# OFA-Sys/ONE-PEACE

Hardware: AMD Instinct MI355X
Metric: pretrain samples/s (tri-modal global batch) ONE-PEACE-4B (higher is better)
Workload: dtype bf16

## Files before the change

one-peace_amd/csrc/attention.hip:

```cpp
#include <type_traits>

#include "common.h"

namespace {

constexpr int HD = 64;
constexpr int BQ = 128;
constexpr int BKV = 64;
constexpr int VSTRIDE = 160;

struct AttnArgs {
  const bf16_t* q; const bf16_t* k; const bf16_t* v; int64_t ld;
  const bf16_t* bias;
  int64_t bias_bs;
  const uint8_t* key_pad;
  bf16_t* out; int64_t ldo;
  float* lse;
  int64_t lse_ld;
  int B, S, Spad, heads;
  float scale;
};

__device__ __forceinline__ bf16x8 pack8(const float* a, const float* b) {
  bf16x8 r;
#pragma unroll
  for (int i = 0; i < 4; ++i) { r[i] = (bf16_t)a[i]; r[4 + i] = (bf16_t)b[i]; }
  return r;
}

__device__ __forceinline__ s16x4 tr_read(const char* p) {
  return __builtin_amdgcn_ds_read_tr16_b64_v4i16((__attribute__((address_space(3))) s16x4*)(p));
}

__device__ __forceinline__ bf16x8 join_tr(s16x4 a, s16x4 b) {
  typedef __attribute__((ext_vector_type(8))) short s16x8;
  s16x8 r = {a[0], a[1], a[2], a[3], b[0], b[1], b[2], b[3]};
  return __builtin_bit_cast(bf16x8, r);
}

__device__ __forceinline__ int tr_off_swz(int rowblk, int db, int g, int t) {
  const int row = rowblk * 16 + g * 4 + (t >> 2);
  const int c = db * 2 + ((t >> 1) & 1);
  return row * 128 + ((c ^ (row & 7)) << 4) + (t & 1) * 8;
}

__device__ __forceinline__ void xcd_work_item(int& bx, int& by, int& bz) {
  const int nx = gridDim.x, ny = gridDim.y;
  const int total = nx * ny * (int)gridDim.z;
  int lin = blockIdx.x + nx * (blockIdx.y + ny * blockIdx.z);
  if ((total & 7) == 0) lin = (lin & 7) * (total >> 3) + (lin >> 3);
  bx = lin % nx;
  by = (lin / nx) % ny;
  bz = lin / (nx * ny);
}

template <bool HAS_BIAS, bool HAS_PAD>
__global__ __launch_bounds__(256, 2) void attn_fwd_kernel(AttnArgs p) {
  __shared__ __attribute__((aligned(16))) char smem[BKV * 128 + BKV * VSTRIDE];
  char* ldsK = smem;
  char* ldsV = smem + BKV * 128;
  const int tid = threadIdx.x, lane = tid & 63, wid = tid >> 6;
  const int g = lane >> 4, t = lane & 15;
  int bx, h, b;
  xcd_work_item(bx, h, b);
  const int q0 = bx * BQ + wid * 32;
  const bool wave_active = q0 < p.S;
  const int64_t row_base = (int64_t)b * p.S;

  bf16x8 qf[2][2];
#pragma unroll
  for (int qb = 0; qb < 2; ++qb) {
    const int qi = min(q0 + qb * 16 + t, p.S - 1);
    const bf16_t* qp = p.q + (row_base + qi) * p.ld + h * HD;
#pragma unroll
    for (int kk = 0; kk < 2; ++kk) qf[qb][kk] = *reinterpret_cast<const bf16x8*>(qp + kk * 32 + g * 8);
  }

  f32x4 ot[2][4];
  float m_run[2], l_run[2];
#pragma unroll
  for (int qb = 0; qb < 2; ++qb) {
    m_run[qb] = -INFINITY;
    l_run[qb] = 0.f;
#pragma unroll
    for (int db = 0; db < 4; ++db) ot[qb][db] = (f32x4){0.f, 0.f, 0.f, 0.f};
  }

  u32x4 rk[2], rv[2];
  int st_row[2], st_c[2];
#pragma unroll
  for (int i = 0; i < 2; ++i) {
    const int c2 = tid + 256 * i;
    st_row[i] = c2 >> 3;
    st_c[i] = c2 & 7;
  }
  auto load_tile = [&](int k0) {
#pragma unroll
    for (int i = 0; i < 2; ++i) {
      const int kr = min(k0 + st_row[i], p.S - 1);
      const int64_t off = (row_base + kr) * p.ld + h * HD + st_c[i] * 8;
      rk[i] = *reinterpret_cast<const u32x4*>(p.k + off);
      rv[i] = *reinterpret_cast<const u32x4*>(p.v + off);
    }
  };
  auto write_tile = [&]() {
#pragma unroll
    for (int i = 0; i < 2; ++i) {
      *reinterpret_cast<u32x4*>(ldsK + st_row[i] * 128 + ((st_c[i] ^ (st_row[i] & 7)) << 4)) = rk[i];
      *reinterpret_cast<u32x4*>(ldsV + st_row[i] * VSTRIDE + st_c[i] * 16) = rv[i];
    }
  };

  const bf16_t* brow[2] = {nullptr, nullptr};
  if constexpr (HAS_BIAS) {
#pragma unroll
    for (int qb = 0; qb < 2; ++qb) {
      const int qi = min(q0 + qb * 16 + t, p.S - 1);
      brow[qb] = p.bias + (int64_t)b * p.bias_bs + ((int64_t)h * p.S + qi) * p.Spad + g * 4;
    }
  }
  const uint8_t* padrow = HAS_PAD ? p.key_pad + (int64_t)b * p.Spad + g * 4 : nullptr;

  auto tile = [&](const int k0, auto full_c) {
    constexpr bool FULL = decltype(full_c)::value;
    const int nkb = FULL ? 4 : ((p.S - k0 + 15) >> 4);
    bf16x4 bv[2][4];
    unsigned padw[4] = {0u, 0u, 0u, 0u};
    if constexpr (HAS_BIAS) {
#pragma unroll
      for (int qb = 0; qb < 2; ++qb)
#pragma unroll
        for (int kb = 0; kb < 4; ++kb) bv[qb][kb] = *reinterpret_cast<const bf16x4*>(brow[qb] + k0 + kb * 16);
    }
    if constexpr (HAS_PAD) {
#pragma unroll
      for (int kb = 0; kb < 4; ++kb) padw[kb] = *reinterpret_cast<const unsigned*>(padrow + k0 + kb * 16);
    }

    f32x4 st[2][4];
#pragma unroll
    for (int qb = 0; qb < 2; ++qb)
#pragma unroll
      for (int kb = 0; kb < 4; ++kb) st[qb][kb] = (f32x4){0.f, 0.f, 0.f, 0.f};
#pragma unroll
    for (int kb = 0; kb < 4; ++kb) {
      if (!FULL && kb >= nkb) break;
#pragma unroll
      for (int kk = 0; kk < 2; ++kk) {
        const bf16x8 kf = *reinterpret_cast<const bf16x8*>(ldsK + (kb * 16 + t) * 128 + (((kk * 4 + g) ^ (t & 7)) << 4));
#pragma unroll
        for (int qb = 0; qb < 2; ++qb)
          st[qb][kb] = __builtin_amdgcn_mfma_f32_16x16x32_bf16(kf, qf[qb][kk], st[qb][kb], 0, 0, 0);
      }
    }

    bf16x8 pf[2][2];
#pragma unroll
    for (int qb = 0; qb < 2; ++qb) {
      float mx = -INFINITY;
#pragma unroll
      for (int kb = 0; kb < 4; ++kb) {
        const int key = k0 + kb * 16 + g * 4;
#pragma unroll
        for (int r = 0; r < 4; ++r) {
          float s = st[qb][kb][r] * p.scale;
          if constexpr (HAS_BIAS) s += (float)bv[qb][kb][r];
          if constexpr (!FULL || HAS_PAD) {
            bool masked = false;
            if constexpr (!FULL) masked = key + r >= p.S;
            if constexpr (HAS_PAD) masked = masked || ((padw[kb] >> (8 * r)) & 0xffu);
            s = masked ? -INFINITY : s;
          }
          st[qb][kb][r] = s;
          mx = fmaxf(mx, s);
        }
      }
      mx = fmaxf(mx, __shfl_xor(mx, 16));
      mx = fmaxf(mx, __shfl_xor(mx, 32));
      const float m_new = fmaxf(m_run[qb], mx);
      const float m_use = (m_new == -INFINITY) ? 0.f : m_new;
      const float alpha = __expf(m_run[qb] - m_use);
      m_run[qb] = m_new;
      float psum = 0.f;
      float pv[4][4];
#pragma unroll
      for (int kb = 0; kb < 4; ++kb)
#pragma unroll
        for (int r = 0; r < 4; ++r) {
          const float e = __expf(st[qb][kb][r] - m_use);
          pv[kb][r] = e;
          psum += e;
        }
      l_run[qb] = l_run[qb] * alpha + psum;
#pragma unroll
      for (int db = 0; db < 4; ++db)
#pragma unroll
        for (int r = 0; r < 4; ++r) ot[qb][db][r] *= alpha;
      pf[qb][0] = pack8(pv[0], pv[1]);
      pf[qb][1] = pack8(pv[2], pv[3]);
    }

#pragma unroll
    for (int m = 0; m < 2; ++m) {
      if (!FULL && 2 * m >= nkb) break;
#pragma unroll
      for (int db = 0; db < 4; ++db) {
        const char* base = ldsV + (t >> 2) * VSTRIDE + (db * 16 + (t & 3) * 4) * 2;
        const s16x4 v0 = tr_read(base + ((2 * m) * 16 + g * 4) * VSTRIDE);
        const s16x4 v1 = tr_read(base + ((2 * m + 1) * 16 + g * 4) * VSTRIDE);
        const bf16x8 vf = join_tr(v0, v1);
#pragma unroll
        for (int qb = 0; qb < 2; ++qb)
          ot[qb][db] = __builtin_amdgcn_mfma_f32_16x16x32_bf16(vf, pf[qb][m], ot[qb][db], 0, 0, 0);
      }
    }
  };

  const int ntiles = (p.S + BKV - 1) / BKV;
  load_tile(0);
  for (int kt = 0; kt < ntiles; ++kt) {
    const int k0 = kt * BKV;
    __syncthreads();
    write_tile();
    __syncthreads();
    if (kt + 1 < ntiles) load_tile(k0 + BKV);
    if (!wave_active) continue;
    if (k0 + BKV <= p.S) tile(k0, std::true_type{});
    else tile(k0, std::false_type{});
  }

  if (!wave_active) return;
#pragma unroll
  for (int qb = 0; qb < 2; ++qb) {
    float l = l_run[qb];
    l += __shfl_xor(l, 16);
    l += __shfl_xor(l, 32);
    const int qi = q0 + qb * 16 + t;
    if (qi >= p.S) continue;
    const float inv = 1.f / l;
    bf16_t* op = p.out + (row_base + qi) * p.ldo + h * HD;
#pragma unroll
    for (int db = 0; db < 4; ++db) {
      bf16x4 o;
#pragma unroll
      for (int r = 0; r < 4; ++r) o[r] = (bf16_t)(ot[qb][db][r] * inv);
      *reinterpret_cast<bf16x4*>(op + db * 16 + g * 4) = o;
    }
    if (g == 0 && p.lse) p.lse[((int64_t)b * p.heads + h) * p.lse_ld + qi] = m_run[qb] + logf(l);
  }
}


constexpr int RES_MAX_S = 320;
constexpr int RES_MAX_NW = 10;
constexpr float LOG2E = 1.4426950408889634f;

constexpr int FRAG_BLOCK = 512;

template <bool HAS_BIAS, bool HAS_PAD>
__global__ __launch_bounds__(RES_MAX_NW * 64, 5) void attn_fwd_res_kernel(AttnArgs p, const bf16_t* __restrict__ bias_frag,
                                                                            int rows_pad, int qb_per_wg, int abl) {
  extern __shared__ __attribute__((aligned(16))) char smem[];
  char* ldsK = smem;
  char* ldsV = smem + rows_pad * 128;
  const int tid = threadIdx.x, lane = tid & 63;
  const int wid = __builtin_amdgcn_readfirstlane(tid >> 6);
  const int nw = blockDim.x >> 6;
  const int g = lane >> 4, t = lane & 15;
  int bx, h, b;
  xcd_work_item(bx, h, b);
  const int64_t row_base = (int64_t)b * p.S;

  if (!(abl & 1)) {
    const int ngrp = rows_pad >> 3;
    const int r_in = lane >> 3, slot = lane & 7;
    for (int grp = wid; grp < 2 * ngrp; grp += nw) {
      const bool isv = grp >= ngrp;
      const int gi = isv ? grp - ngrp : grp;
      const int r = gi * 8 + r_in;
      const int kr = min(r, p.S - 1);
      const bf16_t* src = (isv ? p.v : p.k) + (row_base + kr) * p.ld + h * HD + ((slot ^ (r & 7)) << 3);
      char* dst = (isv ? ldsV : ldsK) + gi * 1024;
      __builtin_amdgcn_global_load_lds((const __attribute__((address_space(1))) void*)src,
                                       (__attribute__((address_space(3))) void*)dst, 16, 0, 0);
    }
  }

  const int nqb = (p.S + 15) >> 4, nkp = (p.S + 31) >> 5;
  for (int lblk = wid, trip = 0; trip == 0 || lblk < qb_per_wg; lblk += nw, ++trip) {
  const int qblk = bx * qb_per_wg + lblk;
  const bool active = lblk < qb_per_wg && qblk < nqb;
  const int q0 = min(qblk, nqb - 1) * 16;
  const int qi = min(q0 + t, p.S - 1);

  bf16x8 qf[2];
  {
    const bf16_t* qp = p.q + (row_base + qi) * p.ld + h * HD;
#pragma unroll
    for (int kk = 0; kk < 2; ++kk) qf[kk] = *reinterpret_cast<const bf16x8*>(qp + kk * 32 + g * 8);
  }
  const bf16_t* fbase = nullptr;
  if constexpr (HAS_BIAS) {
    const int64_t per_head = (int64_t)nqb * nkp * FRAG_BLOCK;
    fbase = bias_frag + ((p.bias_bs != 0 ? (int64_t)b * p.heads : 0) + h) * per_head + (int64_t)(q0 >> 4) * nkp * FRAG_BLOCK + lane * 8;
  }
  const uint8_t* padrow = HAS_PAD ? p.key_pad + (int64_t)b * p.Spad + g * 4 : nullptr;
  bf16x8 sel_lo, sel_hi;
  {
    const bf16_t inv = (bf16_t)(1.0f / p.scale), zero = (bf16_t)0.f;
#pragma unroll
    for (int i = 0; i < 8; ++i) {
      sel_lo[i] = (g * 8 + i == t) ? inv : zero;
      sel_hi[i] = (g * 8 + i == 16 + t) ? inv : zero;
    }
  }

  if (trip == 0) {
    asm volatile("s_waitcnt vmcnt(0)" ::: "memory");
    __syncthreads();
  }
  if (!active || (abl & 2)) continue;

  f32x4 ot[4];
  float m2_run = -INFINITY, l_run = 0.f;
#pragma unroll
  for (int db = 0; db < 4; ++db) ot[db] = (f32x4){0.f, 0.f, 0.f, 0.f};
  int trsw[4];
#pragma unroll
  for (int db = 0; db < 4; ++db) trsw[db] = tr_off_swz(0, db, g, t);
  const int kswz[2] = {((0 * 4 + g) ^ (t & 7)) << 4, ((1 * 4 + g) ^ (t & 7)) << 4};
  const float c1 = p.scale * LOG2E;

  auto tile = [&](const int k0, auto full_c) {
    constexpr bool FULL = decltype(full_c)::value;
    const int nkb = FULL ? 4 : ((p.S - k0 + 15) >> 4);
    bf16x8 bf[2];
    unsigned padw[4] = {0u, 0u, 0u, 0u};
    if constexpr (HAS_BIAS) {
#pragma unroll
      for (int m = 0; m < 2; ++m)
        if (FULL || 2 * m < nkb) bf[m] = *reinterpret_cast<const bf16x8*>(fbase + ((k0 >> 5) + m) * FRAG_BLOCK);
    }
    if constexpr (HAS_PAD) {
#pragma unroll
      for (int kb = 0; kb < 4; ++kb) padw[kb] = *reinterpret_cast<const unsigned*>(padrow + k0 + kb * 16);
    }
    const char* kt = ldsK + k0 * 128;
    const char* vt = ldsV + k0 * 128;

    f32x4 st[4];
#pragma unroll
    for (int kb = 0; kb < 4; ++kb) st[kb] = (f32x4){0.f, 0.f, 0.f, 0.f};
#pragma unroll
    for (int kb = 0; kb < 4; ++kb) {
      if (!FULL && kb >= nkb) break;
#pragma unroll
      for (int kk = 0; kk < 2; ++kk) {
        const bf16x8 kf = *reinterpret_cast<const bf16x8*>(kt + (kb * 16 + t) * 128 + kswz[kk]);
        st[kb] = __builtin_amdgcn_mfma_f32_16x16x32_bf16(kf, qf[kk], st[kb], 0, 0, 0);
      }
      if constexpr (HAS_BIAS)
        st[kb] = __builtin_amdgcn_mfma_f32_16x16x32_bf16(bf[kb >> 1], (kb & 1) ? sel_hi : sel_lo, st[kb], 0, 0, 0);
    }

    float mx = -INFINITY;
#pragma unroll
    for (int kb = 0; kb < 4; ++kb) {
      if (!FULL && kb >= nkb) break;
      const int key = k0 + kb * 16 + g * 4;
#pragma unroll
      for (int r = 0; r < 4; ++r) {
        if constexpr (!FULL || HAS_PAD) {
          bool masked = false;
          if constexpr (!FULL) masked = key + r >= p.S;
          if constexpr (HAS_PAD) masked = masked || ((padw[kb] >> (8 * r)) & 0xffu);
          st[kb][r] = masked ? -INFINITY : st[kb][r];
        }
        mx = fmaxf(mx, st[kb][r]);
      }
    }
    mx = fmaxf(mx, __shfl_xor(mx, 16));
    mx = fmaxf(mx, __shfl_xor(mx, 32));
    const float m2_new = fmaxf(m2_run, mx * c1);
    const float m2_use = (m2_new == -INFINITY) ? 0.f : m2_new;
    const float alpha = __builtin_amdgcn_exp2f(m2_run - m2_use);
    m2_run = m2_new;
    float psum = 0.f;
    float pv[4][4];
#pragma unroll
    for (int kb = 0; kb < 4; ++kb) {
      if (FULL || kb < nkb) {
#pragma unroll
        for (int r = 0; r < 4; ++r) {
          const float e = __builtin_amdgcn_exp2f(__builtin_fmaf(st[kb][r], c1, -m2_use));
          pv[kb][r] = e;
          psum += e;
        }
      } else {
#pragma unroll
        for (int r = 0; r < 4; ++r) pv[kb][r] = 0.f;
      }
    }
    l_run = l_run * alpha + psum;
#pragma unroll
    for (int db = 0; db < 4; ++db)
#pragma unroll
      for (int r = 0; r < 4; ++r) ot[db][r] *= alpha;
    bf16x8 pf[2];
    pf[0] = pack8(pv[0], pv[1]);
    pf[1] = pack8(pv[2], pv[3]);

#pragma unroll
    for (int m = 0; m < 2; ++m) {
      if (!FULL && 2 * m >= nkb) break;
#pragma unroll
      for (int db = 0; db < 4; ++db) {
        const bf16x8 vf = join_tr(tr_read(vt + trsw[db] + (2 * m) * 2048), tr_read(vt + trsw[db] + (2 * m + 1) * 2048));
        ot[db] = __builtin_amdgcn_mfma_f32_16x16x32_bf16(vf, pf[m], ot[db], 0, 0, 0);
      }
    }
  };

  const int ntiles = (p.S + BKV - 1) / BKV;
  for (int kt = 0; kt < ntiles; ++kt) {
    const int k0 = kt * BKV;
    if (k0 + BKV <= p.S) tile(k0, std::true_type{});
    else tile(k0, std::false_type{});
  }

  float l = l_run;
  l += __shfl_xor(l, 16);
  l += __shfl_xor(l, 32);
  if (q0 + t >= p.S) continue;
  const float inv = 1.f / l;
  bf16_t* op = p.out + (row_base + q0 + t) * p.ldo + h * HD;
#pragma unroll
  for (int db = 0; db < 4; ++db) {
    bf16x4 o;
#pragma unroll
    for (int r = 0; r < 4; ++r) o[r] = (bf16_t)(ot[db][r] * inv);
    *reinterpret_cast<bf16x4*>(op + db * 16 + g * 4) = o;
  }
  if (g == 0 && p.lse) p.lse[((int64_t)b * p.heads + h) * p.lse_ld + q0 + t] = m2_run * (1.0f / LOG2E) + logf(l);
  }
}

constexpr int PERS_NW = 8;
constexpr int PERS_MAX_ROWS = 288;
constexpr int PERS_SCR = 68;
constexpr int PERS_PPT = 2;

__device__ __forceinline__ s16x4 tr_read_a(const char* p) {
  s16x4 r;
  asm volatile("ds_read_b64_tr_b16 %0, %1" : "=v"(r) : "v"((unsigned)(uintptr_t)((__attribute__((address_space(3))) const char*)p)));
  return r;
}
#define ATTN_WAIT_LGKM0()                         \
  do {                                            \
    __builtin_amdgcn_s_waitcnt(0xC07F);           \
    __builtin_amdgcn_sched_barrier(0);            \
  } while (0)

__device__ __forceinline__ void gload16_asm(bf16x8& d, const void* p) { asm volatile("global_load_dwordx4 %0, %1, off" : "=v"(d) : "v"(p)); }
__device__ __forceinline__ void gload4_asm(unsigned& d, const void* p) { asm volatile("global_load_dword %0, %1, off" : "=v"(d) : "v"(p)); }
template <int OFF>
__device__ __forceinline__ void gload16_s(bf16x8& d, const void* sbase, unsigned voff) {
  asm volatile("s_nop 4\n\tglobal_load_dwordx4 %0, %1, %2 offset:%3" : "=v"(d) : "v"(voff), "s"(sbase), "n"(OFF));
}
template <int OFF>
__device__ __forceinline__ void gload4_s(unsigned& d, const void* sbase, unsigned voff) {
  asm volatile("s_nop 4\n\tglobal_load_dword %0, %1, %2 offset:%3" : "=v"(d) : "v"(voff), "s"(sbase), "n"(OFF));
}

template <bool HAS_BIAS, bool HAS_PAD>
__global__ __launch_bounds__(PERS_NW * 64, 2) void attn_fwd_pers_kernel(AttnArgs p, const bf16_t* __restrict__ bias_frag, int rows_pad,
                                                                         int nitems) {
  extern __shared__ __attribute__((aligned(16))) char smem[];
  const int tid = threadIdx.x, lane = tid & 63;
  const int wid = __builtin_amdgcn_readfirstlane(tid >> 6);
  const int g = lane >> 4, t = lane & 15;
  const int KVB = 2 * rows_pad * 128;
  float* scratch = reinterpret_cast<float*>(smem + 2 * KVB);
  const int nqb = (p.S + 15) >> 4, nkp = (p.S + 31) >> 5;
  const bool has_left = nqb > 2 * PERS_NW;
  const int q0 = wid * 32;
  const int nact = min(2, max(0, nqb - 2 * wid));
  const int64_t per_head = (int64_t)nqb * nkp * FRAG_BLOCK;
  const int ntiles = (p.S + BKV - 1) / BKV;
  const float c1 = p.scale * LOG2E;

  bf16x8 sel_lo, sel_hi;
  {
    const bf16_t inv = (bf16_t)(1.0f / p.scale), zero = (bf16_t)0.f;
#pragma unroll
    for (int i = 0; i < 8; ++i) {
      sel_lo[i] = (g * 8 + i == t) ? inv : zero;
      sel_hi[i] = (g * 8 + i == 16 + t) ? inv : zero;
    }
  }
  int trsw[4];
#pragma unroll
  for (int db = 0; db < 4; ++db) trsw[db] = tr_off_swz(0, db, g, t);
  const int kswz[2] = {((0 * 4 + g) ^ (t & 7)) << 4, ((1 * 4 + g) ^ (t & 7)) << 4};

  const int ngrp = rows_pad >> 3;
  const int r_in = lane >> 3, slot = lane & 7;
  const int npiece = (2 * ngrp - wid + PERS_NW - 1) / PERS_NW;
  auto piece = [&](int it, int buf, int j) {
    const int b = it / p.heads, h = it - b * p.heads;
    const int grp = wid + j * PERS_NW;
    const bool isv = grp >= ngrp;
    const int gi = isv ? grp - ngrp : grp;
    const int r = gi * 8 + r_in;
    const int kr = min(r, p.S - 1);
    const bf16_t* src = (isv ? p.v : p.k) + ((int64_t)b * p.S + kr) * p.ld + h * HD + ((slot ^ (r & 7)) << 3);
    char* dst = smem + buf * KVB + (isv ? rows_pad * 128 : 0) + gi * 1024;
    __builtin_amdgcn_global_load_lds((const __attribute__((address_space(1))) void*)src,
                                     (__attribute__((address_space(3))) void*)dst, 16, 0, 0);
  };
  auto load_q = [&](int it, int qrow, bf16x8 (&q)[2]) {
    const int b = it / p.heads, h = it - b * p.heads;
    const bf16_t* qp = p.q + ((int64_t)b * p.S + qrow) * p.ld + h * HD;
#pragma unroll
    for (int kk = 0; kk < 2; ++kk) q[kk] = *reinterpret_cast<const bf16x8*>(qp + kk * 32 + g * 8);
  };
  const int qi_main[2] = {min(q0 + t, p.S - 1), min(q0 + 16 + t, p.S - 1)};

  bf16x8 bn[2][2];
  unsigned padn[4] = {0u, 0u, 0u, 0u};
  auto small_loads = [&](int it, int kt) {
    const int b = it / p.heads, h = it - b * p.heads;
    if constexpr (HAS_BIAS) {
      const bf16_t* fhead = bias_frag + ((p.bias_bs != 0 ? (int64_t)b * p.heads : 0) + h) * per_head + lane * 8;
#pragma unroll
      for (int qb = 0; qb < 2; ++qb) {
        const bf16_t* fb = fhead + (int64_t)min(2 * wid + qb, nqb - 1) * nkp * FRAG_BLOCK;
#pragma unroll
        for (int m = 0; m < 2; ++m) gload16_asm(bn[qb][m], fb + min(2 * kt + m, nkp - 1) * FRAG_BLOCK);
      }
    }
    if constexpr (HAS_PAD) {
      const uint8_t* pr = p.key_pad + (int64_t)b * p.Spad + g * 4 + kt * BKV;
#pragma unroll
      for (int kb = 0; kb < 4; ++kb) gload4_asm(padn[kb], pr + kb * 16);
    }
  };

  constexpr int NSMALL = (HAS_BIAS ? 4 : 0) + (HAS_PAD ? 4 : 0);
  bf16x8 qn[2][2], ql[2], bfl[2];
  unsigned padl[2][2] = {{0u, 0u}, {0u, 0u}};
  auto late_loads = [&](int it_next, int it) {
    {
      const int b = it_next / p.heads, h = it_next - b * p.heads;
#pragma unroll
      for (int qb = 0; qb < 2; ++qb) {
        const bf16_t* qp = p.q + ((int64_t)b * p.S + qi_main[qb]) * p.ld + h * HD;
#pragma unroll
        for (int kk = 0; kk < 2; ++kk) gload16_asm(qn[qb][kk], qp + kk * 32 + g * 8);
      }
    }
    if (has_left) {
      const int b = it / p.heads, h = it - b * p.heads;
      const bf16_t* qp = p.q + ((int64_t)b * p.S + p.S - 1) * p.ld + h * HD;
#pragma unroll
      for (int kk = 0; kk < 2; ++kk) gload16_asm(ql[kk], qp + kk * 32 + g * 8);
      if constexpr (HAS_BIAS) {
        const bf16_t* fleft = bias_frag + ((p.bias_bs != 0 ? (int64_t)b * p.heads : 0) + h) * per_head + lane * 8 + (int64_t)(nqb - 1) * nkp * FRAG_BLOCK;
        gload16_asm(bfl[0], fleft + wid * FRAG_BLOCK);
        gload16_asm(bfl[1], fleft + min(PERS_NW, nkp - 1) * FRAG_BLOCK);
      }
      if constexpr (HAS_PAD) {
        const uint8_t* pr = p.key_pad + (int64_t)b * p.Spad + g * 4;
#pragma unroll
        for (int j = 0; j < 2; ++j) {
          gload4_asm(padl[0][j], pr + (2 * wid + j) * 16);
          gload4_asm(padl[1][j], pr + min((2 * PERS_NW + j) * 16, p.Spad - 16));
        }
      }
    }
  };

  int item = blockIdx.x;
  const int step = gridDim.x;
  if (item < nitems) {
    for (int j = 0; j < npiece; ++j) piece(item, 0, j);
    load_q(item, qi_main[0], qn[0]);
    load_q(item, qi_main[1], qn[1]);
    small_loads(item, 0);
  }
  int buf = 0, prev_item = -1;
  auto wait_all = [&]() {
    asm volatile("s_waitcnt vmcnt(0)" : "+v"(qn[0][0]), "+v"(qn[0][1]), "+v"(qn[1][0]), "+v"(qn[1][1]), "+v"(bn[0][0]), "+v"(bn[0][1]), "+v"(bn[1][0]), "+v"(bn[1][1]),
                 "+v"(padn[0]), "+v"(padn[1]), "+v"(padn[2]), "+v"(padn[3]) : : "memory");
  };
  wait_all();

  auto merge_left = [&](int it, int sb) {
    const float* sc = scratch + sb * (PERS_NW * PERS_SCR);
    float M = -INFINITY;
#pragma unroll
    for (int w = 0; w < PERS_NW; ++w) M = fmaxf(M, sc[w * PERS_SCR + 64]);
    float L = 0.f, o = 0.f;
#pragma unroll
    for (int w = 0; w < PERS_NW; ++w) {
      const float f = __builtin_amdgcn_exp2f(sc[w * PERS_SCR + 64] - M);
      L = __builtin_fmaf(sc[w * PERS_SCR + 65], f, L);
      o = __builtin_fmaf(sc[w * PERS_SCR + lane], f, o);
    }
    const int b = it / p.heads, h = it - b * p.heads;
    const int qrow = p.S - 1;
    p.out[((int64_t)b * p.S + qrow) * p.ldo + h * HD + lane] = (bf16_t)(o / L);
    if (lane == 0 && p.lse) p.lse[((int64_t)b * p.heads + h) * p.lse_ld + qrow] = M * (1.0f / LOG2E) + logf(L);
  };

  for (; item < nitems; item += step, buf ^= 1) {
    const int b = item / p.heads, h = item - b * p.heads;
    const int64_t row_base = (int64_t)b * p.S;
    __syncthreads();
    bf16x8 qf[2][2] = {{qn[0][0], qn[0][1]}, {qn[1][0], qn[1][1]}};
    const bool more = item + step < nitems;
    const int nxt = more ? item + step : item;
    if (has_left && prev_item >= 0 && wid == ((prev_item / step) & (PERS_NW - 1))) merge_left(prev_item, buf ^ 1);
    prev_item = item;

    const char* ldsK = smem + buf * KVB;
    const char* ldsV = ldsK + rows_pad * 128;

    f32x4 ot[2][4];
    float m2_run[2] = {-INFINITY, -INFINITY}, l_run[2] = {0.f, 0.f};
#pragma unroll
    for (int qb = 0; qb < 2; ++qb)
#pragma unroll
      for (int db = 0; db < 4; ++db) ot[qb][db] = (f32x4){0.f, 0.f, 0.f, 0.f};

    auto tile = [&](const int kt, auto full_c) {
      constexpr bool FULL = decltype(full_c)::value;
      const int k0 = kt * BKV;
      const int nkb = FULL ? 4 : ((p.S - k0 + 15) >> 4);
      bf16x8 bf[2][2];
      unsigned padw[4] = {0u, 0u, 0u, 0u};
      if constexpr (HAS_BIAS) {
#pragma unroll
        for (int qb = 0; qb < 2; ++qb)
#pragma unroll
          for (int m = 0; m < 2; ++m) bf[qb][m] = bn[qb][m];
      }
      if constexpr (HAS_PAD) {
#pragma unroll
        for (int kb = 0; kb < 4; ++kb) padw[kb] = padn[kb];
      }
      __builtin_amdgcn_sched_barrier(0);
      if constexpr (FULL) {
        small_loads(item, kt + 1);
      } else {
        late_loads(nxt, item);
        small_loads(nxt, 0);
      }
      __builtin_amdgcn_sched_barrier(0);
#pragma unroll
      for (int jj = 0; jj < PERS_PPT; ++jj) piece(nxt, buf ^ 1, min(kt * PERS_PPT + jj, npiece - 1));
      __builtin_amdgcn_sched_barrier(0);
      if (nact == 0) return;

      const char* kt_ = ldsK + k0 * 128;
      const char* vt = ldsV + k0 * 128;
      f32x4 st[2][4];
#pragma unroll
      for (int qb = 0; qb < 2; ++qb)
#pragma unroll
        for (int kb = 0; kb < 4; ++kb) st[qb][kb] = (f32x4){0.f, 0.f, 0.f, 0.f};
#pragma unroll
      for (int kb = 0; kb < 4; ++kb) {
        if (!FULL && kb >= nkb) break;
#pragma unroll
        for (int kk = 0; kk < 2; ++kk) {
          const bf16x8 kf = *reinterpret_cast<const bf16x8*>(kt_ + (kb * 16 + t) * 128 + kswz[kk]);
#pragma unroll
          for (int qb = 0; qb < 2; ++qb) st[qb][kb] = __builtin_amdgcn_mfma_f32_16x16x32_bf16(kf, qf[qb][kk], st[qb][kb], 0, 0, 0);
        }
        if constexpr (HAS_BIAS) {
#pragma unroll
          for (int qb = 0; qb < 2; ++qb)
            st[qb][kb] = __builtin_amdgcn_mfma_f32_16x16x32_bf16(bf[qb][kb >> 1], (kb & 1) ? sel_hi : sel_lo, st[qb][kb], 0, 0, 0);
        }
      }
      s16x4 va0[4], va1[4];
#pragma unroll
      for (int db = 0; db < 4; ++db) {
        va0[db] = tr_read_a(vt + trsw[db]);
        va1[db] = tr_read_a(vt + trsw[db] + 2048);
      }
      bf16x8 pf[2][2];
#pragma unroll
      for (int qb = 0; qb < 2; ++qb) {
        float mx = -INFINITY;
#pragma unroll
        for (int kb = 0; kb < 4; ++kb) {
          if (!FULL && kb >= nkb) break;
          const int key = k0 + kb * 16 + g * 4;
#pragma unroll
          for (int r = 0; r < 4; ++r) {
            if constexpr (!FULL || HAS_PAD) {
              bool masked = false;
              if constexpr (!FULL) masked = key + r >= p.S;
              if constexpr (HAS_PAD) masked = masked || ((padw[kb] >> (8 * r)) & 0xffu);
              st[qb][kb][r] = masked ? -INFINITY : st[qb][kb][r];
            }
            mx = fmaxf(mx, st[qb][kb][r]);
          }
        }
        mx = fmaxf(mx, __shfl_xor(mx, 16));
        mx = fmaxf(mx, __shfl_xor(mx, 32));
        const float m2_new = fmaxf(m2_run[qb], mx * c1);
        const float m2_use = (m2_new == -INFINITY) ? 0.f : m2_new;
        const float alpha = __builtin_amdgcn_exp2f(m2_run[qb] - m2_use);
        m2_run[qb] = m2_new;
        float psum = 0.f;
        float pv[4][4];
#pragma unroll
        for (int kb = 0; kb < 4; ++kb) {
          if (FULL || kb < nkb) {
#pragma unroll
            for (int r = 0; r < 4; ++r) {
              const float e = __builtin_amdgcn_exp2f(__builtin_fmaf(st[qb][kb][r], c1, -m2_use));
              pv[kb][r] = e;
              psum += e;
            }
          } else {
#pragma unroll
            for (int r = 0; r < 4; ++r) pv[kb][r] = 0.f;
          }
        }
        l_run[qb] = l_run[qb] * alpha + psum;
#pragma unroll
        for (int db = 0; db < 4; ++db)
#pragma unroll
          for (int r = 0; r < 4; ++r) ot[qb][db][r] *= alpha;
        pf[qb][0] = pack8(pv[0], pv[1]);
        pf[qb][1] = pack8(pv[2], pv[3]);
      }
      const bool second = FULL || nkb > 2;
      ATTN_WAIT_LGKM0();
      s16x4 vb0[4], vb1[4];
      if (second) {
#pragma unroll
        for (int db = 0; db < 4; ++db) {
          vb0[db] = tr_read_a(vt + trsw[db] + 2 * 2048);
          vb1[db] = tr_read_a(vt + trsw[db] + 3 * 2048);
        }
      }
#pragma unroll
      for (int db = 0; db < 4; ++db) {
        const bf16x8 vf = join_tr(va0[db], va1[db]);
#pragma unroll
        for (int qb = 0; qb < 2; ++qb) ot[qb][db] = __builtin_amdgcn_mfma_f32_16x16x32_bf16(vf, pf[qb][0], ot[qb][db], 0, 0, 0);
      }
      if (second) {
        ATTN_WAIT_LGKM0();
#pragma unroll
        for (int db = 0; db < 4; ++db) {
          const bf16x8 vf = join_tr(vb0[db], vb1[db]);
#pragma unroll
          for (int qb = 0; qb < 2; ++qb) ot[qb][db] = __builtin_amdgcn_mfma_f32_16x16x32_bf16(vf, pf[qb][1], ot[qb][db], 0, 0, 0);
        }
      }
    };
    auto wait_small = [&]() {
      if constexpr (HAS_BIAS && HAS_PAD)
        asm volatile("s_waitcnt vmcnt(%8)" : "+v"(bn[0][0]), "+v"(bn[0][1]), "+v"(bn[1][0]), "+v"(bn[1][1]), "+v"(padn[0]), "+v"(padn[1]), "+v"(padn[2]), "+v"(padn[3]) : "n"(PERS_PPT));
      else if constexpr (HAS_BIAS)
        asm volatile("s_waitcnt vmcnt(%4)" : "+v"(bn[0][0]), "+v"(bn[0][1]), "+v"(bn[1][0]), "+v"(bn[1][1]) : "n"(PERS_PPT));
      else if constexpr (HAS_PAD)
        asm volatile("s_waitcnt vmcnt(%4)" : "+v"(padn[0]), "+v"(padn[1]), "+v"(padn[2]), "+v"(padn[3]) : "n"(PERS_PPT));
    };
#pragma unroll 1
    for (int kt = 0; kt < ntiles - 1; ++kt) {
      tile(kt, std::true_type{});
      wait_small();
    }
    tile(ntiles - 1, std::false_type{});
    if (has_left) {
      f32x4 ol[4];
      float m2 = -INFINITY, lsum = 0.f;
#pragma unroll
      for (int db = 0; db < 4; ++db) ol[db] = (f32x4){0.f, 0.f, 0.f, 0.f};
      asm volatile("s_waitcnt vmcnt(%8)" : "+v"(ql[0]), "+v"(ql[1]), "+v"(bfl[0]), "+v"(bfl[1]), "+v"(padl[0][0]), "+v"(padl[0][1]), "+v"(padl[1][0]), "+v"(padl[1][1]) : "n"(NSMALL + PERS_PPT));
      const int npc = wid == 0 ? 2 : 1;
      for (int pc = 0; pc < npc; ++pc) {
        const int kp = pc == 0 ? wid : PERS_NW;
        f32x4 s4[2];
        const unsigned padw[2] = {padl[pc][0], padl[pc][1]};
#pragma unroll
        for (int j = 0; j < 2; ++j) {
          s4[j] = (f32x4){0.f, 0.f, 0.f, 0.f};
#pragma unroll
          for (int kk = 0; kk < 2; ++kk) {
            const bf16x8 kf = *reinterpret_cast<const bf16x8*>(ldsK + ((2 * kp + j) * 16 + t) * 128 + kswz[kk]);
            s4[j] = __builtin_amdgcn_mfma_f32_16x16x32_bf16(kf, ql[kk], s4[j], 0, 0, 0);
          }
          if constexpr (HAS_BIAS) s4[j] = __builtin_amdgcn_mfma_f32_16x16x32_bf16(bfl[pc], j ? sel_hi : sel_lo, s4[j], 0, 0, 0);
        }
        float mx = -INFINITY;
#pragma unroll
        for (int j = 0; j < 2; ++j)
#pragma unroll
          for (int r = 0; r < 4; ++r) {
            bool masked = (2 * kp + j) * 16 + g * 4 + r >= p.S;
            if constexpr (HAS_PAD) masked = masked || ((padw[j] >> (8 * r)) & 0xffu);
            s4[j][r] = masked ? -INFINITY : s4[j][r];
            mx = fmaxf(mx, s4[j][r]);
          }
        mx = fmaxf(mx, __shfl_xor(mx, 16));
        mx = fmaxf(mx, __shfl_xor(mx, 32));
        const float m2_new = fmaxf(m2, mx * c1);
        const float m2_use = (m2_new == -INFINITY) ? 0.f : m2_new;
        const float alpha = __builtin_amdgcn_exp2f(m2 - m2_use);
        m2 = m2_new;
        float pv[2][4];
        float psum = 0.f;
#pragma unroll
        for (int j = 0; j < 2; ++j)
#pragma unroll
          for (int r = 0; r < 4; ++r) {
            pv[j][r] = __builtin_amdgcn_exp2f(__builtin_fmaf(s4[j][r], c1, -m2_use));
            psum += pv[j][r];
          }
        lsum = lsum * alpha + psum;
        const bf16x8 pf = pack8(pv[0], pv[1]);
        s16x4 v0[4], v1[4];
#pragma unroll
        for (int db = 0; db < 4; ++db) {
          v0[db] = tr_read_a(ldsV + trsw[db] + (2 * kp) * 2048);
          v1[db] = tr_read_a(ldsV + trsw[db] + (2 * kp + 1) * 2048);
        }
        ATTN_WAIT_LGKM0();
#pragma unroll
        for (int db = 0; db < 4; ++db) {
#pragma unroll
          for (int r = 0; r < 4; ++r) ol[db][r] *= alpha;
          ol[db] = __builtin_amdgcn_mfma_f32_16x16x32_bf16(join_tr(v0[db], v1[db]), pf, ol[db], 0, 0, 0);
        }
      }
      lsum += __shfl_xor(lsum, 16);
      lsum += __shfl_xor(lsum, 32);
      float* sc = scratch + (buf * PERS_NW + wid) * PERS_SCR;
      if (t == 0) {
#pragma unroll
        for (int db = 0; db < 4; ++db) *reinterpret_cast<f32x4*>(sc + db * 16 + g * 4) = ol[db];
        if (g == 0) { sc[64] = m2; sc[65] = lsum; }
      }
    }
#pragma unroll
    for (int qb = 0; qb < 2; ++qb) {
      float l = l_run[qb];
      l += __shfl_xor(l, 16);
      l += __shfl_xor(l, 32);
      const int qrow = q0 + qb * 16 + t;
      if (qb < nact && qrow < p.S) {
        const float inv = 1.f / l;
        bf16_t* op = p.out + (row_base + qrow) * p.ldo + h * HD;
#pragma unroll
        for (int db = 0; db < 4; ++db) {
          bf16x4 o;
#pragma unroll
          for (int r = 0; r < 4; ++r) o[r] = (bf16_t)(ot[qb][db][r] * inv);
          *reinterpret_cast<bf16x4*>(op + db * 16 + g * 4) = o;
        }
        if (g == 0 && p.lse) p.lse[((int64_t)b * p.heads + h) * p.lse_ld + qrow] = m2_run[qb] * (1.0f / LOG2E) + logf(l);
      }
    }
    wait_all();
  }
  if (has_left && prev_item >= 0) {
    __syncthreads();
    if (wid == 0) merge_left(prev_item, buf ^ 1);
  }
}

__global__ __launch_bounds__(256) void bias_pack_kernel(const bf16_t* __restrict__ src, bf16_t* __restrict__ dst, int S, int Spad,
                                                        int nqb, int nkp, int64_t total) {
  const int64_t idx = (int64_t)blockIdx.x * 256 + threadIdx.x;
  if (idx >= total) return;
  const int lane = (int)(idx & 63);
  int64_t blk = idx >> 6;
  const int kp = (int)(blk % nkp);
  blk /= nkp;
  const int qb = (int)(blk % nqb);
  const int64_t img = blk / nqb;
  const int g = lane >> 4, t = lane & 15;
  const int key = kp * 32 + (g >> 1) * 16 + t;
  const int qbase = qb * 16 + (g & 1) * 8;
  bf16x8 v;
#pragma unroll
  for (int i = 0; i < 8; ++i) {
    const int q = qbase + i;
    v[i] = (q < S && key < S) ? src[(img * S + q) * Spad + key] : (bf16_t)0.f;
  }
  *reinterpret_cast<bf16x8*>(dst + idx * 8) = v;
}

struct AttnBwdArgs {
  const bf16_t* q; const bf16_t* k; const bf16_t* v; int64_t ld;
  const bf16_t* dout; int64_t ldo;
  const bf16_t* bias;
  const bf16_t* biasT;
  const bf16_t* bias_frag;
  int64_t bias_bs;
  const uint8_t* key_pad;
  const float* lse;
  const float* delta;
  const bf16_t* out;
  float* delta_w;
  bf16_t* dq; bf16_t* dk; bf16_t* dv; int64_t ldg;
  float* dbias;
  int B, S, Spad, heads, bchunk;
  float scale;
  int lone_keys;
};

__global__ __launch_bounds__(256) void attn_delta_kernel(const bf16_t* __restrict__ dout, const bf16_t* __restrict__ out,
                                                         int64_t ldo, float* __restrict__ delta, int B, int S, int Spad,
                                                         int heads) {
  const int64_t gid = (int64_t)blockIdx.x * 256 + threadIdx.x;
  const int per_row = heads * 8;
  const int64_t row = gid / per_row;
  const int rem = (int)(gid - row * per_row);
  float s = 0.f;
  if (row < (int64_t)B * S) {
    float a[8], b[8];
    Vec8<bf16_t>::load(dout + row * ldo + rem * 8, a);
    Vec8<bf16_t>::load(out + row * ldo + rem * 8, b);
#pragma unroll
    for (int j = 0; j < 8; ++j) s += a[j] * b[j];
  }
  s += __shfl_xor(s, 1);
  s += __shfl_xor(s, 2);
  s += __shfl_xor(s, 4);
  if (row < (int64_t)B * S && (rem & 7) == 0) {
    const int h = rem >> 3;
    const int64_t bb = row / S;
    const int qi = (int)(row - bb * S);
    delta[(bb * heads + h) * Spad + qi] = s;
  }
}

__device__ __forceinline__ float delta_from_frags(const bf16x8 (&dO)[2], const bf16x8 (&O)[2]) {
  float s = 0.f;
#pragma unroll
  for (int kk = 0; kk < 2; ++kk)
#pragma unroll
    for (int i = 0; i < 8; ++i) s = __builtin_fmaf((float)dO[kk][i], (float)O[kk][i], s);
  s += __shfl_xor(s, 16);
  s += __shfl_xor(s, 32);
  return s;
}

template <bool HAS_BIAS, int KBW, bool LONE>
__device__ __forceinline__ void attn_bwd_dkdv_body(const AttnBwdArgs& p, char* smem, int bx, int h, int b) {
  constexpr int KB = LONE ? 1 : KBW;
  char* ldsQ = smem;
  char* ldsO = smem + 64 * 128;
  const int tid = threadIdx.x, lane = tid & 63, wid = tid >> 6;
  const int g = lane >> 4, t = lane & 15;
  const int kbase = LONE ? bx * (64 * KBW) : bx * (64 * KBW) + wid * (16 * KBW);
  const bool wave_active = LONE || kbase < p.S;
  const int my_m = wid >> 1, my_j = wid & 1;
  const int64_t row_base = (int64_t)b * p.S;

  bf16x8 kf[KB][2], vf[KB][2];
  bool kdead[KB];
#pragma unroll
  for (int kb = 0; kb < KB; ++kb) {
    const int key = kbase + kb * 16 + t;
    const int kc = min(key, p.S - 1);
    const int64_t off = (row_base + kc) * p.ld + h * HD;
#pragma unroll
    for (int kk = 0; kk < 2; ++kk) {
      kf[kb][kk] = *reinterpret_cast<const bf16x8*>(p.k + off + kk * 32 + g * 8);
      vf[kb][kk] = *reinterpret_cast<const bf16x8*>(p.v + off + kk * 32 + g * 8);
    }
    kdead[kb] = p.key_pad && key < p.S && p.key_pad[(int64_t)b * p.Spad + key];
  }
  f32x4 dvT[KB][4], dkT[KB][4];
#pragma unroll
  for (int kb = 0; kb < KB; ++kb)
#pragma unroll
    for (int db = 0; db < 4; ++db) { dvT[kb][db] = (f32x4){0.f, 0.f, 0.f, 0.f}; dkT[kb][db] = (f32x4){0.f, 0.f, 0.f, 0.f}; }

  u32x4 rq[2], ro[2];
  int st_row[2], st_c[2];
#pragma unroll
  for (int i = 0; i < 2; ++i) { const int c2 = tid + 256 * i; st_row[i] = c2 >> 3; st_c[i] = c2 & 7; }
  auto load_tile = [&](int q0) {
#pragma unroll
    for (int i = 0; i < 2; ++i) {
      const int qr = min(q0 + st_row[i], p.S - 1);
      rq[i] = *reinterpret_cast<const u32x4*>(p.q + (row_base + qr) * p.ld + h * HD + st_c[i] * 8);
      ro[i] = *reinterpret_cast<const u32x4*>(p.dout + (row_base + qr) * p.ldo + h * HD + st_c[i] * 8);
    }
  };
  auto write_tile = [&]() {
#pragma unroll
    for (int i = 0; i < 2; ++i) {
      const int off = st_row[i] * 128 + ((st_c[i] ^ (st_row[i] & 7)) << 4);
      *reinterpret_cast<u32x4*>(ldsQ + off) = rq[i];
      *reinterpret_cast<u32x4*>(ldsO + off) = ro[i];
    }
  };
  int trsw[4];
#pragma unroll
  for (int db = 0; db < 4; ++db) trsw[db] = tr_off_swz(0, db, g, t);

  const int ntiles = (p.S + 63) / 64;
  const float* lse_b = p.lse + ((int64_t)b * p.heads + h) * p.Spad;
  const float* del_b = p.delta + ((int64_t)b * p.heads + h) * p.Spad;
  const bf16_t* brow[KB] = {};
  bf16x8 sel_lo, sel_hi;
  if constexpr (HAS_BIAS) {
#pragma unroll
    for (int kb = 0; kb < KB; ++kb) {
      const int key = min(kbase + kb * 16 + t, p.S - 1);
      brow[kb] = p.biasT + (int64_t)b * p.bias_bs + ((int64_t)h * p.S + key) * p.Spad + g * 8;
    }
    const bf16_t inv = (bf16_t)(1.0f / p.scale), zero = (bf16_t)0.f;
#pragma unroll
    for (int i = 0; i < 8; ++i) {
      sel_lo[i] = (g * 8 + i == t) ? inv : zero;
      sel_hi[i] = (g * 8 + i == 16 + t) ? inv : zero;
    }
  }
  const float c1 = p.scale * LOG2E;
  load_tile(0);
  for (int qt = 0; qt < ntiles; ++qt) {
    const int q0 = qt * 64;
    __syncthreads();
    write_tile();
    __syncthreads();
    if (!wave_active) {
      load_tile(q0 + 64);
      continue;
    }
    f32x4 l4[2][2], d4[2][2];
    bf16x8 bfr[2][KB];
#pragma unroll
    for (int m = 0; m < 2; ++m) {
#pragma unroll
      for (int j = 0; j < 2; ++j) {
        const int qrow = q0 + (2 * m + j) * 16 + g * 4;
        l4[m][j] = *reinterpret_cast<const f32x4*>(lse_b + qrow);
        d4[m][j] = *reinterpret_cast<const f32x4*>(del_b + qrow);
      }
      if constexpr (HAS_BIAS) {
#pragma unroll
        for (int kb = 0; kb < KB; ++kb) bfr[m][kb] = *reinterpret_cast<const bf16x8*>(brow[kb] + q0 + m * 32);
      }
    }
    __builtin_amdgcn_sched_barrier(0);
    load_tile(q0 + 64);
    __builtin_amdgcn_sched_barrier(0);

#pragma unroll
    for (int m = 0; m < 2; ++m) {
      if (q0 + m * 32 >= p.S) break;
      if (LONE && (m != my_m || q0 + (2 * m + my_j) * 16 >= p.S)) continue;
      f32x4 s[2][KB], dp[2][KB];
#pragma unroll
      for (int j = 0; j < 2; ++j)
#pragma unroll
        for (int kb = 0; kb < KB; ++kb) { s[j][kb] = (f32x4){0.f, 0.f, 0.f, 0.f}; dp[j][kb] = (f32x4){0.f, 0.f, 0.f, 0.f}; }
#pragma unroll
      for (int j = 0; j < 2; ++j) {
        if (LONE && j != my_j) continue;
        if (q0 + (2 * m + j) * 16 >= p.S) continue;
        const int qb = 2 * m + j;
#pragma unroll
        for (int kk = 0; kk < 2; ++kk) {
          const int off = (qb * 16 + t) * 128 + (((kk * 4 + g) ^ (t & 7)) << 4);
          const bf16x8 qfr = *reinterpret_cast<const bf16x8*>(ldsQ + off);
          const bf16x8 ofr = *reinterpret_cast<const bf16x8*>(ldsO + off);
#pragma unroll
          for (int kb = 0; kb < KB; ++kb) {
            s[j][kb] = __builtin_amdgcn_mfma_f32_16x16x32_bf16(qfr, kf[kb][kk], s[j][kb], 0, 0, 0);
            dp[j][kb] = __builtin_amdgcn_mfma_f32_16x16x32_bf16(ofr, vf[kb][kk], dp[j][kb], 0, 0, 0);
          }
        }
        if constexpr (HAS_BIAS) {
#pragma unroll
          for (int kb = 0; kb < KB; ++kb)
            s[j][kb] = __builtin_amdgcn_mfma_f32_16x16x32_bf16(j ? sel_hi : sel_lo, bfr[m][kb], s[j][kb], 0, 0, 0);
        }
      }
#pragma unroll
      for (int j = 0; j < 2; ++j) {
        if ((LONE && j != my_j) || q0 + (2 * m + j) * 16 >= p.S) continue;
        const int qrow = q0 + (2 * m + j) * 16 + g * 4;
        float l2[4], dl[4];
#pragma unroll
        for (int r = 0; r < 4; ++r) {
          const bool live = qrow + r < p.S;
          l2[r] = live ? l4[m][j][r] * LOG2E : INFINITY;
          dl[r] = live ? d4[m][j][r] : 0.f;
        }
#pragma unroll
        for (int kb = 0; kb < KB; ++kb) {
#pragma unroll
          for (int r = 0; r < 4; ++r) {
            const float pr = __builtin_amdgcn_exp2f(__builtin_fmaf(s[j][kb][r], c1, -l2[r]));
            s[j][kb][r] = pr;
            dp[j][kb][r] = pr * (dp[j][kb][r] - dl[r]);
          }
        }
      }
      bf16x8 pfr[KB], dsf[KB];
#pragma unroll
      for (int kb = 0; kb < KB; ++kb) {
        float a0[4], a1[4], b0[4], b1[4];
#pragma unroll
        for (int r = 0; r < 4; ++r) {
          a0[r] = s[0][kb][r]; a1[r] = s[1][kb][r];
          b0[r] = dp[0][kb][r]; b1[r] = dp[1][kb][r];
        }
        pfr[kb] = pack8(a0, a1);
        dsf[kb] = pack8(b0, b1);
      }
#pragma unroll
      for (int db = 0; db < 4; ++db) {
        const bf16x8 oT = join_tr(tr_read(ldsO + trsw[db] + (2 * m) * 2048), tr_read(ldsO + trsw[db] + (2 * m + 1) * 2048));
        const bf16x8 qT = join_tr(tr_read(ldsQ + trsw[db] + (2 * m) * 2048), tr_read(ldsQ + trsw[db] + (2 * m + 1) * 2048));
#pragma unroll
        for (int kb = 0; kb < KB; ++kb) {
          dvT[kb][db] = __builtin_amdgcn_mfma_f32_16x16x32_bf16(oT, pfr[kb], dvT[kb][db], 0, 0, 0);
          dkT[kb][db] = __builtin_amdgcn_mfma_f32_16x16x32_bf16(qT, dsf[kb], dkT[kb][db], 0, 0, 0);
        }
      }
    }
  }
  if (!wave_active) return;
  if constexpr (LONE) {
    f32x4* red = reinterpret_cast<f32x4*>(smem);
#pragma unroll
    for (int which = 0; which < 2; ++which) {
      __syncthreads();
      if (wid > 0) {
#pragma unroll
        for (int db = 0; db < 4; ++db) red[((wid - 1) * 4 + db) * 64 + lane] = which ? dkT[0][db] : dvT[0][db];
      }
      __syncthreads();
      if (wid == 0) {
#pragma unroll
        for (int w = 0; w < 3; ++w)
#pragma unroll
          for (int db = 0; db < 4; ++db) {
            if (which) dkT[0][db] += red[(w * 4 + db) * 64 + lane];
            else dvT[0][db] += red[(w * 4 + db) * 64 + lane];
          }
      }
    }
    if (wid > 0) return;
  }
#pragma unroll
  for (int kb = 0; kb < KB; ++kb) {
    const int key = kbase + kb * 16 + t;
    if (key >= p.S) continue;
    bf16_t* kp = p.dk + (row_base + key) * p.ldg + h * HD;
    bf16_t* vp = p.dv + (row_base + key) * p.ldg + h * HD;
#pragma unroll
    for (int db = 0; db < 4; ++db) {
      bf16x4 a, c;
#pragma unroll
      for (int r = 0; r < 4; ++r) {
        a[r] = kdead[kb] ? (bf16_t)0.f : (bf16_t)(dkT[kb][db][r] * p.scale);
        c[r] = kdead[kb] ? (bf16_t)0.f : (bf16_t)dvT[kb][db][r];
      }
      *reinterpret_cast<bf16x4*>(kp + db * 16 + g * 4) = a;
      *reinterpret_cast<bf16x4*>(vp + db * 16 + g * 4) = c;
    }
  }
}

template <bool HAS_BIAS, int KB>
__global__ __launch_bounds__(256, KB == 1 ? 3 : 2) void attn_bwd_dkdv_kernel(AttnBwdArgs p) {
  __shared__ __attribute__((aligned(16))) char smem[2 * 64 * 128];
  int bx, h, b;
  xcd_work_item(bx, h, b);
  if (KB == 2 && bx > 0 && p.S - bx * 128 <= 16 && p.lone_keys) attn_bwd_dkdv_body<HAS_BIAS, KB, true>(p, smem, bx, h, b);
  else attn_bwd_dkdv_body<HAS_BIAS, KB, false>(p, smem, bx, h, b);
}

template <int QB, bool HAS_BIAS, bool HOIST, typename KF, typename VF, typename BF, typename PF>
__device__ __forceinline__ void ds_tile(const AttnBwdArgs& p, int b, int h, int k0, int q0w, int g, int t,
                                        const bf16x8 (&qf)[QB][2], const bf16x8 (&of)[QB][2], const float (&lse)[QB],
                                        const float (&del)[QB], KF kfrag, VF vfrag, BF biasfrag, PF prefetch,
                                        f32x4 (&ds)[QB][4]) {
  unsigned padw[4] = {0u, 0u, 0u, 0u};
  auto load_pad = [&]() {
    if (p.key_pad) {
#pragma unroll
      for (int kb = 0; kb < 4; ++kb)
        padw[kb] = *reinterpret_cast<const unsigned*>(p.key_pad + (int64_t)b * p.Spad + k0 + kb * 16 + g * 4);
    }
  };
  if constexpr (HOIST) load_pad();
  bf16x4 bv[QB][4];
  if constexpr (HAS_BIAS && HOIST) {
#pragma unroll
    for (int qb = 0; qb < QB; ++qb) {
      const int qi = min(q0w + qb * 16 + t, p.S - 1);
#pragma unroll
      for (int kb = 0; kb < 4; ++kb) bv[qb][kb] = biasfrag(qb, kb, qi, k0 + kb * 16 + g * 4);
    }
  }
  if constexpr (HOIST) __builtin_amdgcn_sched_barrier(0);
  prefetch();
  if constexpr (HOIST) __builtin_amdgcn_sched_barrier(0);
  f32x4 st[QB][4];
#pragma unroll
  for (int qb = 0; qb < QB; ++qb)
#pragma unroll
    for (int kb = 0; kb < 4; ++kb) { st[qb][kb] = (f32x4){0.f, 0.f, 0.f, 0.f}; ds[qb][kb] = (f32x4){0.f, 0.f, 0.f, 0.f}; }
#pragma unroll
  for (int kb = 0; kb < 4; ++kb) {
    if (k0 + kb * 16 >= p.S) break;
#pragma unroll
    for (int kk = 0; kk < 2; ++kk) {
      const bf16x8 kfr = kfrag(kb, kk);
      const bf16x8 vfr = vfrag(kb, kk);
#pragma unroll
      for (int qb = 0; qb < QB; ++qb) {
        st[qb][kb] = __builtin_amdgcn_mfma_f32_16x16x32_bf16(kfr, qf[qb][kk], st[qb][kb], 0, 0, 0);
        ds[qb][kb] = __builtin_amdgcn_mfma_f32_16x16x32_bf16(vfr, of[qb][kk], ds[qb][kb], 0, 0, 0);
      }
    }
  }
  if constexpr (!HOIST) load_pad();
#pragma unroll
  for (int qb = 0; qb < QB; ++qb) {
    const int qraw = q0w + qb * 16 + t;
    const int qi = min(qraw, p.S - 1);
#pragma unroll
    for (int kb = 0; kb < 4; ++kb) {
      const int key = k0 + kb * 16 + g * 4;
      if constexpr (HAS_BIAS && !HOIST) bv[qb][kb] = biasfrag(qb, kb, qi, key);
#pragma unroll
      for (int r = 0; r < 4; ++r) {
        const bool dead = (key + r >= p.S) || ((padw[kb] >> (8 * r)) & 0xffu) || (qraw >= p.S);
        float x = st[qb][kb][r] * p.scale;
        if constexpr (HAS_BIAS) x += (float)bv[qb][kb][r];
        x -= lse[qb];
        float pr;
        if constexpr (HOIST) pr = __expf(dead ? -INFINITY : x);
        else pr = dead ? 0.f : __expf(x);
        const float dsv = pr * (ds[qb][kb][r] - del[qb]);
        ds[qb][kb][r] = dead ? 0.f : dsv;
      }
    }
  }
}

template <bool HAS_BIAS>
__global__ __launch_bounds__(256, 2) void attn_bwd_dq_kernel(AttnBwdArgs p) {
  __shared__ __attribute__((aligned(16))) char smem[2 * 64 * 128];
  char* ldsK = smem;
  char* ldsV = smem + 64 * 128;
  const int tid = threadIdx.x, lane = tid & 63, wid = tid >> 6;
  const int g = lane >> 4, t = lane & 15;
  int bx, h, b;
  xcd_work_item(bx, h, b);
  const int q0w = bx * BQ + wid * 32;
  const bool wave_active = q0w < p.S;
  const int64_t row_base = (int64_t)b * p.S;

  bf16x8 qf[2][2], of[2][2];
  float lse[2], del[2];
#pragma unroll
  for (int qb = 0; qb < 2; ++qb) {
    const int qi = min(q0w + qb * 16 + t, p.S - 1);
#pragma unroll
    for (int kk = 0; kk < 2; ++kk) {
      qf[qb][kk] = *reinterpret_cast<const bf16x8*>(p.q + (row_base + qi) * p.ld + h * HD + kk * 32 + g * 8);
      of[qb][kk] = *reinterpret_cast<const bf16x8*>(p.dout + (row_base + qi) * p.ldo + h * HD + kk * 32 + g * 8);
    }
    lse[qb] = p.lse[((int64_t)b * p.heads + h) * p.Spad + qi];
    if (p.out) {
      bf16x8 oo[2];
#pragma unroll
      for (int kk = 0; kk < 2; ++kk) oo[kk] = *reinterpret_cast<const bf16x8*>(p.out + (row_base + qi) * p.ldo + h * HD + kk * 32 + g * 8);
      del[qb] = delta_from_frags(of[qb], oo);
      if (g == 0 && q0w + qb * 16 + t < p.S) p.delta_w[((int64_t)b * p.heads + h) * p.Spad + qi] = del[qb];
    } else {
      del[qb] = p.delta[((int64_t)b * p.heads + h) * p.Spad + qi];
    }
  }
  f32x4 dqT[2][4];
#pragma unroll
  for (int qb = 0; qb < 2; ++qb)
#pragma unroll
    for (int db = 0; db < 4; ++db) dqT[qb][db] = (f32x4){0.f, 0.f, 0.f, 0.f};

  u32x4 rk[2], rv[2];
  int st_row[2], st_c[2];
#pragma unroll
  for (int i = 0; i < 2; ++i) { const int c2 = tid + 256 * i; st_row[i] = c2 >> 3; st_c[i] = c2 & 7; }
  auto load_tile = [&](int k0) {
#pragma unroll
    for (int i = 0; i < 2; ++i) {
      const int kr = min(k0 + st_row[i], p.S - 1);
      const int64_t off = (row_base + kr) * p.ld + h * HD + st_c[i] * 8;
      rk[i] = *reinterpret_cast<const u32x4*>(p.k + off);
      rv[i] = *reinterpret_cast<const u32x4*>(p.v + off);
    }
  };
  auto write_tile = [&]() {
#pragma unroll
    for (int i = 0; i < 2; ++i) {
      const int off = st_row[i] * 128 + ((st_c[i] ^ (st_row[i] & 7)) << 4);
      *reinterpret_cast<u32x4*>(ldsK + off) = rk[i];
      *reinterpret_cast<u32x4*>(ldsV + off) = rv[i];
    }
  };
  int trsw[4];
#pragma unroll
  for (int db = 0; db < 4; ++db) trsw[db] = tr_off_swz(0, db, g, t);

  const int ntiles = (p.S + BKV - 1) / BKV;
  load_tile(0);
  for (int kt = 0; kt < ntiles; ++kt) {
    const int k0 = kt * BKV;
    __syncthreads();
    write_tile();
    __syncthreads();
    if (!wave_active) {
      load_tile(k0 + BKV);
      continue;
    }
    auto prefetch = [&]() { load_tile(k0 + BKV); };
    f32x4 ds[2][4];
    auto kfrag = [&](int kb, int kk) {
      return *reinterpret_cast<const bf16x8*>(ldsK + (kb * 16 + t) * 128 + (((kk * 4 + g) ^ (t & 7)) << 4));
    };
    auto vfrag = [&](int kb, int kk) {
      return *reinterpret_cast<const bf16x8*>(ldsV + (kb * 16 + t) * 128 + (((kk * 4 + g) ^ (t & 7)) << 4));
    };
    auto biasfrag = [&](int, int, int qi, int key) {
      return *reinterpret_cast<const bf16x4*>(p.bias + (int64_t)b * p.bias_bs + ((int64_t)h * p.S + qi) * p.Spad + key);
    };
    ds_tile<2, HAS_BIAS, true>(p, b, h, k0, q0w, g, t, qf, of, lse, del, kfrag, vfrag, biasfrag, prefetch, ds);
#pragma unroll
    for (int m = 0; m < 2; ++m) {
      if (k0 + m * 32 >= p.S) break;
      bf16x8 dsf[2];
#pragma unroll
      for (int qb = 0; qb < 2; ++qb) {
        float a0[4], a1[4];
#pragma unroll
        for (int r = 0; r < 4; ++r) { a0[r] = ds[qb][2 * m][r]; a1[r] = ds[qb][2 * m + 1][r]; }
        dsf[qb] = pack8(a0, a1);
      }
#pragma unroll
      for (int db = 0; db < 4; ++db) {
        const bf16x8 kT = join_tr(tr_read(ldsK + trsw[db] + (2 * m) * 2048), tr_read(ldsK + trsw[db] + (2 * m + 1) * 2048));
#pragma unroll
        for (int qb = 0; qb < 2; ++qb)
          dqT[qb][db] = __builtin_amdgcn_mfma_f32_16x16x32_bf16(kT, dsf[qb], dqT[qb][db], 0, 0, 0);
      }
    }
  }
  if (!wave_active) return;
#pragma unroll
  for (int qb = 0; qb < 2; ++qb) {
    const int qi = q0w + qb * 16 + t;
    if (qi >= p.S) continue;
    bf16_t* qp = p.dq + (row_base + qi) * p.ldg + h * HD;
#pragma unroll
    for (int db = 0; db < 4; ++db) {
      bf16x4 a;
#pragma unroll
      for (int r = 0; r < 4; ++r) a[r] = (bf16_t)(dqT[qb][db][r] * p.scale);
      *reinterpret_cast<bf16x4*>(qp + db * 16 + g * 4) = a;
    }
  }
}

template <int NT, bool FRAG, int LASTB>
__global__ __launch_bounds__(256, 2) void attn_bwd_dq_dbias_kernel(AttnBwdArgs p) {
  __shared__ __attribute__((aligned(16))) char smem[2 * 64 * 128];
  char* ldsK = smem;
  char* ldsV = smem + 64 * 128;
  const int tid = threadIdx.x, lane = tid & 63, wid = tid >> 6;
  const int g = lane >> 4, t = lane & 15;
  int bx, h, chunk;
  xcd_work_item(bx, h, chunk);
  const int q0w = bx * 64 + wid * 16;
  const bool wave_active = q0w < p.S;
  const int qi = min(q0w + t, p.S - 1);

  f32x4 acc[NT][4];
#pragma unroll
  for (int kt = 0; kt < NT; ++kt)
#pragma unroll
    for (int kb = 0; kb < 4; ++kb) acc[kt][kb] = (f32x4){0.f, 0.f, 0.f, 0.f};

  u32x4 rk[2], rv[2];
  int st_row[2], st_c[2];
#pragma unroll
  for (int i = 0; i < 2; ++i) { const int c2 = tid + 256 * i; st_row[i] = c2 >> 3; st_c[i] = c2 & 7; }
  auto load_tile = [&](int b, int k0) {
#pragma unroll
    for (int i = 0; i < 2; ++i) {
      const int kr = min(k0 + st_row[i], p.S - 1);
      const int64_t off = ((int64_t)b * p.S + kr) * p.ld + h * HD + st_c[i] * 8;
      rk[i] = *reinterpret_cast<const u32x4*>(p.k + off);
      rv[i] = *reinterpret_cast<const u32x4*>(p.v + off);
    }
  };
  auto write_tile = [&]() {
#pragma unroll
    for (int i = 0; i < 2; ++i) {
      const int off = st_row[i] * 128 + ((st_c[i] ^ (st_row[i] & 7)) << 4);
      *reinterpret_cast<u32x4*>(ldsK + off) = rk[i];
      *reinterpret_cast<u32x4*>(ldsV + off) = rv[i];
    }
  };
  bf16x8 qn[1][2], on[1][2], oon[2];
  float lsen[1], deln[1];
  const bool own_delta = p.out != nullptr;
  auto load_q = [&](int b) {
    const int64_t row = (int64_t)b * p.S + qi;
#pragma unroll
    for (int kk = 0; kk < 2; ++kk) {
      qn[0][kk] = *reinterpret_cast<const bf16x8*>(p.q + row * p.ld + h * HD + kk * 32 + g * 8);
      on[0][kk] = *reinterpret_cast<const bf16x8*>(p.dout + row * p.ldo + h * HD + kk * 32 + g * 8);
      if (own_delta) oon[kk] = *reinterpret_cast<const bf16x8*>(p.out + row * p.ldo + h * HD + kk * 32 + g * 8);
    }
    lsen[0] = p.lse[((int64_t)b * p.heads + h) * p.Spad + qi];
    if (!own_delta) deln[0] = p.delta[((int64_t)b * p.heads + h) * p.Spad + qi];
  };
  int trsw[4];
#pragma unroll
  for (int db = 0; db < 4; ++db) trsw[db] = tr_off_swz(0, db, g, t);

  const int nqb = (p.S + 15) >> 4, nkp = (p.S + 31) >> 5;
  const int64_t per_head = (int64_t)nqb * nkp * FRAG_BLOCK;
  const bf16_t* fbase = nullptr;
  bf16x8 sel_lo, sel_hi;
  const float c1 = p.scale * LOG2E;
  if constexpr (FRAG) {
    fbase = p.bias_frag + (int64_t)h * per_head + (int64_t)(min(q0w, p.S - 1) >> 4) * nkp * FRAG_BLOCK + lane * 8;
    const bf16_t inv = (bf16_t)(1.0f / p.scale), zero = (bf16_t)0.f;
#pragma unroll
    for (int i = 0; i < 8; ++i) {
      sel_lo[i] = (g * 8 + i == t) ? inv : zero;
      sel_hi[i] = (g * 8 + i == 16 + t) ? inv : zero;
    }
  }
  const int b_begin = chunk * p.bchunk, b_end = min(p.B, (chunk + 1) * p.bchunk);
  if (b_begin >= b_end) return;
  load_tile(b_begin, 0);
  load_q(b_begin);
  for (int b = b_begin; b < b_end; ++b) {
    bf16x8 qf[1][2], of[1][2];
    float lse[1], del[1];
#pragma unroll
    for (int kk = 0; kk < 2; ++kk) { qf[0][kk] = qn[0][kk]; of[0][kk] = on[0][kk]; }
    lse[0] = lsen[0];
    if (own_delta) {
      del[0] = delta_from_frags(of[0], oon);
      if (g == 0 && q0w + t < p.S) p.delta_w[((int64_t)b * p.heads + h) * p.Spad + qi] = del[0];
    } else {
      del[0] = deln[0];
    }
    if (b + 1 < b_end) load_q(b + 1);
    int bias_resample = 0;
    asm volatile("" : "+s"(bias_resample));
    f32x4 dqT[4];
#pragma unroll
    for (int db = 0; db < 4; ++db) dqT[db] = (f32x4){0.f, 0.f, 0.f, 0.f};
#pragma unroll 1
    for (int kt = 0; kt < NT; ++kt) {
      const int k0 = kt * BKV;
      __syncthreads();
      write_tile();
      __syncthreads();
      const bool last_kt = kt + 1 >= NT;
      const int nb = last_kt ? min(b + 1, b_end - 1) : b, nk0 = last_kt ? 0 : k0 + BKV;
      auto prefetch = [&]() { load_tile(nb, nk0); };
      if (!wave_active) {
        prefetch();
        continue;
      }
      f32x4 ds[1][4];
      auto kfrag = [&](int kb, int kk) {
        return *reinterpret_cast<const bf16x8*>(ldsK + (kb * 16 + t) * 128 + (((kk * 4 + g) ^ (t & 7)) << 4));
      };
      auto vfrag = [&](int kb, int kk) {
        return *reinterpret_cast<const bf16x8*>(ldsV + (kb * 16 + t) * 128 + (((kk * 4 + g) ^ (t & 7)) << 4));
      };
      auto biasfrag = [&](int, int, int qrow, int key) {
        return *reinterpret_cast<const bf16x4*>(p.bias + bias_resample + (int64_t)b * p.bias_bs + ((int64_t)h * p.S + qrow) * p.Spad + key);
      };
      if constexpr (FRAG) {
        bf16x8 bfr[2];
        unsigned padw[4] = {0u, 0u, 0u, 0u};
        const bf16_t* fb = fbase + (p.bias_bs != 0 ? (int64_t)b * p.heads * per_head : 0) + bias_resample;
#pragma unroll
        for (int m = 0; m < 2; ++m) bfr[m] = *reinterpret_cast<const bf16x8*>(fb + (int64_t)min((k0 >> 5) + m, nkp - 1) * FRAG_BLOCK);
        if (p.key_pad) {
#pragma unroll
          for (int kb = 0; kb < 4; ++kb)
            padw[kb] = *reinterpret_cast<const unsigned*>(p.key_pad + (int64_t)b * p.Spad + k0 + kb * 16 + g * 4);
        }
        __builtin_amdgcn_sched_barrier(0);
        prefetch();
        __builtin_amdgcn_sched_barrier(0);
        f32x4 st[4];
#pragma unroll
        for (int kb = 0; kb < 4; ++kb) { st[kb] = (f32x4){0.f, 0.f, 0.f, 0.f}; ds[0][kb] = (f32x4){0.f, 0.f, 0.f, 0.f}; }
#pragma unroll
        for (int kb = 0; kb < 4; ++kb) {
          if (k0 + kb * 16 >= p.S) break;
#pragma unroll
          for (int kk = 0; kk < 2; ++kk) {
            st[kb] = __builtin_amdgcn_mfma_f32_16x16x32_bf16(kfrag(kb, kk), qf[0][kk], st[kb], 0, 0, 0);
            ds[0][kb] = __builtin_amdgcn_mfma_f32_16x16x32_bf16(vfrag(kb, kk), of[0][kk], ds[0][kb], 0, 0, 0);
          }
          st[kb] = __builtin_amdgcn_mfma_f32_16x16x32_bf16(bfr[kb >> 1], (kb & 1) ? sel_hi : sel_lo, st[kb], 0, 0, 0);
        }
        const float nl2 = -lse[0] * LOG2E, dl = del[0];
        const bool may_mask = (k0 + BKV > p.S) || (p.key_pad != nullptr);
        if (may_mask) {
#pragma unroll
          for (int kb = 0; kb < 4; ++kb) {
            const int key = k0 + kb * 16 + g * 4;
#pragma unroll
            for (int r = 0; r < 4; ++r) {
              const bool dead = (key + r >= p.S) || ((padw[kb] >> (8 * r)) & 0xffu);
              const float pr = __builtin_amdgcn_exp2f(dead ? -INFINITY : __builtin_fmaf(st[kb][r], c1, nl2));
              ds[0][kb][r] = pr * (ds[0][kb][r] - dl);
            }
          }
        } else {
#pragma unroll
          for (int kb = 0; kb < 4; ++kb)
#pragma unroll
            for (int r = 0; r < 4; ++r)
              ds[0][kb][r] = __builtin_amdgcn_exp2f(__builtin_fmaf(st[kb][r], c1, nl2)) * (ds[0][kb][r] - dl);
        }
      } else {
        ds_tile<1, true, (NT < 6)>(p, b, h, k0, q0w, g, t, qf, of, lse, del, kfrag, vfrag, biasfrag, prefetch, ds);
      }
#pragma unroll
      for (int c = 0; c < NT; ++c) {
        if (kt == c) {
#pragma unroll
          for (int kb = 0; kb < 4; ++kb)
            if (c < NT - 1 || kb < LASTB) acc[c][kb] += ds[0][kb];
        }
      }
#pragma unroll
      for (int m = 0; m < 2; ++m) {
        if (k0 + m * 32 >= p.S) break;
        float a0[4], a1[4];
#pragma unroll
        for (int r = 0; r < 4; ++r) { a0[r] = ds[0][2 * m][r]; a1[r] = ds[0][2 * m + 1][r]; }
        const bf16x8 dsf = pack8(a0, a1);
#pragma unroll
        for (int db = 0; db < 4; ++db) {
          const bf16x8 kT = join_tr(tr_read(ldsK + trsw[db] + (2 * m) * 2048), tr_read(ldsK + trsw[db] + (2 * m + 1) * 2048));
          dqT[db] = __builtin_amdgcn_mfma_f32_16x16x32_bf16(kT, dsf, dqT[db], 0, 0, 0);
        }
      }
    }
    if (wave_active && q0w + t < p.S) {
      bf16_t* qp = p.dq + ((int64_t)b * p.S + q0w + t) * p.ldg + h * HD;
#pragma unroll
      for (int db = 0; db < 4; ++db) {
        bf16x4 a;
#pragma unroll
        for (int r = 0; r < 4; ++r) a[r] = (bf16_t)(dqT[db][r] * p.scale);
        *reinterpret_cast<bf16x4*>(qp + db * 16 + g * 4) = a;
      }
    }
  }
  if (!wave_active || q0w + t >= p.S) return;
  float* drow = p.dbias + (((int64_t)chunk * p.heads + h) * p.S + q0w + t) * p.Spad + g * 4;
#pragma unroll
  for (int kt = 0; kt < NT; ++kt) {
    f32x4 cur[4];
#pragma unroll
    for (int kb = 0; kb < 4; ++kb)
      if ((kt < NT - 1 || kb < LASTB) && kt * BKV + kb * 16 < p.Spad) cur[kb] = *reinterpret_cast<const f32x4*>(drow + kt * BKV + kb * 16);
#pragma unroll
    for (int kb = 0; kb < 4; ++kb)
      if ((kt < NT - 1 || kb < LASTB) && kt * BKV + kb * 16 < p.Spad)
        *reinterpret_cast<f32x4*>(drow + kt * BKV + kb * 16) = cur[kb] + acc[kt][kb];
  }
}

template <bool HAS_BIAS, bool HAS_PAD, int NT, int LASTB, bool LEFT>
__device__ __forceinline__ void attn_bwd_dq_pers_body(const AttnBwdArgs& p, char* smem, int rows_pad, int nqh, int qhalf0) {
  const int tid = threadIdx.x, lane = tid & 63;
  const int wid = __builtin_amdgcn_readfirstlane(tid >> 6);
  const int g = lane >> 4, t = lane & 15;
  const int KVB = 2 * rows_pad * 128;
  float* scratch = reinterpret_cast<float*>(smem + 2 * KVB);
  const int nqb = (p.S + 15) >> 4, nkp = (p.S + 31) >> 5;
  const int qhalf = qhalf0, h = (blockIdx.x / nqh) % p.heads, chunk = blockIdx.x / (nqh * p.heads);
  const int b_begin = chunk * p.bchunk, b_end = min(p.B, b_begin + p.bchunk);
  if (b_begin >= b_end) return;
  const int qblk = qhalf * PERS_NW + wid;
  const bool active = qblk < min(nqb, 2 * PERS_NW);
  constexpr bool has_left = LEFT;
  const int q0w = min(qblk, nqb - 1) * 16;
  const int qi = min(q0w + t, p.S - 1);
  const float c1 = p.scale * LOG2E;
  const int64_t per_head = (int64_t)nqb * nkp * FRAG_BLOCK;

  bf16x8 sel_lo, sel_hi;
  {
    const bf16_t inv = (bf16_t)(1.0f / p.scale), zero = (bf16_t)0.f;
#pragma unroll
    for (int i = 0; i < 8; ++i) {
      sel_lo[i] = (g * 8 + i == t) ? inv : zero;
      sel_hi[i] = (g * 8 + i == 16 + t) ? inv : zero;
    }
  }
  int trsw[4];
#pragma unroll
  for (int db = 0; db < 4; ++db) trsw[db] = tr_off_swz(0, db, g, t);
  const int kswz[2] = {((0 * 4 + g) ^ (t & 7)) << 4, ((1 * 4 + g) ^ (t & 7)) << 4};

  const int ngrp = rows_pad >> 3;
  const int r_in = lane >> 3, slot = lane & 7;
  const int npiece = (2 * ngrp - wid + PERS_NW - 1) / PERS_NW;
  auto piece = [&](int b, int buf, int j) {
    const int grp = wid + j * PERS_NW;
    const bool isv = grp >= ngrp;
    const int gi = isv ? grp - ngrp : grp;
    int rl = r_in;
    asm volatile("" : "+v"(rl));
    const int r = gi * 8 + rl;
    const int kr = min(r, p.S - 1);
    const unsigned voff = (unsigned)((kr * (int)p.ld + ((slot ^ (r & 7)) << 3)) * 2);
    const char* sbase = (const char*)((isv ? p.v : p.k) + (int64_t)b * p.S * p.ld + h * HD);
    char* dst = smem + buf * KVB + (isv ? rows_pad * 128 : 0) + gi * 1024;
    __builtin_amdgcn_global_load_lds((const __attribute__((address_space(1))) void*)(sbase + voff),
                                     (__attribute__((address_space(3))) void*)dst, 16, 0, 0);
  };

  constexpr int NSMALL = (HAS_BIAS ? 2 : 0) + (HAS_PAD ? 4 : 0);
  constexpr int BPPT = 3;
  auto ppt_of = [](int kt) { return kt < 3 ? BPPT : 0; };
  const bf16_t* fwave = HAS_BIAS ? p.bias_frag + (int64_t)h * per_head + (int64_t)(q0w >> 4) * nkp * FRAG_BLOCK : nullptr;
  const bf16_t* fleft = HAS_BIAS ? p.bias_frag + (int64_t)h * per_head + (int64_t)(nqb - 1) * nkp * FRAG_BLOCK : nullptr;
  const unsigned vo_frag = lane * 16, vo_pad = g * 4;
  const unsigned vo_q = (unsigned)(((int64_t)qi * p.ld + h * HD + g * 8) * 2), vo_o = (unsigned)(((int64_t)qi * p.ldo + h * HD + g * 8) * 2);
  const unsigned vo_ql = (unsigned)(((int64_t)(p.S - 1) * p.ld + h * HD + g * 8) * 2), vo_ol = (unsigned)(((int64_t)(p.S - 1) * p.ldo + h * HD + g * 8) * 2);
  const unsigned vo_lse = qi * 4, vo_lsel = (p.S - 1) * 4;
  bf16x8 bn[2];
  unsigned padn[4] = {0u, 0u, 0u, 0u};
  auto small_loads = [&](int b, int kt) {
    if constexpr (HAS_BIAS) {
      gload16_s<0>(bn[0], fwave + min(2 * kt, nkp - 1) * FRAG_BLOCK, vo_frag);
      gload16_s<0>(bn[1], fwave + min(2 * kt + 1, nkp - 1) * FRAG_BLOCK, vo_frag);
    }
    if constexpr (HAS_PAD) {
      const uint8_t* pr = p.key_pad + (int64_t)b * p.Spad + kt * BKV;
      gload4_s<0>(padn[0], pr, vo_pad);
      gload4_s<16>(padn[1], pr, vo_pad);
      gload4_s<32>(padn[2], pr, vo_pad);
      gload4_s<48>(padn[3], pr, vo_pad);
    }
  };
  bf16x8 qn[2], don[2], oon[2], ql[2], dol[2], ool[2], bfl[2];
  float lsen, lsel;
  unsigned padl[2][2] = {{0u, 0u}, {0u, 0u}};
  auto query_loads = [&](int b, unsigned voq, unsigned voo, unsigned vol, bf16x8 (&q)[2], bf16x8 (&d)[2], bf16x8 (&o)[2], float& l) {
    const bf16_t* sq = p.q + (int64_t)b * p.S * p.ld;
    const bf16_t* sd = p.dout + (int64_t)b * p.S * p.ldo;
    const bf16_t* so = p.out + (int64_t)b * p.S * p.ldo;
    gload16_s<0>(q[0], sq, voq);
    gload16_s<64>(q[1], sq, voq);
    gload16_s<0>(d[0], sd, voo);
    gload16_s<64>(d[1], sd, voo);
    gload16_s<0>(o[0], so, voo);
    gload16_s<64>(o[1], so, voo);
    unsigned lw;
    gload4_s<0>(lw, p.lse + ((int64_t)b * p.heads + h) * p.Spad, vol);
    l = __builtin_bit_cast(float, lw);
  };
  auto late_loads = [&](int b_next, int b) {
    (void)b_next;
    if (has_left) {
      query_loads(b, vo_ql, vo_ol, vo_lsel, ql, dol, ool, lsel);
      if constexpr (HAS_BIAS) {
        gload16_s<0>(bfl[0], fleft + wid * FRAG_BLOCK, vo_frag);
        gload16_s<0>(bfl[1], fleft + min(PERS_NW, nkp - 1) * FRAG_BLOCK, vo_frag);
      }
      if constexpr (HAS_PAD) {
        const uint8_t* pr = p.key_pad + (int64_t)b * p.Spad;
        gload4_s<0>(padl[0][0], pr + 2 * wid * 16, vo_pad);
        gload4_s<16>(padl[0][1], pr + 2 * wid * 16, vo_pad);
        gload4_s<0>(padl[1][0], pr + min(2 * PERS_NW * 16, p.Spad - 32), vo_pad);
        gload4_s<16>(padl[1][1], pr + min(2 * PERS_NW * 16, p.Spad - 32), vo_pad);
      }
    }
  };

  f32x4 acc[NT][4], accl[2][2];
#pragma unroll
  for (int kt = 0; kt < NT; ++kt)
#pragma unroll
    for (int kb = 0; kb < 4; ++kb) acc[kt][kb] = (f32x4){0.f, 0.f, 0.f, 0.f};
#pragma unroll
  for (int i = 0; i < 2; ++i)
#pragma unroll
    for (int j = 0; j < 2; ++j) accl[i][j] = (f32x4){0.f, 0.f, 0.f, 0.f};

  for (int j = 0; j < npiece; ++j) piece(b_begin, 0, j);
  query_loads(b_begin, vo_q, vo_o, vo_lse, qn, don, oon, lsen);
  small_loads(b_begin, 0);
  int buf = 0, prev_b = -1;
  auto merge_left = [&](int b, int sb) {
    const float* sc = scratch + sb * (PERS_NW * 64);
    float o = 0.f;
#pragma unroll
    for (int w = 0; w < PERS_NW; ++w) o += sc[w * 64 + lane];
    p.dq[((int64_t)b * p.S + p.S - 1) * p.ldg + h * HD + lane] = (bf16_t)(o * p.scale);
  };

  auto wait_all = [&]() {
    asm volatile("s_waitcnt vmcnt(0)" : "+v"(qn[0]), "+v"(qn[1]), "+v"(don[0]), "+v"(don[1]), "+v"(oon[0]), "+v"(oon[1]), "+v"(lsen), "+v"(bn[0]), "+v"(bn[1]),
                 "+v"(padn[0]), "+v"(padn[1]), "+v"(padn[2]), "+v"(padn[3]) : : "memory");
  };
  wait_all();
  for (int b = b_begin; b < b_end; ++b, buf ^= 1) {
    __syncthreads();
    const bf16x8 qf[2] = {qn[0], qn[1]}, dof[2] = {don[0], don[1]};
    const float dl = delta_from_frags(dof, oon);
    const float nl2 = -lsen * LOG2E;
    if (active && g == 0 && q0w + t < p.S) p.delta_w[((int64_t)b * p.heads + h) * p.Spad + q0w + t] = dl;
    const int nxt = b + 1 < b_end ? b + 1 : b;
    if (has_left && prev_b >= 0 && wid == (prev_b & (PERS_NW - 1))) merge_left(prev_b, buf ^ 1);
    prev_b = b;
    const char* ldsK = smem + buf * KVB;
    const char* ldsV = ldsK + rows_pad * 128;
    f32x4 dqT[4];
#pragma unroll
    for (int db = 0; db < 4; ++db) dqT[db] = (f32x4){0.f, 0.f, 0.f, 0.f};

    auto tile = [&](const int kt, auto last_c) {
      constexpr bool LAST = decltype(last_c)::value;
      const int k0 = kt * BKV;
      if (kt > 0) {
        if (ppt_of(kt - 1) > 0) {
          if constexpr (HAS_BIAS && HAS_PAD)
            asm volatile("s_waitcnt vmcnt(%6)" : "+v"(bn[0]), "+v"(bn[1]), "+v"(padn[0]), "+v"(padn[1]), "+v"(padn[2]), "+v"(padn[3]) : "n"(BPPT));
          else if constexpr (HAS_BIAS)
            asm volatile("s_waitcnt vmcnt(%2)" : "+v"(bn[0]), "+v"(bn[1]) : "n"(BPPT));
          else if constexpr (HAS_PAD)
            asm volatile("s_waitcnt vmcnt(%4)" : "+v"(padn[0]), "+v"(padn[1]), "+v"(padn[2]), "+v"(padn[3]) : "n"(BPPT));
        } else {
          if constexpr (HAS_BIAS && HAS_PAD)
            asm volatile("s_waitcnt vmcnt(0)" : "+v"(bn[0]), "+v"(bn[1]), "+v"(padn[0]), "+v"(padn[1]), "+v"(padn[2]), "+v"(padn[3]));
          else if constexpr (HAS_BIAS)
            asm volatile("s_waitcnt vmcnt(0)" : "+v"(bn[0]), "+v"(bn[1]));
          else if constexpr (HAS_PAD)
            asm volatile("s_waitcnt vmcnt(0)" : "+v"(padn[0]), "+v"(padn[1]), "+v"(padn[2]), "+v"(padn[3]));
        }
      }
      bf16x8 bf[2];
      unsigned padw[4] = {0u, 0u, 0u, 0u};
      if constexpr (HAS_BIAS) { bf[0] = bn[0]; bf[1] = bn[1]; }
      if constexpr (HAS_PAD) {
#pragma unroll
        for (int kb = 0; kb < 4; ++kb) padw[kb] = padn[kb];
      }
      __builtin_amdgcn_sched_barrier(0);
      if constexpr (!LAST) {
        if constexpr (!LEFT) {
          if (kt == NT - 2) query_loads(nxt, vo_q, vo_o, vo_lse, qn, don, oon, lsen);
        }
        small_loads(b, kt + 1);
      } else {
        late_loads(nxt, b);
        small_loads(nxt, 0);
      }
      __builtin_amdgcn_sched_barrier(0);
#pragma unroll
      for (int jj = 0; jj < BPPT; ++jj)
        if (ppt_of(kt) > 0) piece(nxt, buf ^ 1, min(kt * BPPT + jj, npiece - 1));
      __builtin_amdgcn_sched_barrier(0);
      const char* kt_ = ldsK + k0 * 128;
      const char* vt = ldsV + k0 * 128;
      constexpr int NKB = LAST ? LASTB : 4;
      constexpr int NM = (NKB + 1) / 2;
      if (!active) return;
#pragma unroll
      for (int m = 0; m < NM; ++m) {
        f32x4 st[2], ds[2];
#pragma unroll
        for (int j = 0; j < 2; ++j) {
          const int kb = 2 * m + j;
          st[j] = (f32x4){0.f, 0.f, 0.f, 0.f};
          ds[j] = (f32x4){0.f, 0.f, 0.f, 0.f};
          if (kb >= NKB) continue;
#pragma unroll
          for (int kk = 0; kk < 2; ++kk) {
            const bf16x8 kf = *reinterpret_cast<const bf16x8*>(kt_ + (kb * 16 + t) * 128 + kswz[kk]);
            const bf16x8 vf = *reinterpret_cast<const bf16x8*>(vt + (kb * 16 + t) * 128 + kswz[kk]);
            st[j] = __builtin_amdgcn_mfma_f32_16x16x32_bf16(kf, qf[kk], st[j], 0, 0, 0);
            ds[j] = __builtin_amdgcn_mfma_f32_16x16x32_bf16(vf, dof[kk], ds[j], 0, 0, 0);
          }
          if constexpr (HAS_BIAS) st[j] = __builtin_amdgcn_mfma_f32_16x16x32_bf16(bf[m], j ? sel_hi : sel_lo, st[j], 0, 0, 0);
        }
#pragma unroll
        for (int j = 0; j < 2; ++j) {
          const int kb = 2 * m + j;
          if (kb >= NKB) continue;
          const int key = k0 + kb * 16 + g * 4;
#pragma unroll
          for (int r = 0; r < 4; ++r) {
            float x = __builtin_fmaf(st[j][r], c1, nl2);
            if constexpr (LAST || HAS_PAD) {
              bool dead = false;
              if constexpr (LAST) dead = key + r >= p.S;
              if constexpr (HAS_PAD) dead = dead || ((padw[kb] >> (8 * r)) & 0xffu);
              x = dead ? -INFINITY : x;
            }
            ds[j][r] = __builtin_amdgcn_exp2f(x) * (ds[j][r] - dl);
          }
        }
        if constexpr (HAS_BIAS) {
#pragma unroll
          for (int j = 0; j < 2; ++j)
            if (2 * m + j < NKB) acc[kt][2 * m + j] += ds[j];
        }
        float a0[4], a1[4];
#pragma unroll
        for (int r = 0; r < 4; ++r) { a0[r] = ds[0][r]; a1[r] = ds[1][r]; }
        const bf16x8 dsf = pack8(a0, a1);
        s16x4 k0r[4], k1r[4];
#pragma unroll
        for (int db = 0; db < 4; ++db) {
          k0r[db] = tr_read_a(kt_ + trsw[db] + (2 * m) * 2048);
          k1r[db] = tr_read_a(kt_ + trsw[db] + (2 * m + 1) * 2048);
        }
        ATTN_WAIT_LGKM0();
#pragma unroll
        for (int db = 0; db < 4; ++db) dqT[db] = __builtin_amdgcn_mfma_f32_16x16x32_bf16(join_tr(k0r[db], k1r[db]), dsf, dqT[db], 0, 0, 0);
      }
    };
#pragma unroll
    for (int kt = 0; kt < NT - 1; ++kt) tile(kt, std::false_type{});
    tile(NT - 1, std::true_type{});

    if (active && q0w + t < p.S) {
      bf16_t* qp = p.dq + ((int64_t)b * p.S + q0w + t) * p.ldg + h * HD;
#pragma unroll
      for (int db = 0; db < 4; ++db) {
        bf16x4 a;
#pragma unroll
        for (int r = 0; r < 4; ++r) a[r] = (bf16_t)(dqT[db][r] * p.scale);
        *reinterpret_cast<bf16x4*>(qp + db * 16 + g * 4) = a;
      }
    }
    if (has_left) {
      query_loads(nxt, vo_q, vo_o, vo_lse, qn, don, oon, lsen);
      asm volatile("s_waitcnt vmcnt(%0)" :: "n"(NSMALL + 7) : "memory");
      asm volatile("" : "+v"(ql[0]), "+v"(ql[1]), "+v"(dol[0]), "+v"(dol[1]), "+v"(ool[0]), "+v"(ool[1]), "+v"(bfl[0]), "+v"(bfl[1]), "+v"(lsel),
                   "+v"(padl[0][0]), "+v"(padl[0][1]), "+v"(padl[1][0]), "+v"(padl[1][1]));
      const float dll = delta_from_frags(dol, ool);
      const float nl2l = -lsel * LOG2E;
      if (wid == 0 && lane == 0) p.delta_w[((int64_t)b * p.heads + h) * p.Spad + p.S - 1] = dll;
      f32x4 dql[4];
#pragma unroll
      for (int db = 0; db < 4; ++db) dql[db] = (f32x4){0.f, 0.f, 0.f, 0.f};
#pragma unroll
      for (int pc = 0; pc < 2; ++pc) {
        if (pc == 1 && wid != 0) break;
        const int kp = pc == 0 ? wid : PERS_NW;
        f32x4 s4[2], d4[2];
#pragma unroll
        for (int j = 0; j < 2; ++j) {
          s4[j] = (f32x4){0.f, 0.f, 0.f, 0.f};
          d4[j] = (f32x4){0.f, 0.f, 0.f, 0.f};
#pragma unroll
          for (int kk = 0; kk < 2; ++kk) {
            const bf16x8 kf = *reinterpret_cast<const bf16x8*>(ldsK + ((2 * kp + j) * 16 + t) * 128 + kswz[kk]);
            const bf16x8 vf = *reinterpret_cast<const bf16x8*>(ldsV + ((2 * kp + j) * 16 + t) * 128 + kswz[kk]);
            s4[j] = __builtin_amdgcn_mfma_f32_16x16x32_bf16(kf, ql[kk], s4[j], 0, 0, 0);
            d4[j] = __builtin_amdgcn_mfma_f32_16x16x32_bf16(vf, dol[kk], d4[j], 0, 0, 0);
          }
          if constexpr (HAS_BIAS) s4[j] = __builtin_amdgcn_mfma_f32_16x16x32_bf16(bfl[pc], j ? sel_hi : sel_lo, s4[j], 0, 0, 0);
        }
        float a0[4], a1[4];
#pragma unroll
        for (int j = 0; j < 2; ++j)
#pragma unroll
          for (int r = 0; r < 4; ++r) {
            bool dead = (2 * kp + j) * 16 + g * 4 + r >= p.S;
            if constexpr (HAS_PAD) dead = dead || ((padl[pc][j] >> (8 * r)) & 0xffu);
            const float x = dead ? -INFINITY : __builtin_fmaf(s4[j][r], c1, nl2l);
            const float v = __builtin_amdgcn_exp2f(x) * (d4[j][r] - dll);
            d4[j][r] = v;
            (j ? a1 : a0)[r] = v;
          }
        if constexpr (HAS_BIAS) { accl[pc][0] += d4[0]; accl[pc][1] += d4[1]; }
        const bf16x8 dsf = pack8(a0, a1);
        s16x4 k0r[4], k1r[4];
#pragma unroll
        for (int db = 0; db < 4; ++db) {
          k0r[db] = tr_read_a(ldsK + trsw[db] + (2 * kp) * 2048);
          k1r[db] = tr_read_a(ldsK + trsw[db] + (2 * kp + 1) * 2048);
        }
        ATTN_WAIT_LGKM0();
#pragma unroll
        for (int db = 0; db < 4; ++db) dql[db] = __builtin_amdgcn_mfma_f32_16x16x32_bf16(join_tr(k0r[db], k1r[db]), dsf, dql[db], 0, 0, 0);
      }
      float* sc = scratch + (buf * PERS_NW + wid) * 64;
      if (t == 0) {
#pragma unroll
        for (int db = 0; db < 4; ++db) *reinterpret_cast<f32x4*>(sc + db * 16 + g * 4) = dql[db];
      }
    }

    wait_all();
  }
  if (has_left && prev_b >= 0) {
    __syncthreads();
    if (wid == 0) merge_left(prev_b, buf ^ 1);
  }
  if constexpr (HAS_BIAS) {
    if (p.dbias == nullptr) return;
    if (active && q0w + t < p.S) {
      float* drow = p.dbias + (((int64_t)chunk * p.heads + h) * p.S + q0w + t) * p.Spad + g * 4;
#pragma unroll
      for (int kt = 0; kt < NT; ++kt) {
        f32x4 cur[4];
#pragma unroll
        for (int kb = 0; kb < 4; ++kb)
          if ((kt < NT - 1 || kb < LASTB) && kt * BKV + kb * 16 < p.Spad) cur[kb] = *reinterpret_cast<const f32x4*>(drow + kt * BKV + kb * 16);
#pragma unroll
        for (int kb = 0; kb < 4; ++kb)
          if ((kt < NT - 1 || kb < LASTB) && kt * BKV + kb * 16 < p.Spad)
            *reinterpret_cast<f32x4*>(drow + kt * BKV + kb * 16) = cur[kb] + acc[kt][kb];
      }
    }
    if (has_left && t == 0) {
      float* drow = p.dbias + (((int64_t)chunk * p.heads + h) * p.S + p.S - 1) * p.Spad + g * 4;
#pragma unroll
      for (int pc = 0; pc < 2; ++pc) {
        if (pc == 1 && wid != 0) break;
        const int kp = pc == 0 ? wid : PERS_NW;
#pragma unroll
        for (int j = 0; j < 2; ++j) {
          const int key0 = (2 * kp + j) * 16;
          if (key0 < p.Spad) {
            float* d = drow + key0;
            *reinterpret_cast<f32x4*>(d) = *reinterpret_cast<const f32x4*>(d) + accl[pc][j];
          }
        }
      }
    }
  }
}

template <bool HAS_BIAS, bool HAS_PAD, int NT, int LASTB>
__global__ __launch_bounds__(PERS_NW * 64, 2) void attn_bwd_dq_pers_kernel(AttnBwdArgs p, int rows_pad, int nqh) {
  extern __shared__ __attribute__((aligned(16))) char smem[];
  const int qhalf = blockIdx.x % nqh;
  const bool lone = ((p.S + 15) >> 4) > 2 * PERS_NW && qhalf == nqh - 1;
  if constexpr (NT == 5) {
    if (lone) {
      attn_bwd_dq_pers_body<HAS_BIAS, HAS_PAD, NT, LASTB, true>(p, smem, rows_pad, nqh, qhalf);
      return;
    }
  }
  attn_bwd_dq_pers_body<HAS_BIAS, HAS_PAD, NT, LASTB, false>(p, smem, rows_pad, nqh, qhalf);
}

constexpr int PERS_SCRL = 136;

template <int OFF>
__device__ __forceinline__ void gload1_s(unsigned& d, const void* sbase, unsigned voff) {
  asm volatile("s_nop 4\n\tglobal_load_ubyte %0, %1, %2 offset:%3" : "=v"(d) : "v"(voff), "s"(sbase), "n"(OFF));
}

__device__ __forceinline__ u32x4 attn_raw_rsrc(const void* base, int nbytes) {
  const uint64_t a = (uint64_t)base;
  return (u32x4){(unsigned)__builtin_amdgcn_readfirstlane((int)(unsigned)a), (unsigned)__builtin_amdgcn_readfirstlane((int)(unsigned)(a >> 32)) & 0xffffu,
                 (unsigned)__builtin_amdgcn_readfirstlane(nbytes), 0x00020000u};
}
__device__ __forceinline__ void bstore8(const bf16x4& data, const u32x4& rsrc, unsigned voff) {
  asm volatile("s_nop 4\n\tbuffer_store_dwordx2 %0, %1, %2, 0 offen\n\ts_nop 1" ::"v"(data), "v"(voff), "s"(rsrc) : "memory");
}

template <bool HAS_BIAS, bool HAS_PAD, int NT, bool LONE>
__global__ __launch_bounds__(PERS_NW * 64, 2) void attn_bwd_dkdv_pers_kernel(AttnBwdArgs p, int rows_pad, int nitems) {
  extern __shared__ __attribute__((aligned(16))) char smem[];
  const int tid = threadIdx.x, lane = tid & 63;
  const int wid = __builtin_amdgcn_readfirstlane(tid >> 6);
  const int g = lane >> 4, t = lane & 15;
  const int QBY = rows_pad * 128;
  const int BUFB = 2 * QBY + 6144;
  float* scratch = reinterpret_cast<float*>(smem + 2 * BUFB);
  const int kbase = wid * 32;
  const bool wave_active = kbase < min(p.S, 256);
  const float c1 = p.scale * LOG2E;

  bf16x8 sel_lo, sel_hi;
  {
    const bf16_t inv = (bf16_t)(1.0f / p.scale), zero = (bf16_t)0.f;
#pragma unroll
    for (int i = 0; i < 8; ++i) {
      sel_lo[i] = (g * 8 + i == t) ? inv : zero;
      sel_hi[i] = (g * 8 + i == 16 + t) ? inv : zero;
    }
  }
  int trsw[4];
#pragma unroll
  for (int db = 0; db < 4; ++db) trsw[db] = tr_off_swz(0, db, g, t);
  const int kswz[2] = {((0 * 4 + g) ^ (t & 7)) << 4, ((1 * 4 + g) ^ (t & 7)) << 4};

  const int ngrp = rows_pad >> 3;
  const int NG = 2 * ngrp + (LONE ? 6 : 4);
  const int r_in = lane >> 3, slot = lane & 7;
  const int npiece = (NG - wid + PERS_NW - 1) / PERS_NW;
  auto piece = [&](int it, int buf, int j) {
    const int b = it / p.heads, h = it - b * p.heads;
    const int grp = wid + j * PERS_NW;
    int rl = r_in;
    asm volatile("" : "+v"(rl));
    const char* sbase;
    unsigned voff;
    int dst_off;
    if (grp < 2 * ngrp) {
      const bool isd = grp >= ngrp;
      const int gi = isd ? grp - ngrp : grp;
      const int r = gi * 8 + rl;
      const int qr = min(r, p.S - 1);
      const int ldx = isd ? (int)p.ldo : (int)p.ld;
      voff = (unsigned)((qr * ldx + ((slot ^ (r & 7)) << 3)) * 2);
      sbase = isd ? (const char*)(p.dout + (int64_t)b * p.S * p.ldo + h * HD) : (const char*)(p.q + (int64_t)b * p.S * p.ld + h * HD);
      dst_off = (isd ? QBY : 0) + gi * 1024;
    } else {
      const int e = grp - 2 * ngrp;
      if (e < 4) {
        voff = (unsigned)min((e & 1) * 1024 + (rl * 8 + slot) * 16, p.Spad * 4 - 16);
        sbase = (const char*)((e < 2 ? p.lse : p.delta) + ((int64_t)b * p.heads + h) * p.Spad);
      } else {
        voff = (unsigned)(((p.S - 1) * (int)p.ld + slot * 8) * 2);
        sbase = (const char*)((e == 4 ? p.k : p.v) + (int64_t)b * p.S * p.ld + h * HD);
      }
      dst_off = 2 * QBY + e * 1024;
    }
    __builtin_amdgcn_global_load_lds((const __attribute__((address_space(1))) void*)(sbase + voff),
                                     (__attribute__((address_space(3))) void*)(smem + buf * BUFB + dst_off), 16, 0, 0);
  };

  const int key_kb[2] = {min(kbase + t, p.S - 1), min(kbase + 16 + t, p.S - 1)};
  const unsigned vo_k[2] = {(unsigned)((key_kb[0] * (int)p.ld + g * 8) * 2), (unsigned)((key_kb[1] * (int)p.ld + g * 8) * 2)};
  bf16x8 kf[2][2], vf[2][2], kn[LONE ? 1 : 2][2], vn[LONE ? 1 : 2][2];
  unsigned kdn[2] = {0u, 0u}, kdl = 0u;
  auto kv_loads = [&](int it, bf16x8 (&kd)[2][2], bf16x8 (&vd)[2][2]) {
    const int b = it / p.heads, h = it - b * p.heads;
    const bf16_t* sk = p.k + (int64_t)b * p.S * p.ld + h * HD;
    const bf16_t* sv = p.v + (int64_t)b * p.S * p.ld + h * HD;
#pragma unroll
    for (int kb = 0; kb < 2; ++kb) {
      gload16_s<0>(kd[kb][0], sk, vo_k[kb]);
      gload16_s<64>(kd[kb][1], sk, vo_k[kb]);
      gload16_s<0>(vd[kb][0], sv, vo_k[kb]);
      gload16_s<64>(vd[kb][1], sv, vo_k[kb]);
    }
    if constexpr (HAS_PAD) {
      const uint8_t* pr = p.key_pad + (int64_t)b * p.Spad;
      gload1_s<0>(kdn[0], pr, (unsigned)key_kb[0]);
      gload1_s<0>(kdn[1], pr, (unsigned)key_kb[1]);
      if constexpr (LONE) gload1_s<0>(kdl, pr, (unsigned)(p.S - 1));
    }
  };
  constexpr int NKV = 8 + (HAS_PAD ? (LONE ? 3 : 2) : 0);
  const unsigned vo_b[2] = {(unsigned)((key_kb[0] * p.Spad + g * 8) * 2), (unsigned)((key_kb[1] * p.Spad + g * 8) * 2)};
  const unsigned vo_bl = (unsigned)(((p.S - 1) * p.Spad + g * 8) * 2);
  bf16x8 bn[2][2], bfl[2];
  auto bias_loads = [&](int it, auto qt_c, auto m_c) {
    constexpr int QT = decltype(qt_c)::value, M = decltype(m_c)::value;
    if constexpr (HAS_BIAS) {
      const int h = it % p.heads;
      const bf16_t* sb = p.biasT + (int64_t)h * p.S * p.Spad;
      gload16_s<(QT * 64 + M * 32) * 2>(bn[M][0], sb, vo_b[0]);
      gload16_s<(QT * 64 + M * 32) * 2>(bn[M][1], sb, vo_b[1]);
    }
  };
  constexpr int NBH = HAS_BIAS ? 2 : 0;
  auto lone_bias_loads = [&](int it) {
    if constexpr (HAS_BIAS && LONE) {
      const int h = it % p.heads;
      const bf16_t* sb = p.biasT + (int64_t)h * p.S * p.Spad;
      gload16_s<0>(bfl[0], sb + wid * 32, vo_bl);
      gload16_s<512>(bfl[1], sb, vo_bl);
    }
  };
  constexpr int NLB = (HAS_BIAS && LONE) ? 2 : 0;
  constexpr int BPPT = NT == 5 ? 3 : 4;

  int item = blockIdx.x;
  const int step = gridDim.x;
  using I0 = std::integral_constant<int, 0>;
  using I1 = std::integral_constant<int, 1>;
  if (item < nitems) {
    for (int j = 0; j < npiece; ++j) piece(item, 0, j);
    if constexpr (LONE) kv_loads(item, kf, vf);
    else kv_loads(item, kn, vn);
    bias_loads(item, I0{}, I0{});
    bias_loads(item, I0{}, I1{});
  }
#define DKDV_WAIT_LOADS(NST)                                                                                                                  \
  do {                                                                                                                                     \
    if constexpr (LONE)                                                                                                                    \
      asm volatile("s_waitcnt vmcnt(%15)" : "+v"(kf[0][0]), "+v"(kf[0][1]), "+v"(kf[1][0]), "+v"(kf[1][1]), "+v"(vf[0][0]), "+v"(vf[0][1]),   \
                   "+v"(vf[1][0]), "+v"(vf[1][1]), "+v"(bn[0][0]), "+v"(bn[0][1]), "+v"(bn[1][0]), "+v"(bn[1][1]), "+v"(kdn[0]), "+v"(kdn[1]), \
                   "+v"(kdl) : "n"(NST) : "memory");                                                                                      \
    else                                                                                                                                   \
      asm volatile("s_waitcnt vmcnt(%15)" : "+v"(kn[0][0]), "+v"(kn[0][1]), "+v"(kn[1][0]), "+v"(kn[1][1]), "+v"(vn[0][0]), "+v"(vn[0][1]),   \
                   "+v"(vn[1][0]), "+v"(vn[1][1]), "+v"(bn[0][0]), "+v"(bn[0][1]), "+v"(bn[1][0]), "+v"(bn[1][1]), "+v"(kdn[0]), "+v"(kdn[1]), \
                   "+v"(kdl) : "n"(NST) : "memory");                                                                                      \
  } while (0)
  DKDV_WAIT_LOADS(0);
  int buf = 0, prev_item = -1;
  auto merge_lone = [&](int it, int sb) {
    const float* sc = scratch + sb * (PERS_NW * PERS_SCRL);
    float dv = 0.f, dk = 0.f;
#pragma unroll
    for (int w = 0; w < PERS_NW; ++w) { dv += sc[w * PERS_SCRL + lane]; dk += sc[w * PERS_SCRL + 64 + lane]; }
    const bool dead = sc[128] != 0.f;
    const int b = it / p.heads, h = it - b * p.heads;
    const int64_t row = ((int64_t)b * p.S + p.S - 1) * p.ldg + h * HD + lane;
    p.dv[row] = dead ? (bf16_t)0.f : (bf16_t)dv;
    p.dk[row] = dead ? (bf16_t)0.f : (bf16_t)(dk * p.scale);
  };

  for (; item < nitems; item += step, buf ^= 1) {
    const int b = item / p.heads, h = item - b * p.heads;
    asm volatile("s_waitcnt lgkmcnt(0)" ::: "memory");
    __builtin_amdgcn_s_barrier();
    asm volatile("" ::: "memory");
    if constexpr (!LONE) {
#pragma unroll
      for (int kb = 0; kb < 2; ++kb)
#pragma unroll
        for (int kk = 0; kk < 2; ++kk) { kf[kb][kk] = kn[kb][kk]; vf[kb][kk] = vn[kb][kk]; }
    }
    const bool kdead[2] = {HAS_PAD && kdn[0] != 0u, HAS_PAD && kdn[1] != 0u};
    const bool ldead = HAS_PAD && LONE && kdl != 0u;
    const int nxt = item + step < nitems ? item + step : item;
    if (LONE && prev_item >= 0 && wid == ((prev_item / step) & (PERS_NW - 1))) merge_lone(prev_item, buf ^ 1);
    prev_item = item;
    const char* ldsQ = smem + buf * BUFB;
    const char* ldsO = ldsQ + QBY;
    const float* ldsL = reinterpret_cast<const float*>(ldsQ + 2 * QBY);
    const float* ldsD = ldsL + 512;

    f32x4 dvT[2][4], dkT[2][4];
#pragma unroll
    for (int kb = 0; kb < 2; ++kb)
#pragma unroll
      for (int db = 0; db < 4; ++db) { dvT[kb][db] = (f32x4){0.f, 0.f, 0.f, 0.f}; dkT[kb][db] = (f32x4){0.f, 0.f, 0.f, 0.f}; }

    auto half = [&](const int q0h, auto nkb_c, const bf16x8 (&kx)[2][2], const bf16x8 (&vx)[2][2], const bf16x8 (&bx)[2],
                    f32x4 (&dvx)[2][4], f32x4 (&dkx)[2][4]) {
      constexpr int NKB = decltype(nkb_c)::value;
      f32x4 s[2][NKB], dp[2][NKB];
#pragma unroll
      for (int j = 0; j < 2; ++j)
#pragma unroll
        for (int kb = 0; kb < NKB; ++kb) { s[j][kb] = (f32x4){0.f, 0.f, 0.f, 0.f}; dp[j][kb] = (f32x4){0.f, 0.f, 0.f, 0.f}; }
      const bool second = q0h + 16 < p.S;
#pragma unroll
      for (int j = 0; j < 2; ++j) {
        if (j == 1 && !second) continue;
#pragma unroll
        for (int kk = 0; kk < 2; ++kk) {
          const int off = (q0h + j * 16 + t) * 128 + kswz[kk];
          const bf16x8 qfr = *reinterpret_cast<const bf16x8*>(ldsQ + off);
          const bf16x8 ofr = *reinterpret_cast<const bf16x8*>(ldsO + off);
#pragma unroll
          for (int kb = 0; kb < NKB; ++kb) {
            s[j][kb] = __builtin_amdgcn_mfma_f32_16x16x32_bf16(qfr, kx[kb][kk], s[j][kb], 0, 0, 0);
            dp[j][kb] = __builtin_amdgcn_mfma_f32_16x16x32_bf16(ofr, vx[kb][kk], dp[j][kb], 0, 0, 0);
          }
        }
        if constexpr (HAS_BIAS) {
#pragma unroll
          for (int kb = 0; kb < NKB; ++kb) s[j][kb] = __builtin_amdgcn_mfma_f32_16x16x32_bf16(j ? sel_hi : sel_lo, bx[kb], s[j][kb], 0, 0, 0);
        }
      }
      const s16x4 zero4 = {0, 0, 0, 0};
      s16x4 o0[2], o1[2], q0r[2], q1r[2];
      auto tr_request = [&](int dh) {
#pragma unroll
        for (int i = 0; i < 2; ++i) {
          const int db = 2 * dh + i;
          o0[i] = tr_read_a(ldsO + q0h * 128 + trsw[db]);
          q0r[i] = tr_read_a(ldsQ + q0h * 128 + trsw[db]);
          o1[i] = zero4;
          q1r[i] = zero4;
          if (second) {
            o1[i] = tr_read_a(ldsO + q0h * 128 + trsw[db] + 2048);
            q1r[i] = tr_read_a(ldsQ + q0h * 128 + trsw[db] + 2048);
          }
        }
      };
      float l2[2][4], dl[2][4];
#pragma unroll
      for (int j = 0; j < 2; ++j) {
        if (j == 1 && !second) continue;
        const int qrow = q0h + j * 16 + g * 4;
        const f32x4 l4 = *reinterpret_cast<const f32x4*>(ldsL + qrow);
        const f32x4 d4 = *reinterpret_cast<const f32x4*>(ldsD + qrow);
#pragma unroll
        for (int r = 0; r < 4; ++r) {
          const bool live = qrow + r < p.S;
          l2[j][r] = live ? l4[r] * LOG2E : INFINITY;
          dl[j][r] = live ? d4[r] : 0.f;
        }
      }
      __builtin_amdgcn_sched_barrier(0);
      tr_request(0);
      __builtin_amdgcn_sched_barrier(0);
#pragma unroll
      for (int j = 0; j < 2; ++j) {
        if (j == 1 && !second) continue;
#pragma unroll
        for (int kb = 0; kb < NKB; ++kb) {
#pragma unroll
          for (int r = 0; r < 4; ++r) {
            const float pr = __builtin_amdgcn_exp2f(__builtin_fmaf(s[j][kb][r], c1, -l2[j][r]));
            s[j][kb][r] = pr;
            dp[j][kb][r] = pr * (dp[j][kb][r] - dl[j][r]);
          }
        }
      }
      bf16x8 pfr[NKB], dsf[NKB];
#pragma unroll
      for (int kb = 0; kb < NKB; ++kb) {
        float a0[4], a1[4], b0[4], b1[4];
#pragma unroll
        for (int r = 0; r < 4; ++r) {
          a0[r] = s[0][kb][r]; a1[r] = s[1][kb][r];
          b0[r] = dp[0][kb][r]; b1[r] = dp[1][kb][r];
        }
        pfr[kb] = pack8(a0, a1);
        dsf[kb] = pack8(b0, b1);
      }
#pragma unroll
      for (int dh = 0; dh < 2; ++dh) {
        if (dh == 1) tr_request(1);
        ATTN_WAIT_LGKM0();
#pragma unroll
        for (int i = 0; i < 2; ++i) {
          const int db = 2 * dh + i;
          const bf16x8 oT = join_tr(o0[i], o1[i]), qT = join_tr(q0r[i], q1r[i]);
#pragma unroll
          for (int kb = 0; kb < NKB; ++kb) {
            dvx[kb][db] = __builtin_amdgcn_mfma_f32_16x16x32_bf16(oT, pfr[kb], dvx[kb][db], 0, 0, 0);
            dkx[kb][db] = __builtin_amdgcn_mfma_f32_16x16x32_bf16(qT, dsf[kb], dkx[kb][db], 0, 0, 0);
          }
        }
      }
    };

    auto tile = [&](auto qt_c) {
      constexpr int QT = decltype(qt_c)::value;
      constexpr bool LAST = QT == NT - 1;
      using QN = std::integral_constant<int, LAST ? 0 : QT + 1>;
      if constexpr (!LAST) {
#pragma unroll
        for (int jj = 0; jj < BPPT; ++jj) piece(nxt, buf ^ 1, min(QT * BPPT + jj, npiece - 1));
      }
      __builtin_amdgcn_sched_barrier(0);
      if (wave_active) half(QT * 64, std::integral_constant<int, 2>{}, kf, vf, bn[0], dvT, dkT);
      __builtin_amdgcn_sched_barrier(0);
      if constexpr (!LAST) bias_loads(item, QN{}, I0{});
      if constexpr (HAS_BIAS && QT > 0) {
        if constexpr (!LAST) asm volatile("s_waitcnt vmcnt(%2)" : "+v"(bn[1][0]), "+v"(bn[1][1]) : "n"(BPPT + NBH));
        else asm volatile("s_waitcnt vmcnt(0)" : "+v"(bn[1][0]), "+v"(bn[1][1]));
      }
      __builtin_amdgcn_sched_barrier(0);
      if (wave_active && QT * 64 + 32 < p.S) half(QT * 64 + 32, std::integral_constant<int, 2>{}, kf, vf, bn[1], dvT, dkT);
      __builtin_amdgcn_sched_barrier(0);
      if constexpr (!LAST) {
        bias_loads(item, QN{}, I1{});
        if constexpr (HAS_BIAS) asm volatile("s_waitcnt vmcnt(%2)" : "+v"(bn[0][0]), "+v"(bn[0][1]) : "n"(NBH));
      } else {
        lone_bias_loads(item);
        bias_loads(nxt, I0{}, I0{});
        bias_loads(nxt, I0{}, I1{});
        if constexpr (!LONE) kv_loads(nxt, kn, vn);
      }
    };
    tile(std::integral_constant<int, 0>{});
    tile(std::integral_constant<int, 1>{});
    tile(std::integral_constant<int, 2>{});
    tile(std::integral_constant<int, 3>{});
    if constexpr (NT == 5) tile(std::integral_constant<int, 4>{});

    if constexpr (LONE) {
      kv_loads(nxt, kf, vf);
      if constexpr (NLB > 0) asm volatile("s_waitcnt vmcnt(%2)" : "+v"(bfl[0]), "+v"(bfl[1]) : "n"(NKV + 2 * NBH));
      const char* ldsLK = ldsQ + 2 * QBY + 4096;
      bf16x8 kl[2][2], vl[2][2];
#pragma unroll
      for (int kk = 0; kk < 2; ++kk) {
        kl[0][kk] = *reinterpret_cast<const bf16x8*>(ldsLK + (kk * 4 + g) * 16);
        vl[0][kk] = *reinterpret_cast<const bf16x8*>(ldsLK + 1024 + (kk * 4 + g) * 16);
        kl[1][kk] = kl[0][kk];
        vl[1][kk] = vl[0][kk];
      }
      f32x4 dvl[2][4], dkl[2][4];
#pragma unroll
      for (int db = 0; db < 4; ++db) { dvl[0][db] = (f32x4){0.f, 0.f, 0.f, 0.f}; dkl[0][db] = (f32x4){0.f, 0.f, 0.f, 0.f}; }
      const bf16x8 bl0[2] = {bfl[0], bfl[0]}, bl1[2] = {bfl[1], bfl[1]};
      half(wid * 32, std::integral_constant<int, 1>{}, kl, vl, bl0, dvl, dkl);
      if (wid == 0) half(256, std::integral_constant<int, 1>{}, kl, vl, bl1, dvl, dkl);
      float* sc = scratch + (buf * PERS_NW + wid) * PERS_SCRL;
      if (t == 0) {
#pragma unroll
        for (int db = 0; db < 4; ++db) {
          *reinterpret_cast<f32x4*>(sc + db * 16 + g * 4) = dvl[0][db];
          *reinterpret_cast<f32x4*>(sc + 64 + db * 16 + g * 4) = dkl[0][db];
        }
      }
      if (wid == 0 && lane == 0) sc[128] = ldead ? 1.f : 0.f;
    }

    {
      const int nrec = ((min(p.S, 256) - 1) * (int)p.ldg + HD) * 2;
      const u32x4 rk = attn_raw_rsrc(p.dk + (int64_t)b * p.S * p.ldg + h * HD, nrec);
      const u32x4 rv = attn_raw_rsrc(p.dv + (int64_t)b * p.S * p.ldg + h * HD, nrec);
#pragma unroll
      for (int kb = 0; kb < 2; ++kb) {
        const unsigned voff = (unsigned)(((kbase + kb * 16 + t) * (int)p.ldg + g * 4) * 2);
#pragma unroll
        for (int db = 0; db < 4; ++db) {
          bf16x4 a, c;
#pragma unroll
          for (int r = 0; r < 4; ++r) {
            a[r] = kdead[kb] ? (bf16_t)0.f : (bf16_t)(dkT[kb][db][r] * p.scale);
            c[r] = kdead[kb] ? (bf16_t)0.f : (bf16_t)dvT[kb][db][r];
          }
          bstore8(a, rk, voff + db * 32);
          bstore8(c, rv, voff + db * 32);
        }
      }
      DKDV_WAIT_LOADS(16);
    }
  }
  if (LONE && prev_item >= 0) {
    __syncthreads();
    if (wid == 0) merge_lone(prev_item, buf ^ 1);
  }
}

#undef DKDV_WAIT_LOADS

__global__ __launch_bounds__(256, 2) void attn_bwd_dbias_kernel(AttnBwdArgs p) {
  __shared__ __attribute__((aligned(16))) char smem[2 * 64 * 128];
  char* ldsK = smem;
  char* ldsV = smem + 64 * 128;
  const int tid = threadIdx.x, lane = tid & 63, wid = tid >> 6;
  const int g = lane >> 4, t = lane & 15;
  const int h = blockIdx.z % p.heads, chunk = blockIdx.z / p.heads;
  const int q0w = blockIdx.x * BQ + wid * 32;
  const int k0 = blockIdx.y * BKV;
  const bool wave_active = q0w < p.S;
  f32x4 acc[2][4];
  bf16x4 breg[2][4];
#pragma unroll
  for (int qb = 0; qb < 2; ++qb) {
    const int qi = min(q0w + qb * 16 + t, p.S - 1);
#pragma unroll
    for (int kb = 0; kb < 4; ++kb) {
      acc[qb][kb] = (f32x4){0.f, 0.f, 0.f, 0.f};
      if (p.bias)
        breg[qb][kb] = *reinterpret_cast<const bf16x4*>(p.bias + (int64_t)(chunk * p.bchunk) * p.bias_bs + ((int64_t)h * p.S + qi) * p.Spad +
                                                        k0 + kb * 16 + g * 4);
    }
  }
  u32x4 rk[2], rv[2];
  int st_row[2], st_c[2];
#pragma unroll
  for (int i = 0; i < 2; ++i) { const int c2 = tid + 256 * i; st_row[i] = c2 >> 3; st_c[i] = c2 & 7; }
  auto load_tile = [&](int b) {
#pragma unroll
    for (int i = 0; i < 2; ++i) {
      const int kr = min(k0 + st_row[i], p.S - 1);
      const int64_t off = ((int64_t)b * p.S + kr) * p.ld + h * HD + st_c[i] * 8;
      rk[i] = *reinterpret_cast<const u32x4*>(p.k + off);
      rv[i] = *reinterpret_cast<const u32x4*>(p.v + off);
    }
  };
  auto write_tile = [&]() {
#pragma unroll
    for (int i = 0; i < 2; ++i) {
      const int off = st_row[i] * 128 + ((st_c[i] ^ (st_row[i] & 7)) << 4);
      *reinterpret_cast<u32x4*>(ldsK + off) = rk[i];
      *reinterpret_cast<u32x4*>(ldsV + off) = rv[i];
    }
  };
  const int b_begin = chunk * p.bchunk, b_end = min(p.B, (chunk + 1) * p.bchunk);
  bf16x8 qn[2][2], on[2][2];
  float lsen[2], deln[2];
  auto load_q = [&](int b) {
    const int64_t row_base = (int64_t)b * p.S;
#pragma unroll
    for (int qb = 0; qb < 2; ++qb) {
      const int qi = min(q0w + qb * 16 + t, p.S - 1);
#pragma unroll
      for (int kk = 0; kk < 2; ++kk) {
        qn[qb][kk] = *reinterpret_cast<const bf16x8*>(p.q + (row_base + qi) * p.ld + h * HD + kk * 32 + g * 8);
        on[qb][kk] = *reinterpret_cast<const bf16x8*>(p.dout + (row_base + qi) * p.ldo + h * HD + kk * 32 + g * 8);
      }
      lsen[qb] = p.lse[((int64_t)b * p.heads + h) * p.Spad + qi];
      deln[qb] = p.delta[((int64_t)b * p.heads + h) * p.Spad + qi];
    }
  };
  if (b_begin < b_end) {
    load_tile(b_begin);
    if (wave_active) load_q(b_begin);
  }
  for (int b = b_begin; b < b_end; ++b) {
    __syncthreads();
    write_tile();
    __syncthreads();
    if (b + 1 < b_end) load_tile(b + 1);
    if (!wave_active) continue;
    bf16x8 qf[2][2], of[2][2];
    float lse[2], del[2];
#pragma unroll
    for (int qb = 0; qb < 2; ++qb) {
#pragma unroll
      for (int kk = 0; kk < 2; ++kk) { qf[qb][kk] = qn[qb][kk]; of[qb][kk] = on[qb][kk]; }
      lse[qb] = lsen[qb];
      del[qb] = deln[qb];
    }
    if (b + 1 < b_end) load_q(b + 1);
    auto kfrag = [&](int kb, int kk) {
      return *reinterpret_cast<const bf16x8*>(ldsK + (kb * 16 + t) * 128 + (((kk * 4 + g) ^ (t & 7)) << 4));
    };
    auto vfrag = [&](int kb, int kk) {
      return *reinterpret_cast<const bf16x8*>(ldsV + (kb * 16 + t) * 128 + (((kk * 4 + g) ^ (t & 7)) << 4));
    };
    auto biasfrag = [&](int qb, int kb, int, int) { return breg[qb][kb]; };
    f32x4 ds[2][4];
    ds_tile<2, true, false>(p, b, h, k0, q0w, g, t, qf, of, lse, del, kfrag, vfrag, biasfrag, [] {}, ds);
#pragma unroll
    for (int qb = 0; qb < 2; ++qb)
#pragma unroll
      for (int kb = 0; kb < 4; ++kb)
#pragma unroll
        for (int r = 0; r < 4; ++r) acc[qb][kb][r] += ds[qb][kb][r];
  }
  if (!wave_active) return;
#pragma unroll
  for (int qb = 0; qb < 2; ++qb) {
    const int qi = q0w + qb * 16 + t;
    if (qi >= p.S) continue;
#pragma unroll
    for (int kb = 0; kb < 4; ++kb) {
      float* dst = p.dbias + ((int64_t)chunk * p.heads + h) * ((int64_t)p.S * p.Spad) + (int64_t)qi * p.Spad + k0 + kb * 16 + g * 4;
      if (k0 + kb * 16 >= p.Spad) continue;
#pragma unroll
      for (int r = 0; r < 4; ++r) dst[r] += acc[qb][kb][r];
    }
  }
}


template <bool HAS_BIAS, bool HAS_PAD>
int launch_fwd_res(const AttnArgs& a, const bf16_t* frag, dim3 grid, int nw, size_t sh, int rows_pad, int qb_per_wg, int abl,
                   hipStream_t s) {
  OP_ENSURE_LDS((attn_fwd_res_kernel<HAS_BIAS, HAS_PAD>), 2 * RES_MAX_S * 128, "attn_fwd");
  hipLaunchKernelGGL((attn_fwd_res_kernel<HAS_BIAS, HAS_PAD>), grid, dim3(nw * 64), sh, s, a, frag, rows_pad, qb_per_wg, abl);
  return OP_OK;
}

template <bool HAS_BIAS, bool HAS_PAD>
int launch_fwd_pers(const AttnArgs& a, const bf16_t* frag, int nwg, size_t sh, int rows_pad, int nitems, hipStream_t s) {
  OP_ENSURE_LDS((attn_fwd_pers_kernel<HAS_BIAS, HAS_PAD>), 4 * PERS_MAX_ROWS * 128 + 2 * PERS_NW * PERS_SCR * 4, "attn_fwd");
  hipLaunchKernelGGL((attn_fwd_pers_kernel<HAS_BIAS, HAS_PAD>), dim3(nwg), dim3(PERS_NW * 64), sh, s, a, frag, rows_pad, nitems);
  return OP_OK;
}

inline int attn_num_cus() {
  static int cached[16] = {0};
  int dev = 0;
  if (hipGetDevice(&dev) != hipSuccess || dev < 0 || dev >= 16) dev = 0;
  if (cached[dev] == 0) {
    int n = 0;
    if (hipDeviceGetAttribute(&n, hipDeviceAttributeMultiprocessorCount, dev) != hipSuccess || n <= 0) n = 256;
    cached[dev] = n;
  }
  return cached[dev];
}

inline int dbias_chunks(int64_t B, int64_t S, int64_t heads, bool merge, bool round2_rule = false, int forced = 0) {
  if (!merge || ceil_div(S, BKV) > 6) return 1;
  if (forced > 0) return ceil_div(B, ceil_div(B, min((int64_t)forced, B)));
  if (round2_rule) {
    const int64_t base2 = (int64_t)ceil_div(S, 64) * heads;
    int chunks = (int)((768 + base2 - 1) / base2);
    if (chunks < 1) chunks = 1;
    if (chunks > B) chunks = (int)B;
    return ceil_div(B, ceil_div(B, chunks));
  }
  const int cus = attn_num_cus();
  const int64_t base = (int64_t)ceil_div(S, 64) * heads, slots = 2 * (int64_t)cus;
  int best = 1;
  double best_cost = 1e30;
  for (int c = 1; c <= 32 && c <= B; ++c) {
    const int bchunk = ceil_div(B, c), n = ceil_div(B, bchunk);
    if (n != c) continue;
    const double cost = (double)ceil_div(base * n, slots) * bchunk + 0.05 * n;
    if (cost < best_cost - 1e-9) { best_cost = cost; best = c; }
  }
  return best;
}

inline int sep_bchunk(int64_t B, int64_t S, int64_t heads) {
  const int64_t base = (int64_t)ceil_div(S, BQ) * ceil_div(S, BKV) * heads;
  int chunks = (int)((1024 + base - 1) / base);
  if (chunks < 1) chunks = 1;
  if (chunks > B) chunks = (int)B;
  return ceil_div(B, chunks);
}

inline int pers_bwd_chunks(int64_t B, int64_t S, int64_t heads) {
  const int nqh = ceil_div(min((int64_t)ceil_div(S, 16), (int64_t)2 * PERS_NW), PERS_NW);
  int c = (int)(attn_num_cus() / (heads * nqh));
  if (c < 1) c = 1;
  if (c > B) c = (int)B;
  return ceil_div(B, ceil_div(B, c));
}
inline bool pers_bwd_shape(int64_t S) { return S > 192 && S <= 257; }

template <bool HAS_BIAS, bool HAS_PAD>
int launch_bwd_dq_pers(const AttnBwdArgs& a, int nwg, size_t sh, int rows_pad, int nqh, hipStream_t s) {
  if (a.S > 256) {
    OP_ENSURE_LDS((attn_bwd_dq_pers_kernel<HAS_BIAS, HAS_PAD, 5, 1>), 4 * PERS_MAX_ROWS * 128 + 2 * PERS_NW * 64 * 4, "attn_bwd");
    hipLaunchKernelGGL((attn_bwd_dq_pers_kernel<HAS_BIAS, HAS_PAD, 5, 1>), dim3(nwg), dim3(PERS_NW * 64), sh, s, a, rows_pad, nqh);
  } else {
    OP_ENSURE_LDS((attn_bwd_dq_pers_kernel<HAS_BIAS, HAS_PAD, 4, 4>), 4 * PERS_MAX_ROWS * 128 + 2 * PERS_NW * 64 * 4, "attn_bwd");
    hipLaunchKernelGGL((attn_bwd_dq_pers_kernel<HAS_BIAS, HAS_PAD, 4, 4>), dim3(nwg), dim3(PERS_NW * 64), sh, s, a, rows_pad, nqh);
  }
  return OP_OK;
}

inline int dkdv_pers_rows(int64_t S) { return (int)((S + 15) / 16) * 16; }
inline size_t dkdv_pers_lds(int64_t S) { return (size_t)2 * (2 * dkdv_pers_rows(S) * 128 + 6144) + 2 * PERS_NW * PERS_SCRL * 4; }
template <bool HAS_BIAS, bool HAS_PAD>
int launch_bwd_dkdv_pers(const AttnBwdArgs& a, hipStream_t s) {
  const int rows_pad = dkdv_pers_rows(a.S);
  const size_t sh = dkdv_pers_lds(a.S);
  const int nitems = a.B * a.heads;
  const int nwg = min(nitems, attn_num_cus());
  if (a.S > 256) {
    OP_ENSURE_LDS((attn_bwd_dkdv_pers_kernel<HAS_BIAS, HAS_PAD, 5, true>), (int)dkdv_pers_lds(257), "attn_bwd");
    hipLaunchKernelGGL((attn_bwd_dkdv_pers_kernel<HAS_BIAS, HAS_PAD, 5, true>), dim3(nwg), dim3(PERS_NW * 64), sh, s, a, rows_pad, nitems);
  } else {
    OP_ENSURE_LDS((attn_bwd_dkdv_pers_kernel<HAS_BIAS, HAS_PAD, 4, false>), (int)dkdv_pers_lds(256), "attn_bwd");
    hipLaunchKernelGGL((attn_bwd_dkdv_pers_kernel<HAS_BIAS, HAS_PAD, 4, false>), dim3(nwg), dim3(PERS_NW * 64), sh, s, a, rows_pad, nitems);
  }
  return OP_OK;
}

}

extern "C" int op_prof_begin(int family, double work, void* stream);
extern "C" void op_prof_end(int slot, void* stream);

extern "C" {

int64_t op_attn_bwd_dbias_slabs(int64_t B, int64_t S, int64_t heads, int64_t tune) {
  if ((tune & 1) || ceil_div(S, BKV) > 6) return ceil_div(B, sep_bchunk(B, S, heads));
  const int64_t n = dbias_chunks(B, S, heads, !(tune & 1), (tune & 2) != 0, (int)((tune >> 4) & 63));
  if (!(tune & 1) && !(tune & 1024) && pers_bwd_shape(S)) return max(n, (int64_t)pers_bwd_chunks(B, S, heads));
  return n;
}

int op_attn_fwd(const void* q, const void* k, const void* v, int64_t ld, const void* bias, int64_t bias_batch_stride,
                const void* bias_frag, const void* key_pad, void* out, int64_t ldo, float* lse, int64_t lse_ld, int64_t B,
                int64_t S, int64_t Spad, int64_t heads, int64_t head_dim, float scale, int64_t tune, void* stream) {
  OP_CHECK_ARG(q && k && v && out, "attn_fwd: null pointer");
  OP_CHECK_ARG(head_dim == HD, "attn_fwd: head_dim %lld unsupported (only 64)", (long long)head_dim);
  OP_CHECK_ARG(B > 0 && S > 0 && heads > 0 && ld % 8 == 0 && ldo % 4 == 0, "attn_fwd: bad sizes");
  OP_CHECK_ARG((!bias && !key_pad) || (Spad >= ((S + 63) / 64) * 64 && Spad % 8 == 0),
               "attn_fwd: Spad must be >= S rounded up to 64");
  AttnArgs a;
  a.q = (const bf16_t*)q; a.k = (const bf16_t*)k; a.v = (const bf16_t*)v; a.ld = ld;
  a.bias = (const bf16_t*)bias; a.bias_bs = bias ? bias_batch_stride : 0; a.key_pad = (const uint8_t*)key_pad;
  a.out = (bf16_t*)out; a.ldo = ldo; a.lse = lse; a.lse_ld = lse_ld > 0 ? lse_ld : S;
  a.B = (int)B; a.S = (int)S; a.Spad = (int)Spad; a.heads = (int)heads; a.scale = scale;
  dim3 grid(ceil_div(S, BQ), (unsigned)heads, (unsigned)B);
  const int slot = op_prof_begin(1, 4.0 * (double)B * (double)heads * (double)S * (double)S * HD, stream);
  hipStream_t s = (hipStream_t)stream;
  const bool inv_exact = (float)(bf16_t)(1.0f / scale) * scale == 1.0f;
  if (!(tune & 1) && !(tune & 128) && S > 192 && S <= 257 && (!bias || (bias_frag && inv_exact))) {
    const int rows_pad = ceil_div(S, 32) * 32;
    const size_t sh = (size_t)4 * rows_pad * 128 + 2 * PERS_NW * PERS_SCR * 4;
    const int nitems = (int)(B * heads);
    const int nwg = min(nitems, attn_num_cus());
    const bf16_t* fr = (const bf16_t*)bias_frag;
    int rc;
    if (bias && key_pad) rc = launch_fwd_pers<true, true>(a, fr, nwg, sh, rows_pad, nitems, s);
    else if (bias) rc = launch_fwd_pers<true, false>(a, fr, nwg, sh, rows_pad, nitems, s);
    else if (key_pad) rc = launch_fwd_pers<false, true>(a, fr, nwg, sh, rows_pad, nitems, s);
    else rc = launch_fwd_pers<false, false>(a, fr, nwg, sh, rows_pad, nitems, s);
    op_prof_end(slot, stream);
    if (rc != OP_OK) return rc;
    OP_LAUNCH_CHECK();
    return OP_OK;
  }
  if (!(tune & 1) && S <= RES_MAX_S && (!bias || (bias_frag && inv_exact))) {
    const int nqb = ceil_div(S, 16);
    const int nwg = ceil_div(nqb, RES_MAX_NW);
    const int qb_per_wg = ceil_div(nqb, nwg);
    int nwaves = qb_per_wg;
    if ((tune >> 3) & 15) nwaves = min(qb_per_wg, (int)((tune >> 3) & 15));
    else if (qb_per_wg == 9) nwaves = 8;
    const int rows_pad = ceil_div(S, 32) * 32;
    const size_t sh = (size_t)2 * rows_pad * 128;
    const dim3 rgrid(nwg, (unsigned)heads, (unsigned)B);
    const int abl = (int)((tune >> 1) & 3);
    const bf16_t* fr = (const bf16_t*)bias_frag;
    int rc;
    if (bias && key_pad) rc = launch_fwd_res<true, true>(a, fr, rgrid, nwaves, sh, rows_pad, qb_per_wg, abl, s);
    else if (bias) rc = launch_fwd_res<true, false>(a, fr, rgrid, nwaves, sh, rows_pad, qb_per_wg, abl, s);
    else if (key_pad) rc = launch_fwd_res<false, true>(a, fr, rgrid, nwaves, sh, rows_pad, qb_per_wg, abl, s);
    else rc = launch_fwd_res<false, false>(a, fr, rgrid, nwaves, sh, rows_pad, qb_per_wg, abl, s);
    op_prof_end(slot, stream);
    if (rc != OP_OK) return rc;
    OP_LAUNCH_CHECK();
    return OP_OK;
  }
  if (bias && key_pad) hipLaunchKernelGGL((attn_fwd_kernel<true, true>), grid, dim3(256), 0, s, a);
  else if (bias) hipLaunchKernelGGL((attn_fwd_kernel<true, false>), grid, dim3(256), 0, s, a);
  else if (key_pad) hipLaunchKernelGGL((attn_fwd_kernel<false, true>), grid, dim3(256), 0, s, a);
  else hipLaunchKernelGGL((attn_fwd_kernel<false, false>), grid, dim3(256), 0, s, a);
  op_prof_end(slot, stream);
  OP_LAUNCH_CHECK();
  return OP_OK;
}


int64_t op_attn_bias_frag_elems(int64_t n_img, int64_t S) {
  return n_img * (int64_t)ceil_div(S, 16) * ceil_div(S, 32) * FRAG_BLOCK;
}

int op_attn_bias_pack(const void* src, void* dst, int64_t n_img, int64_t S, int64_t Spad, void* stream) {
  OP_CHECK_ARG(src && dst && n_img > 0 && S > 0 && Spad >= S, "attn_bias_pack: bad args");
  const int nqb = ceil_div(S, 16), nkp = ceil_div(S, 32);
  const int64_t total = n_img * nqb * nkp * 64;
  hipLaunchKernelGGL(bias_pack_kernel, dim3(ceil_div(total, 256)), dim3(256), 0, (hipStream_t)stream, (const bf16_t*)src,
                     (bf16_t*)dst, (int)S, (int)Spad, nqb, nkp, total);
  OP_LAUNCH_CHECK();
  return OP_OK;
}

int op_attn_bwd_delta(const void* dout, const void* out, int64_t ldo, float* delta, int64_t B, int64_t S, int64_t Spad,
                      int64_t heads, void* stream) {
  OP_CHECK_ARG(dout && out && delta && ldo % 8 == 0, "attn_bwd_delta: bad args");
  const int64_t threads = B * S * heads * 8;
  hipLaunchKernelGGL(attn_delta_kernel, dim3(ceil_div(threads, 256)), dim3(256), 0, (hipStream_t)stream, (const bf16_t*)dout,
                     (const bf16_t*)out, ldo, delta, (int)B, (int)S, (int)Spad, (int)heads);
  OP_LAUNCH_CHECK();
  return OP_OK;
}

int op_attn_bwd(const void* q, const void* k, const void* v, int64_t ld, const void* dout, const void* out, int64_t ldo, const void* bias,
                const void* biasT, const void* bias_frag, int64_t bias_batch_stride, const void* key_pad, const float* lse,
                float* delta, void* dq,
                void* dk, void* dv, int64_t ldg, float* dbias, int64_t B, int64_t S, int64_t Spad, int64_t heads,
                int64_t head_dim, float scale, int64_t tune, void* stream) {
  const bool merge_dbias = !(tune & 1);
  OP_CHECK_ARG(q && k && v && dout && lse && delta && dq && dk && dv, "attn_bwd: null pointer");
  OP_CHECK_ARG(head_dim == HD, "attn_bwd: head_dim %lld unsupported (only 64)", (long long)head_dim);
  OP_CHECK_ARG(Spad >= ((S + 127) / 128) * 128 && Spad % 8 == 0, "attn_bwd: Spad must be >= S rounded up to 128");
  OP_CHECK_ARG((bias == nullptr) == (biasT == nullptr), "attn_bwd: bias and biasT must be given together");
  OP_CHECK_ARG(!dbias || bias, "attn_bwd: dbias without a bias");
  OP_CHECK_ARG(ld % 8 == 0 && ldo % 8 == 0 && ldg % 4 == 0, "attn_bwd: bad leading dims");
  AttnBwdArgs a;
  a.q = (const bf16_t*)q; a.k = (const bf16_t*)k; a.v = (const bf16_t*)v; a.ld = ld;
  a.dout = (const bf16_t*)dout; a.ldo = ldo; a.bias = (const bf16_t*)bias; a.biasT = (const bf16_t*)biasT;
  a.bias_frag = bias ? (const bf16_t*)bias_frag : nullptr;
  a.bias_bs = bias ? bias_batch_stride : 0;
  a.key_pad = (const uint8_t*)key_pad; a.lse = lse; a.delta = delta; a.out = (const bf16_t*)out; a.delta_w = delta;
  a.dq = (bf16_t*)dq; a.dk = (bf16_t*)dk; a.dv = (bf16_t*)dv; a.ldg = ldg; a.dbias = dbias;
  a.B = (int)B; a.S = (int)S; a.Spad = (int)Spad; a.heads = (int)heads; a.scale = scale;
  a.lone_keys = !(tune & 2048);
  a.bchunk = sep_bchunk(B, S, heads);
  hipStream_t s = (hipStream_t)stream;
  const double fl = 4.0 * (double)B * (double)heads * (double)S * (double)S * HD;
  int slot;
  const int bchunk_dkdv = a.bchunk;
  auto launch_dkdv = [&]() {
    AttnBwdArgs d = a;
    d.bchunk = bchunk_dkdv;
    const int sl = op_prof_begin(2, 2.0 * fl, stream);
    const bool kb1 = ((tune >> 2) & 3) == 2;
    if (kb1) {
      if (bias) hipLaunchKernelGGL((attn_bwd_dkdv_kernel<true, 1>), dim3(ceil_div(S, 64), (unsigned)heads, (unsigned)B), dim3(256), 0, s, d);
      else hipLaunchKernelGGL((attn_bwd_dkdv_kernel<false, 1>), dim3(ceil_div(S, 64), (unsigned)heads, (unsigned)B), dim3(256), 0, s, d);
    } else {
      if (bias) hipLaunchKernelGGL((attn_bwd_dkdv_kernel<true, 2>), dim3(ceil_div(S, 128), (unsigned)heads, (unsigned)B), dim3(256), 0, s, d);
      else hipLaunchKernelGGL((attn_bwd_dkdv_kernel<false, 2>), dim3(ceil_div(S, 128), (unsigned)heads, (unsigned)B), dim3(256), 0, s, d);
    }
    op_prof_end(sl, stream);
  };
  if (!out) {
    launch_dkdv();
    OP_LAUNCH_CHECK();
  }
  const int nt = ceil_div(S, BKV);
  if (merge_dbias && !(tune & 1024) && out && pers_bwd_shape(S) && a.bias_bs == 0 &&
      (!bias || (a.bias_frag != nullptr && (float)(bf16_t)(1.0f / scale) * scale == 1.0f))) {
    const int nqb = ceil_div(S, 16);
    const int nqh = ceil_div(min(nqb, 2 * PERS_NW), PERS_NW);
    const int chunks = pers_bwd_chunks(B, S, heads);
    a.bchunk = ceil_div(B, chunks);
    const int rows_pad = S > 256 ? PERS_MAX_ROWS : 256;
    const size_t sh = (size_t)4 * rows_pad * 128 + 2 * PERS_NW * 64 * 4;
    const int nwg = chunks * (int)heads * nqh;
    AttnBwdArgs d = a;
    if (!bias) d.dbias = nullptr;
    slot = op_prof_begin(2, 1.5 * fl, stream);
    int rc;
    if (bias && key_pad) rc = launch_bwd_dq_pers<true, true>(d, nwg, sh, rows_pad, nqh, s);
    else if (bias) rc = launch_bwd_dq_pers<true, false>(d, nwg, sh, rows_pad, nqh, s);
    else if (key_pad) rc = launch_bwd_dq_pers<false, true>(d, nwg, sh, rows_pad, nqh, s);
    else rc = launch_bwd_dq_pers<false, false>(d, nwg, sh, rows_pad, nqh, s);
    op_prof_end(slot, stream);
    if (rc != OP_OK) return rc;
    OP_LAUNCH_CHECK();
    a.bchunk = bchunk_dkdv;
    if (!(tune & 4096) && (!bias || biasT) && (S != 256 || (tune & 8192))) {
      const int sl = op_prof_begin(2, 2.0 * fl, stream);
      if (bias && key_pad) rc = launch_bwd_dkdv_pers<true, true>(a, s);
      else if (bias) rc = launch_bwd_dkdv_pers<true, false>(a, s);
      else if (key_pad) rc = launch_bwd_dkdv_pers<false, true>(a, s);
      else rc = launch_bwd_dkdv_pers<false, false>(a, s);
      op_prof_end(sl, stream);
      if (rc != OP_OK) return rc;
    } else {
      launch_dkdv();
    }
    OP_LAUNCH_CHECK();
    return OP_OK;
  }
  if (dbias && nt <= 6 && merge_dbias) {
    const int chunks = a.bias_bs != 0 ? (int)B : dbias_chunks(B, S, heads, true, (tune & 2) != 0, (int)((tune >> 4) & 63));
    a.bchunk = ceil_div(B, chunks);
    const dim3 grid(ceil_div(S, 64), (unsigned)heads, (unsigned)chunks);
    const bool one_block = ceil_div(S - (nt - 1) * BKV, 16) == 1;
    const bool frag = a.bias_frag != nullptr && (float)(bf16_t)(1.0f / scale) * scale == 1.0f && (nt <= 4 || (nt == 5 && one_block));
#define DQDB(N)                                                                                                           \
  do {                                                                                                                    \
    if (frag && one_block) hipLaunchKernelGGL((attn_bwd_dq_dbias_kernel<N, true, 1>), grid, dim3(256), 0, s, a);           \
    else if (frag) hipLaunchKernelGGL((attn_bwd_dq_dbias_kernel<N, true, 4>), grid, dim3(256), 0, s, a);                   \
    else if (one_block) hipLaunchKernelGGL((attn_bwd_dq_dbias_kernel<N, false, 1>), grid, dim3(256), 0, s, a);             \
    else hipLaunchKernelGGL((attn_bwd_dq_dbias_kernel<N, false, 4>), grid, dim3(256), 0, s, a);                            \
  } while (0)
    slot = op_prof_begin(2, 1.5 * fl, stream);
    switch (nt) {
      case 1: DQDB(1); break;
      case 2: DQDB(2); break;
      case 3: DQDB(3); break;
      case 4: DQDB(4); break;
      case 5: DQDB(5); break;
      default: DQDB(6); break;
    }
#undef DQDB
    op_prof_end(slot, stream);
    OP_LAUNCH_CHECK();
    if (out) {
      launch_dkdv();
      OP_LAUNCH_CHECK();
    }
    return OP_OK;
  }
  slot = op_prof_begin(2, 1.5 * fl, stream);
  if (bias) hipLaunchKernelGGL(attn_bwd_dq_kernel<true>, dim3(ceil_div(S, BQ), (unsigned)heads, (unsigned)B), dim3(256), 0, s, a);
  else hipLaunchKernelGGL(attn_bwd_dq_kernel<false>, dim3(ceil_div(S, BQ), (unsigned)heads, (unsigned)B), dim3(256), 0, s, a);
  op_prof_end(slot, stream);
  OP_LAUNCH_CHECK();
  if (out) {
    launch_dkdv();
    OP_LAUNCH_CHECK();
  }
  if (dbias) {
    if (a.bias_bs != 0) a.bchunk = 1;
    const int chunks = ceil_div(B, a.bchunk);
    hipLaunchKernelGGL(attn_bwd_dbias_kernel, dim3(ceil_div(S, BQ), ceil_div(S, BKV), (unsigned)(heads * chunks)), dim3(256), 0,
                       s, a);
    OP_LAUNCH_CHECK();
  }
  return OP_OK;
}

}
```

Before: 187.7.

## Cut register pressure in persistent attention kernels via rematerialized kernargs and scalar offsets

New measurement: 188.5 (median of 6 runs). About the same (+0.5%).

```diff
diff --git a/one-peace_amd/csrc/attention.hip b/one-peace_amd/csrc/attention.hip
--- a/one-peace_amd/csrc/attention.hip
+++ b/one-peace_amd/csrc/attention.hip
@@ -472,6 +472,42 @@
   asm volatile("s_nop 4\n\tglobal_load_dword %0, %1, %2 offset:%3" : "=v"(d) : "v"(voff), "s"(sbase), "n"(OFF));
 }
 
+__device__ __forceinline__ int lane_fresh(int v) {
+  asm volatile("" : "+v"(v));
+  return v;
+}
+__device__ __forceinline__ int wave_fresh(int v) {
+  v = __builtin_amdgcn_readfirstlane(v);
+  asm volatile("" : "+s"(v));
+  return v;
+}
+template <typename A>
+__device__ __forceinline__ const A __attribute__((address_space(4)))* kernarg_fresh() {
+  auto* ka = __builtin_amdgcn_kernarg_segment_ptr();
+  asm volatile("" : "+s"(ka));
+  return (const A __attribute__((address_space(4)))*)ka;
+}
+template <int R>
+__device__ __forceinline__ void mask_pad2(f32x4& a, f32x4& b, unsigned w, float ninf) {
+  unsigned tmp;
+  float s0 = a[R], s1 = b[R];
+  asm("v_and_b32 %2, %4, %3\n\tv_cmp_ne_u32 vcc, 0, %2\n\tv_cndmask_b32 %0, %0, %5, vcc\n\tv_cndmask_b32 %1, %1, %5, vcc"
+      : "+v"(s0), "+v"(s1), "=&v"(tmp) : "v"(w), "n"(0xffu << (8 * R)), "v"(ninf) : "vcc");
+  a[R] = s0;
+  b[R] = s1;
+}
+static_assert(sizeof(AttnArgs) % 8 == 0, "the argument behind AttnArgs starts right behind it (kernarg_fresh)");
+__device__ __forceinline__ void gload16x2_s(bf16x8& d0, bf16x8& d1, const void* s0, const void* s1, unsigned voff) {
+  asm volatile("s_nop 4\n\tglobal_load_dwordx4 %0, %2, %3\n\tglobal_load_dwordx4 %1, %2, %4" : "=&v"(d0), "=&v"(d1) : "v"(voff), "s"(s0), "s"(s1));
+}
+__device__ __forceinline__ void gload16x2_i(bf16x8& d0, bf16x8& d1, const void* s0, unsigned voff) {
+  asm volatile("s_nop 4\n\tglobal_load_dwordx4 %0, %2, %3\n\tglobal_load_dwordx4 %1, %2, %3 offset:64" : "=&v"(d0), "=&v"(d1) : "v"(voff), "s"(s0));
+}
+__device__ __forceinline__ void gload4x4_s(unsigned (&d)[4], const void* s0, unsigned voff) {
+  asm volatile("s_nop 4\n\tglobal_load_dword %0, %4, %5\n\tglobal_load_dword %1, %4, %5 offset:16\n\tglobal_load_dword %2, %4, %5 offset:32\n\t"
+               "global_load_dword %3, %4, %5 offset:48" : "=&v"(d[0]), "=&v"(d[1]), "=&v"(d[2]), "=&v"(d[3]) : "v"(voff), "s"(s0));
+}
+
 template <bool HAS_BIAS, bool HAS_PAD>
 __global__ __launch_bounds__(PERS_NW * 64, 2) void attn_fwd_pers_kernel(AttnArgs p, const bf16_t* __restrict__ bias_frag, int rows_pad,
                                                                          int nitems) {
@@ -479,14 +515,16 @@
   const int tid = threadIdx.x, lane = tid & 63;
   const int wid = __builtin_amdgcn_readfirstlane(tid >> 6);
   const int g = lane >> 4, t = lane & 15;
+  const int S = p.S, heads = p.heads;
+  const unsigned ldb = (unsigned)p.ld * 2u;
   const int KVB = 2 * rows_pad * 128;
   float* scratch = reinterpret_cast<float*>(smem + 2 * KVB);
-  const int nqb = (p.S + 15) >> 4, nkp = (p.S + 31) >> 5;
-  const bool has_left = nqb > 2 * PERS_NW;
+  const int nqb = (S + 15) >> 4, nkp = (S + 31) >> 5;
+  const int has_left_ = wave_fresh(nqb > 2 * PERS_NW);
   const int q0 = wid * 32;
-  const int nact = min(2, max(0, nqb - 2 * wid));
-  const int64_t per_head = (int64_t)nqb * nkp * FRAG_BLOCK;
-  const int ntiles = (p.S + BKV - 1) / BKV;
+  const int nact_ = min(2, max(0, nqb - 2 * wid));
+  const unsigned qb_bytes = (unsigned)nkp * (FRAG_BLOCK * 2);
+  const int ntiles = (S + BKV - 1) / BKV;
   const float c1 = p.scale * LOG2E;
 
   bf16x8 sel_lo, sel_hi;
@@ -503,78 +541,62 @@
   for (int db = 0; db < 4; ++db) trsw[db] = tr_off_swz(0, db, g, t);
   const int kswz[2] = {((0 * 4 + g) ^ (t & 7)) << 4, ((1 * 4 + g) ^ (t & 7)) << 4};
 
+  auto qkv_off = [&](int b, int h) { return (int64_t)(b * S) * ldb + h * (HD * 2); };
+  auto bias_ptr = [&](const char* frag, bool per_sample, int b, int h) {
+    return frag + (int64_t)((per_sample ? b * heads : 0) + h) * ((int64_t)nqb * qb_bytes);
+  };
+  auto pad_ptr = [&](const uint8_t* key_pad, int Spad, int b) { return reinterpret_cast<const char*>(key_pad) + (int64_t)b * Spad; };
+  const unsigned g4 = g * 4, g16 = g * 16, l16 = lane * 16;
+  const unsigned qvoff[2] = {(unsigned)min(q0 + t, S - 1) * ldb + g16, (unsigned)min(q0 + 16 + t, S - 1) * ldb + g16};
+  const unsigned bvoff[2] = {(unsigned)min(2 * wid, nqb - 1) * qb_bytes + l16, (unsigned)min(2 * wid + 1, nqb - 1) * qb_bytes + l16};
+
   const int ngrp = rows_pad >> 3;
-  const int r_in = lane >> 3, slot = lane & 7;
+  const int r_in = lane >> 3;
+  const unsigned pswz = ((lane & 7) ^ r_in) << 4;
   const int npiece = (2 * ngrp - wid + PERS_NW - 1) / PERS_NW;
-  auto piece = [&](int it, int buf, int j) {
-    const int b = it / p.heads, h = it - b * p.heads;
+  auto piece = [&](const char* kb_, const char* vb_, int buf, int j) {
     const int grp = wid + j * PERS_NW;
     const bool isv = grp >= ngrp;
     const int gi = isv ? grp - ngrp : grp;
-    const int r = gi * 8 + r_in;
-    const int kr = min(r, p.S - 1);
-    const bf16_t* src = (isv ? p.v : p.k) + ((int64_t)b * p.S + kr) * p.ld + h * HD + ((slot ^ (r & 7)) << 3);
-    char* dst = smem + buf * KVB + (isv ? rows_pad * 128 : 0) + gi * 1024;
+    const unsigned voff = __umul24((unsigned)min(gi * 8 + r_in, S - 1), ldb) + pswz;
+    const char* src = (isv ? vb_ : kb_) + voff;
+    char* dst = smem + buf * KVB + grp * 1024;
     __builtin_amdgcn_global_load_lds((const __attribute__((address_space(1))) void*)src,
                                      (__attribute__((address_space(3))) void*)dst, 16, 0, 0);
   };
-  auto load_q = [&](int it, int qrow, bf16x8 (&q)[2]) {
-    const int b = it / p.heads, h = it - b * p.heads;
-    const bf16_t* qp = p.q + ((int64_t)b * p.S + qrow) * p.ld + h * HD;
-#pragma unroll
-    for (int kk = 0; kk < 2; ++kk) q[kk] = *reinterpret_cast<const bf16x8*>(qp + kk * 32 + g * 8);
-  };
-  const int qi_main[2] = {min(q0 + t, p.S - 1), min(q0 + 16 + t, p.S - 1)};
 
   bf16x8 bn[2][2];
   unsigned padn[4] = {0u, 0u, 0u, 0u};
-  auto small_loads = [&](int it, int kt) {
-    const int b = it / p.heads, h = it - b * p.heads;
+  auto small_loads = [&](const char* bias_it, const char* pad_it, int kt) {
     if constexpr (HAS_BIAS) {
-      const bf16_t* fhead = bias_frag + ((p.bias_bs != 0 ? (int64_t)b * p.heads : 0) + h) * per_head + lane * 8;
-#pragma unroll
-      for (int qb = 0; qb < 2; ++qb) {
-        const bf16_t* fb = fhead + (int64_t)min(2 * wid + qb, nqb - 1) * nkp * FRAG_BLOCK;
-#pragma unroll
-        for (int m = 0; m < 2; ++m) gload16_asm(bn[qb][m], fb + min(2 * kt + m, nkp - 1) * FRAG_BLOCK);
-      }
-    }
-    if constexpr (HAS_PAD) {
-      const uint8_t* pr = p.key_pad + (int64_t)b * p.Spad + g * 4 + kt * BKV;
-#pragma unroll
-      for (int kb = 0; kb < 4; ++kb) gload4_asm(padn[kb], pr + kb * 16);
-    }
+      const char* s0 = bias_it + kt * (2 * FRAG_BLOCK * 2);
+      const char* s1 = bias_it + min(2 * kt + 1, nkp - 1) * (FRAG_BLOCK * 2);
+#pragma unroll
+      for (int qb = 0; qb < 2; ++qb) gload16x2_s(bn[qb][0], bn[qb][1], s0, s1, bvoff[qb]);
+    }
+    if constexpr (HAS_PAD) gload4x4_s(padn, pad_it + kt * BKV, g4);
   };
 
   constexpr int NSMALL = (HAS_BIAS ? 4 : 0) + (HAS_PAD ? 4 : 0);
   bf16x8 qn[2][2], ql[2], bfl[2];
   unsigned padl[2][2] = {{0u, 0u}, {0u, 0u}};
-  auto late_loads = [&](int it_next, int it) {
-    {
-      const int b = it_next / p.heads, h = it_next - b * p.heads;
-#pragma unroll
-      for (int qb = 0; qb < 2; ++qb) {
-        const bf16_t* qp = p.q + ((int64_t)b * p.S + qi_main[qb]) * p.ld + h * HD;
-#pragma unroll
-        for (int kk = 0; kk < 2; ++kk) gload16_asm(qn[qb][kk], qp + kk * 32 + g * 8);
-      }
-    }
-    if (has_left) {
-      const int b = it / p.heads, h = it - b * p.heads;
-      const bf16_t* qp = p.q + ((int64_t)b * p.S + p.S - 1) * p.ld + h * HD;
-#pragma unroll
-      for (int kk = 0; kk < 2; ++kk) gload16_asm(ql[kk], qp + kk * 32 + g * 8);
+  auto load_q = [&](const char* q_it) {
+#pragma unroll
+    for (int qb = 0; qb < 2; ++qb) gload16x2_i(qn[qb][0], qn[qb][1], q_it, qvoff[qb]);
+  };
+  auto late_loads = [&](const char* q_next, int b, int h, const char* bias_it, const char* pad_it) {
+    load_q(q_next);
+    if (wave_fresh(has_left_)) {
+      gload16x2_i(ql[0], ql[1], reinterpret_cast<const char*>(kernarg_fresh<AttnArgs>()->q) + qkv_off(b, h) + (unsigned)(S - 1) * ldb, g16);
       if constexpr (HAS_BIAS) {
-        const bf16_t* fleft = bias_frag + ((p.bias_bs != 0 ? (int64_t)b * p.heads : 0) + h) * per_head + lane * 8 + (int64_t)(nqb - 1) * nkp * FRAG_BLOCK;
-        gload16_asm(bfl[0], fleft + wid * FRAG_BLOCK);
-        gload16_asm(bfl[1], fleft + min(PERS_NW, nkp - 1) * FRAG_BLOCK);
+        const char* fleft = bias_it + (unsigned)(nqb - 1) * qb_bytes;
+        gload16x2_s(bfl[0], bfl[1], fleft + wid * (FRAG_BLOCK * 2), fleft + min(PERS_NW, nkp - 1) * (FRAG_BLOCK * 2), l16);
       }
       if constexpr (HAS_PAD) {
-        const uint8_t* pr = p.key_pad + (int64_t)b * p.Spad + g * 4;
 #pragma unroll
         for (int j = 0; j < 2; ++j) {
-          gload4_asm(padl[0][j], pr + (2 * wid + j) * 16);
-          gload4_asm(padl[1][j], pr + min((2 * PERS_NW + j) * 16, p.Spad - 16));
+          gload4_s<0>(padl[0][j], pad_it + (2 * wid + j) * 16, g4);
+          gload4_s<0>(padl[1][j], pad_it + min((2 * PERS_NW + j) * 16, kernarg_fresh<AttnArgs>()->Spad - 16), g4);
         }
       }
     }
@@ -582,20 +604,21 @@
 
   int item = blockIdx.x;
   const int step = gridDim.x;
+  int b = item / heads, h = item - b * heads;
   if (item < nitems) {
-    for (int j = 0; j < npiece; ++j) piece(item, 0, j);
-    load_q(item, qi_main[0], qn[0]);
-    load_q(item, qi_main[1], qn[1]);
-    small_loads(item, 0);
-  }
-  int buf = 0, prev_item = -1;
+    const int64_t o = qkv_off(b, h);
+    for (int j = 0; j < npiece; ++j) piece(reinterpret_cast<const char*>(p.k) + o, reinterpret_cast<const char*>(p.v) + o, 0, j);
+    load_q(reinterpret_cast<const char*>(p.q) + o);
+    small_loads(bias_ptr(reinterpret_cast<const char*>(bias_frag), p.bias_bs != 0, b, h), pad_ptr(p.key_pad, p.Spad, b), 0);
+  }
+  int buf = 0, trip = 0, pb = 0, ph = 0;
   auto wait_all = [&]() {
     asm volatile("s_waitcnt vmcnt(0)" : "+v"(qn[0][0]), "+v"(qn[0][1]), "+v"(qn[1][0]), "+v"(qn[1][1]), "+v"(bn[0][0]), "+v"(bn[0][1]), "+v"(bn[1][0]), "+v"(bn[1][1]),
                  "+v"(padn[0]), "+v"(padn[1]), "+v"(padn[2]), "+v"(padn[3]) : : "memory");
   };
   wait_all();
 
-  auto merge_left = [&](int it, int sb) {
+  auto merge_left = [&](int b_, int h_, int sb) {
     const float* sc = scratch + sb * (PERS_NW * PERS_SCR);
     float M = -INFINITY;
 #pragma unroll
@@ -607,21 +630,34 @@
       L = __builtin_fmaf(sc[w * PERS_SCR + 65], f, L);
       o = __builtin_fmaf(sc[w * PERS_SCR + lane], f, o);
     }
-    const int b = it / p.heads, h = it - b * p.heads;
-    const int qrow = p.S - 1;
-    p.out[((int64_t)b * p.S + qrow) * p.ldo + h * HD + lane] = (bf16_t)(o / L);
-    if (lane == 0 && p.lse) p.lse[((int64_t)b * p.heads + h) * p.lse_ld + qrow] = M * (1.0f / LOG2E) + logf(L);
-  };
-
-  for (; item < nitems; item += step, buf ^= 1) {
-    const int b = item / p.heads, h = item - b * p.heads;
-    const int64_t row_base = (int64_t)b * p.S;
+    const int qrow = S - 1;
+    const auto* pa = kernarg_fresh<AttnArgs>();
+    float* const lse = pa->lse;
+    pa->out[((int64_t)b_ * S + qrow) * pa->ldo + h_ * HD + lane] = (bf16_t)(o / L);
+    if (lane_fresh(lane) == 0 && lse) lse[((int64_t)b_ * heads + h_) * pa->lse_ld + qrow] = M * (1.0f / LOG2E) + logf(L);
+  };
+
+  for (; item < nitems; item += step, buf ^= 1, ++trip) {
+    const bool has_left = wave_fresh(has_left_) != 0;
+    const int nact = wave_fresh(nact_);
     __syncthreads();
     bf16x8 qf[2][2] = {{qn[0][0], qn[0][1]}, {qn[1][0], qn[1][1]}};
     const bool more = item + step < nitems;
     const int nxt = more ? item + step : item;
-    if (has_left && prev_item >= 0 && wid == ((prev_item / step) & (PERS_NW - 1))) merge_left(prev_item, buf ^ 1);
-    prev_item = item;
+    if (has_left && trip > 0 && wid == ((trip - 1) & (PERS_NW - 1))) merge_left(pb, ph, buf ^ 1);
+    const int bn_ = nxt / heads, hn_ = nxt - bn_ * heads;
+    const auto* pi = kernarg_fresh<AttnArgs>();
+    const int64_t off_n = qkv_off(bn_, hn_);
+    const char* const k_nxt = reinterpret_cast<const char*>(pi->k) + off_n;
+    const char* const v_nxt = reinterpret_cast<const char*>(pi->v) + off_n;
+    const char* const q_nxt = reinterpret_cast<const char*>(pi->q) + off_n;
+    const char* const frag = *reinterpret_cast<const char* const __attribute__((address_space(4)))*>(
+        reinterpret_cast<const char __attribute__((address_space(4)))*>(pi) + sizeof(AttnArgs));
+    const bool per_sample = pi->bias_bs != 0;
+    const char* const bias_it = HAS_BIAS ? bias_ptr(frag, per_sample, b, h) : nullptr;
+    const char* const bias_nxt = HAS_BIAS ? bias_ptr(frag, per_sample, bn_, hn_) : nullptr;
+    const char* const pad_it = HAS_PAD ? pad_ptr(pi->key_pad, pi->Spad, b) : nullptr;
+    const char* const pad_nxt = HAS_PAD ? pad_ptr(pi->key_pad, pi->Spad, bn_) : nullptr;
 
     const char* ldsK = smem + buf * KVB;
     const char* ldsV = ldsK + rows_pad * 128;
@@ -636,7 +672,7 @@
     auto tile = [&](const int kt, auto full_c) {
       constexpr bool FULL = decltype(full_c)::value;
       const int k0 = kt * BKV;
-      const int nkb = FULL ? 4 : ((p.S - k0 + 15) >> 4);
+      const int nkb = FULL ? 4 : wave_fresh((S - k0 + 15) >> 4);
       bf16x8 bf[2][2];
       unsigned padw[4] = {0u, 0u, 0u, 0u};
       if constexpr (HAS_BIAS) {
@@ -651,14 +687,14 @@
       }
       __builtin_amdgcn_sched_barrier(0);
       if constexpr (FULL) {
-        small_loads(item, kt + 1);
+        small_loads(bias_it, pad_it, kt + 1);
       } else {
-        late_loads(nxt, item);
-        small_loads(nxt, 0);
+        late_loads(q_nxt, b, h, bias_it, pad_it);
+        small_loads(bias_nxt, pad_nxt, 0);
       }
       __builtin_amdgcn_sched_barrier(0);
 #pragma unroll
-      for (int jj = 0; jj < PERS_PPT; ++jj) piece(nxt, buf ^ 1, min(kt * PERS_PPT + jj, npiece - 1));
+      for (int jj = 0; jj < PERS_PPT; ++jj) piece(k_nxt, v_nxt, buf ^ 1, min(kt * PERS_PPT + jj, npiece - 1));
       __builtin_amdgcn_sched_barrier(0);
       if (nact == 0) return;
 
@@ -691,23 +727,40 @@
         va1[db] = tr_read_a(vt + trsw[db] + 2048);
       }
       bf16x8 pf[2][2];
+      if constexpr (!FULL || HAS_PAD) {
+        const int lim = FULL ? 0 : lane_fresh(S - k0 - (int)g4);
+        float ninf = -INFINITY;
+        if constexpr (HAS_PAD) {
+          asm volatile("s_nop 7\n\ts_nop 3" : "+v"(ninf), "+v"(st[0][0]), "+v"(st[0][1]), "+v"(st[0][2]), "+v"(st[0][3]), "+v"(st[1][0]), "+v"(st[1][1]),
+                       "+v"(st[1][2]), "+v"(st[1][3]));
+        }
+#pragma unroll
+        for (int kb = 0; kb < 4; ++kb) {
+          if (!FULL && kb >= nkb) break;
+          if constexpr (!FULL) {
+#pragma unroll
+            for (int r = 0; r < 4; ++r) {
+              const bool masked = kb * 16 + r >= lim;
+#pragma unroll
+              for (int qb = 0; qb < 2; ++qb) st[qb][kb][r] = masked ? -INFINITY : st[qb][kb][r];
+            }
+          }
+          if constexpr (HAS_PAD) {
+            mask_pad2<0>(st[0][kb], st[1][kb], padw[kb], ninf);
+            mask_pad2<1>(st[0][kb], st[1][kb], padw[kb], ninf);
+            mask_pad2<2>(st[0][kb], st[1][kb], padw[kb], ninf);
+            mask_pad2<3>(st[0][kb], st[1][kb], padw[kb], ninf);
+          }
+        }
+      }
 #pragma unroll
       for (int qb = 0; qb < 2; ++qb) {
         float mx = -INFINITY;
 #pragma unroll
         for (int kb = 0; kb < 4; ++kb) {
           if (!FULL && kb >= nkb) break;
-          const int key = k0 + kb * 16 + g * 4;
-#pragma unroll
-          for (int r = 0; r < 4; ++r) {
-            if constexpr (!FULL || HAS_PAD) {
-              bool masked = false;
-              if constexpr (!FULL) masked = key + r >= p.S;
-              if constexpr (HAS_PAD) masked = masked || ((padw[kb] >> (8 * r)) & 0xffu);
-              st[qb][kb][r] = masked ? -INFINITY : st[qb][kb][r];
-            }
-            mx = fmaxf(mx, st[qb][kb][r]);
-          }
+#pragma unroll
+          for (int r = 0; r < 4; ++r) mx = fmaxf(mx, st[qb][kb][r]);
         }
         mx = fmaxf(mx, __shfl_xor(mx, 16));
         mx = fmaxf(mx, __shfl_xor(mx, 32));
@@ -732,10 +785,12 @@
           }
         }
         l_run[qb] = l_run[qb] * alpha + psum;
-#pragma unroll
-        for (int db = 0; db < 4; ++db)
-#pragma unroll
-          for (int r = 0; r < 4; ++r) ot[qb][db][r] *= alpha;
+        if (__builtin_amdgcn_ballot_w64(alpha != 1.0f) != 0) {
+#pragma unroll
+          for (int db = 0; db < 4; ++db)
+#pragma unroll
+            for (int r = 0; r < 4; ++r) asm("v_mul_f32 %0, %0, %1" : "+v"(ot[qb][db][r]) : "v"(alpha));
+        }
         pf[qb][0] = pack8(pv[0], pv[1]);
         pf[qb][1] = pack8(pv[2], pv[3]);
       }
@@ -788,6 +843,7 @@
       const int npc = wid == 0 ? 2 : 1;
       for (int pc = 0; pc < npc; ++pc) {
         const int kp = pc == 0 ? wid : PERS_NW;
+        const int liml = lane_fresh(S - kp * 32 - (int)g4);
         f32x4 s4[2];
         const unsigned padw[2] = {padl[pc][0], padl[pc][1]};
 #pragma unroll
@@ -805,7 +861,7 @@
         for (int j = 0; j < 2; ++j)
 #pragma unroll
           for (int r = 0; r < 4; ++r) {
-            bool masked = (2 * kp + j) * 16 + g * 4 + r >= p.S;
+            bool masked = j * 16 + r >= liml;
             if constexpr (HAS_PAD) masked = masked || ((padw[j] >> (8 * r)) & 0xffu);
             s4[j][r] = masked ? -INFINITY : s4[j][r];
             mx = fmaxf(mx, s4[j][r]);
@@ -844,36 +900,42 @@
       lsum += __shfl_xor(lsum, 16);
       lsum += __shfl_xor(lsum, 32);
       float* sc = scratch + (buf * PERS_NW + wid) * PERS_SCR;
-      if (t == 0) {
+      const int ll = lane_fresh(lane);
+      if ((ll & 15) == 0) {
 #pragma unroll
         for (int db = 0; db < 4; ++db) *reinterpret_cast<f32x4*>(sc + db * 16 + g * 4) = ol[db];
-        if (g == 0) { sc[64] = m2; sc[65] = lsum; }
-      }
-    }
+        if (ll == 0) { sc[64] = m2; sc[65] = lsum; }
+      }
+    }
+    const auto* pa = kernarg_fresh<AttnArgs>();
+    const unsigned ldob = (unsigned)pa->ldo * 2u;
+    float* const lse = pa->lse;
 #pragma unroll
     for (int qb = 0; qb < 2; ++qb) {
       float l = l_run[qb];
       l += __shfl_xor(l, 16);
       l += __shfl_xor(l, 32);
-      const int qrow = q0 + qb * 16 + t;
-      if (qb < nact && qrow < p.S) {
+      const int qrow = lane_fresh(q0 + qb * 16 + t);
+      if (qb < nact && qrow < S) {
         const float inv = 1.f / l;
-        bf16_t* op = p.out + (row_base + qrow) * p.ldo + h * HD;
+        char* op = reinterpret_cast<char*>(pa->out) + ((int64_t)(b * S) * ldob + h * (HD * 2)) + ((unsigned)qrow * ldob + g * 8);
 #pragma unroll
         for (int db = 0; db < 4; ++db) {
           bf16x4 o;
 #pragma unroll
           for (int r = 0; r < 4; ++r) o[r] = (bf16_t)(ot[qb][db][r] * inv);
-          *reinterpret_cast<bf16x4*>(op + db * 16 + g * 4) = o;
-        }
-        if (g == 0 && p.lse) p.lse[((int64_t)b * p.heads + h) * p.lse_ld + qrow] = m2_run[qb] * (1.0f / LOG2E) + logf(l);
-      }
-    }
+          *reinterpret_cast<bf16x4*>(op + db * 32) = o;
+        }
+        if (lane_fresh(lane) < 16 && lse) lse[((int64_t)b * heads + h) * pa->lse_ld + qrow] = m2_run[qb] * (1.0f / LOG2E) + logf(l);
+      }
+    }
+    pb = b, ph = h;
+    b = bn_, h = hn_;
     wait_all();
   }
-  if (has_left && prev_item >= 0) {
+  if (has_left_ && wave_fresh(trip) > 0) {
     __syncthreads();
-    if (wid == 0) merge_left(prev_item, buf ^ 1);
+    if (wid == 0) merge_left(pb, ph, buf ^ 1);
   }
 }
 
@@ -917,6 +979,7 @@
   float scale;
   int lone_keys;
 };
+static_assert(sizeof(AttnBwdArgs) % 8 == 0, "the arguments behind AttnBwdArgs start right behind it (kernarg_fresh)");
 
 __global__ __launch_bounds__(256) void attn_delta_kernel(const bf16_t* __restrict__ dout, const bf16_t* __restrict__ out,
                                                          int64_t ldo, float* __restrict__ delta, int B, int S, int Spad,
@@ -1602,7 +1665,7 @@
   const int wid = __builtin_amdgcn_readfirstlane(tid >> 6);
   const int g = lane >> 4, t = lane & 15;
   const int KVB = 2 * rows_pad * 128;
-  float* scratch = reinterpret_cast<float*>(smem + 2 * KVB);
+  auto scratch_ = [&]() { return reinterpret_cast<float*>(smem + 4 * wave_fresh(rows_pad) * 128); };
   const int nqb = (p.S + 15) >> 4, nkp = (p.S + 31) >> 5;
   const int qhalf = qhalf0, h = (blockIdx.x / nqh) % p.heads, chunk = blockIdx.x / (nqh * p.heads);
   const int b_begin = chunk * p.bchunk, b_end = min(p.B, b_begin + p.bchunk);
@@ -1613,7 +1676,8 @@
   const int q0w = min(qblk, nqb - 1) * 16;
   const int qi = min(q0w + t, p.S - 1);
   const float c1 = p.scale * LOG2E;
-  const int64_t per_head = (int64_t)nqb * nkp * FRAG_BLOCK;
+  const int per_head = nqb * nkp * FRAG_BLOCK;
+  const int ld_ = (int)p.ld, ldo_ = (int)p.ldo;
 
   bf16x8 sel_lo, sel_hi;
   {
@@ -1632,16 +1696,17 @@
   const int ngrp = rows_pad >> 3;
   const int r_in = lane >> 3, slot = lane & 7;
   const int npiece = (2 * ngrp - wid + PERS_NW - 1) / PERS_NW;
-  auto piece = [&](int b, int buf, int j) {
-    const int grp = wid + j * PERS_NW;
+  auto piece = [&](const bf16_t* kb_, const bf16_t* vb_, int w_, int rows_pad, int buf, int j) {
+    const int ngrp = rows_pad >> 3, KVB = 2 * rows_pad * 128;
+    const int grp = w_ + j * PERS_NW;
     const bool isv = grp >= ngrp;
     const int gi = isv ? grp - ngrp : grp;
     int rl = r_in;
     asm volatile("" : "+v"(rl));
     const int r = gi * 8 + rl;
     const int kr = min(r, p.S - 1);
-    const unsigned voff = (unsigned)((kr * (int)p.ld + ((slot ^ (r & 7)) << 3)) * 2);
-    const char* sbase = (const char*)((isv ? p.v : p.k) + (int64_t)b * p.S * p.ld + h * HD);
+    const unsigned voff = __umul24((unsigned)kr, (unsigned)ld_ * 2u) + (unsigned)((slot ^ (r & 7)) << 4);
+    const char* sbase = (const char*)(isv ? vb_ : kb_);
     char* dst = smem + buf * KVB + (isv ? rows_pad * 128 : 0) + gi * 1024;
     __builtin_amdgcn_global_load_lds((const __attribute__((address_space(1))) void*)(sbase + voff),
                                      (__attribute__((address_space(3))) void*)dst, 16, 0, 0);
@@ -1653,18 +1718,18 @@
   const bf16_t* fwave = HAS_BIAS ? p.bias_frag + (int64_t)h * per_head + (int64_t)(q0w >> 4) * nkp * FRAG_BLOCK : nullptr;
   const bf16_t* fleft = HAS_BIAS ? p.bias_frag + (int64_t)h * per_head + (int64_t)(nqb - 1) * nkp * FRAG_BLOCK : nullptr;
   const unsigned vo_frag = lane * 16, vo_pad = g * 4;
-  const unsigned vo_q = (unsigned)(((int64_t)qi * p.ld + h * HD + g * 8) * 2), vo_o = (unsigned)(((int64_t)qi * p.ldo + h * HD + g * 8) * 2);
-  const unsigned vo_ql = (unsigned)(((int64_t)(p.S - 1) * p.ld + h * HD + g * 8) * 2), vo_ol = (unsigned)(((int64_t)(p.S - 1) * p.ldo + h * HD + g * 8) * 2);
+  const unsigned vo_q = (unsigned)(((int64_t)qi * ld_ + h * HD + g * 8) * 2), vo_o = (unsigned)(((int64_t)qi * ldo_ + h * HD + g * 8) * 2);
+  const unsigned vo_ql = (unsigned)(((int64_t)(p.S - 1) * ld_ + h * HD + g * 8) * 2), vo_ol = (unsigned)(((int64_t)(p.S - 1) * ldo_ + h * HD + g * 8) * 2);
   const unsigned vo_lse = qi * 4, vo_lsel = (p.S - 1) * 4;
   bf16x8 bn[2];
   unsigned padn[4] = {0u, 0u, 0u, 0u};
-  auto small_loads = [&](int b, int kt) {
+  auto small_loads = [&](const bf16_t* fw, int nkp_, const uint8_t* pad_b, int kt) {
     if constexpr (HAS_BIAS) {
-      gload16_s<0>(bn[0], fwave + min(2 * kt, nkp - 1) * FRAG_BLOCK, vo_frag);
-      gload16_s<0>(bn[1], fwave + min(2 * kt + 1, nkp - 1) * FRAG_BLOCK, vo_frag);
+      gload16_s<0>(bn[0], fw + min(2 * kt, nkp_ - 1) * FRAG_BLOCK, vo_frag);
+      gload16_s<0>(bn[1], fw + min(2 * kt + 1, nkp_ - 1) * FRAG_BLOCK, vo_frag);
     }
     if constexpr (HAS_PAD) {
-      const uint8_t* pr = p.key_pad + (int64_t)b * p.Spad + kt * BKV;
+      const uint8_t* pr = pad_b + kt * BKV;
       gload4_s<0>(padn[0], pr, vo_pad);
       gload4_s<16>(padn[1], pr, vo_pad);
       gload4_s<32>(padn[2], pr, vo_pad);
@@ -1675,9 +1740,10 @@
   float lsen, lsel;
   unsigned padl[2][2] = {{0u, 0u}, {0u, 0u}};
   auto query_loads = [&](int b, unsigned voq, unsigned voo, unsigned vol, bf16x8 (&q)[2], bf16x8 (&d)[2], bf16x8 (&o)[2], float& l) {
-    const bf16_t* sq = p.q + (int64_t)b * p.S * p.ld;
-    const bf16_t* sd = p.dout + (int64_t)b * p.S * p.ldo;
-    const bf16_t* so = p.out + (int64_t)b * p.S * p.ldo;
+    const auto* pa = kernarg_fresh<AttnBwdArgs>();
+    const bf16_t* sq = pa->q + (int64_t)b * p.S * ld_;
+    const bf16_t* sd = pa->dout + (int64_t)b * p.S * ldo_;
+    const bf16_t* so = pa->out + (int64_t)b * p.S * ldo_;
     gload16_s<0>(q[0], sq, voq);
     gload16_s<64>(q[1], sq, voq);
     gload16_s<0>(d[0], sd, voo);
@@ -1685,21 +1751,19 @@
     gload16_s<0>(o[0], so, voo);
     gload16_s<64>(o[1], so, voo);
     unsigned lw;
-    gload4_s<0>(lw, p.lse + ((int64_t)b * p.heads + h) * p.Spad, vol);
+    gload4_s<0>(lw, pa->lse + ((int64_t)b * p.heads + h) * p.Spad, vol);
     l = __builtin_bit_cast(float, lw);
   };
-  auto late_loads = [&](int b_next, int b) {
-    (void)b_next;
+  auto late_loads = [&](int b, const bf16_t* fl, int nkp_, const uint8_t* pr, int w_) {
     if (has_left) {
       query_loads(b, vo_ql, vo_ol, vo_lsel, ql, dol, ool, lsel);
       if constexpr (HAS_BIAS) {
-        gload16_s<0>(bfl[0], fleft + wid * FRAG_BLOCK, vo_frag);
-        gload16_s<0>(bfl[1], fleft + min(PERS_NW, nkp - 1) * FRAG_BLOCK, vo_frag);
+        gload16_s<0>(bfl[0], fl + w_ * FRAG_BLOCK, vo_frag);
+        gload16_s<0>(bfl[1], fl + min(PERS_NW, nkp_ - 1) * FRAG_BLOCK, vo_frag);
       }
       if constexpr (HAS_PAD) {
-        const uint8_t* pr = p.key_pad + (int64_t)b * p.Spad;
-        gload4_s<0>(padl[0][0], pr + 2 * wid * 16, vo_pad);
-        gload4_s<16>(padl[0][1], pr + 2 * wid * 16, vo_pad);
+        gload4_s<0>(padl[0][0], pr + 2 * w_ * 16, vo_pad);
+        gload4_s<16>(padl[0][1], pr + 2 * w_ * 16, vo_pad);
         gload4_s<0>(padl[1][0], pr + min(2 * PERS_NW * 16, p.Spad - 32), vo_pad);
         gload4_s<16>(padl[1][1], pr + min(2 * PERS_NW * 16, p.Spad - 32), vo_pad);
       }
@@ -1716,16 +1780,17 @@
 #pragma unroll
     for (int j = 0; j < 2; ++j) accl[i][j] = (f32x4){0.f, 0.f, 0.f, 0.f};
 
-  for (int j = 0; j < npiece; ++j) piece(b_begin, 0, j);
+  for (int j = 0; j < npiece; ++j) piece(p.k + (int64_t)b_begin * p.S * ld_ + h * HD, p.v + (int64_t)b_begin * p.S * ld_ + h * HD, wid, rows_pad, 0, j);
   query_loads(b_begin, vo_q, vo_o, vo_lse, qn, don, oon, lsen);
-  small_loads(b_begin, 0);
-  int buf = 0, prev_b = -1;
+  small_loads(fwave, nkp, p.key_pad + (int64_t)b_begin * p.Spad, 0);
+  int buf = 0;
   auto merge_left = [&](int b, int sb) {
-    const float* sc = scratch + sb * (PERS_NW * 64);
+    const float* sc = scratch_() + sb * (PERS_NW * 64);
     float o = 0.f;
 #pragma unroll
     for (int w = 0; w < PERS_NW; ++w) o += sc[w * 64 + lane];
-    p.dq[((int64_t)b * p.S + p.S - 1) * p.ldg + h * HD + lane] = (bf16_t)(o * p.scale);
+    const auto* pa = kernarg_fresh<AttnBwdArgs>();
+    pa->dq[((int64_t)b * p.S + p.S - 1) * pa->ldg + h * HD + lane] = (bf16_t)(o * pa->scale);
   };
 
   auto wait_all = [&]() {
@@ -1738,12 +1803,19 @@
     const bf16x8 qf[2] = {qn[0], qn[1]}, dof[2] = {don[0], don[1]};
     const float dl = delta_from_frags(dof, oon);
     const float nl2 = -lsen * LOG2E;
-    if (active && g == 0 && q0w + t < p.S) p.delta_w[((int64_t)b * p.heads + h) * p.Spad + q0w + t] = dl;
+    const auto* pa = kernarg_fresh<AttnBwdArgs>();
+    const int w_ = wave_fresh(wid), nkp_ = wave_fresh(nkp), rp_ = wave_fresh(rows_pad);
+    const int np_ = (2 * (rp_ >> 3) - w_ + PERS_NW - 1) / PERS_NW;
+    const int tq = lane_fresh(q0w + t);
+    if (active && lane_fresh(lane) < 16 && tq < p.S) pa->delta_w[((int64_t)b * p.heads + h) * p.Spad + tq] = dl;
     const int nxt = b + 1 < b_end ? b + 1 : b;
-    if (has_left && prev_b >= 0 && wid == (prev_b & (PERS_NW - 1))) merge_left(prev_b, buf ^ 1);
-    prev_b = b;
-    const char* ldsK = smem + buf * KVB;
-    const char* ldsV = ldsK + rows_pad * 128;
+    const bf16_t* const k_nxt = pa->k + (int64_t)nxt * p.S * ld_ + h * HD;
+    const bf16_t* const v_nxt = pa->v + (int64_t)nxt * p.S * ld_ + h * HD;
+    const bf16_t* const fw = HAS_BIAS ? pa->bias_frag + (int64_t)h * per_head + (int64_t)wave_fresh(q0w >> 4) * nkp_ * FRAG_BLOCK : nullptr;
+    const uint8_t* const pad_b = HAS_PAD ? pa->key_pad + (int64_t)b * p.Spad : nullptr;
+    if (has_left && b > b_begin && wid == ((b - 1) & (PERS_NW - 1))) merge_left(b - 1, buf ^ 1);
+    const char* ldsK = smem + buf * (2 * rp_ * 128);
+    const char* ldsV = ldsK + rp_ * 128;
     f32x4 dqT[4];
 #pragma unroll
     for (int db = 0; db < 4; ++db) dqT[db] = (f32x4){0.f, 0.f, 0.f, 0.f};
@@ -1780,15 +1852,15 @@
         if constexpr (!LEFT) {
           if (kt == NT - 2) query_loads(nxt, vo_q, vo_o, vo_lse, qn, don, oon, lsen);
         }
-        small_loads(b, kt + 1);
+        small_loads(fw, nkp_, pad_b, kt + 1);
       } else {
-        late_loads(nxt, b);
-        small_loads(nxt, 0);
+        late_loads(b, HAS_BIAS ? fw + (nqb - 1 - wave_fresh(q0w >> 4)) * nkp_ * FRAG_BLOCK : nullptr, nkp_, pad_b, w_);
+        small_loads(fw, nkp_, HAS_PAD ? pad_b + (nxt - b) * p.Spad : nullptr, 0);
       }
       __builtin_amdgcn_sched_barrier(0);
 #pragma unroll
       for (int jj = 0; jj < BPPT; ++jj)
-        if (ppt_of(kt) > 0) piece(nxt, buf ^ 1, min(kt * BPPT + jj, npiece - 1));
+        if (ppt_of(kt) > 0) piece(k_nxt, v_nxt, w_, rp_, buf ^ 1, min(kt * BPPT + jj, np_ - 1));
       __builtin_amdgcn_sched_barrier(0);
       const char* kt_ = ldsK + k0 * 128;
       const char* vt = ldsV + k0 * 128;
@@ -1817,13 +1889,13 @@
         for (int j = 0; j < 2; ++j) {
           const int kb = 2 * m + j;
           if (kb >= NKB) continue;
-          const int key = k0 + kb * 16 + g * 4;
+          const int lim = LAST ? lane_fresh(p.S - k0 - g * 4) : 0;
 #pragma unroll
           for (int r = 0; r < 4; ++r) {
             float x = __builtin_fmaf(st[j][r], c1, nl2);
             if constexpr (LAST || HAS_PAD) {
               bool dead = false;
-              if constexpr (LAST) dead = key + r >= p.S;
+              if constexpr (LAST) dead = kb * 16 + r >= lim;
               if constexpr (HAS_PAD) dead = dead || ((padw[kb] >> (8 * r)) & 0xffu);
               x = dead ? -INFINITY : x;
             }
@@ -1854,13 +1926,15 @@
     for (int kt = 0; kt < NT - 1; ++kt) tile(kt, std::false_type{});
     tile(NT - 1, std::true_type{});
 
-    if (active && q0w + t < p.S) {
-      bf16_t* qp = p.dq + ((int64_t)b * p.S + q0w + t) * p.ldg + h * HD;
+    if (active && tq < p.S) {
+      const auto* pq = kernarg_fresh<AttnBwdArgs>();
+      const float scale = pq->scale;
+      bf16_t* qp = pq->dq + ((int64_t)b * p.S + tq) * pq->ldg + h * HD;
 #pragma unroll
       for (int db = 0; db < 4; ++db) {
         bf16x4 a;
 #pragma unroll
-        for (int r = 0; r < 4; ++r) a[r] = (bf16_t)(dqT[db][r] * p.scale);
+        for (int r = 0; r < 4; ++r) a[r] = (bf16_t)(dqT[db][r] * scale);
         *reinterpret_cast<bf16x4*>(qp + db * 16 + g * 4) = a;
       }
     }
@@ -1871,14 +1945,15 @@
                    "+v"(padl[0][0]), "+v"(padl[0][1]), "+v"(padl[1][0]), "+v"(padl[1][1]));
       const float dll = delta_from_frags(dol, ool);
       const float nl2l = -lsel * LOG2E;
-      if (wid == 0 && lane == 0) p.delta_w[((int64_t)b * p.heads + h) * p.Spad + p.S - 1] = dll;
+      if (wid == 0 && lane_fresh(lane) == 0) kernarg_fresh<AttnBwdArgs>()->delta_w[((int64_t)b * p.heads + h) * p.Spad + wave_fresh(p.S - 1)] = dll;
       f32x4 dql[4];
 #pragma unroll
       for (int db = 0; db < 4; ++db) dql[db] = (f32x4){0.f, 0.f, 0.f, 0.f};
 #pragma unroll
       for (int pc = 0; pc < 2; ++pc) {
         if (pc == 1 && wid != 0) break;
-        const int kp = pc == 0 ? wid : PERS_NW;
+        const int kp = pc == 0 ? w_ : PERS_NW;
+        const int liml = lane_fresh(p.S - kp * 32 - g * 4);
         f32x4 s4[2], d4[2];
 #pragma unroll
         for (int j = 0; j < 2; ++j) {
@@ -1898,7 +1973,7 @@
         for (int j = 0; j < 2; ++j)
 #pragma unroll
           for (int r = 0; r < 4; ++r) {
-            bool dead = (2 * kp + j) * 16 + g * 4 + r >= p.S;
+            bool dead = j * 16 + r >= liml;
             if constexpr (HAS_PAD) dead = dead || ((padl[pc][j] >> (8 * r)) & 0xffu);
             const float x = dead ? -INFINITY : __builtin_fmaf(s4[j][r], c1, nl2l);
             const float v = __builtin_amdgcn_exp2f(x) * (d4[j][r] - dll);
@@ -1917,8 +1992,8 @@
 #pragma unroll
         for (int db = 0; db < 4; ++db) dql[db] = __builtin_amdgcn_mfma_f32_16x16x32_bf16(join_tr(k0r[db], k1r[db]), dsf, dql[db], 0, 0, 0);
       }
-      float* sc = scratch + (buf * PERS_NW + wid) * 64;
-      if (t == 0) {
+      float* sc = scratch_() + (buf * PERS_NW + wid) * 64;
+      if ((lane_fresh(lane) & 15) == 0) {
 #pragma unroll
         for (int db = 0; db < 4; ++db) *reinterpret_cast<f32x4*>(sc + db * 16 + g * 4) = dql[db];
       }
@@ -1926,28 +2001,34 @@
 
     wait_all();
   }
-  if (has_left && prev_b >= 0) {
+  if (has_left) {
     __syncthreads();
-    if (wid == 0) merge_left(prev_b, buf ^ 1);
+    if (wid == 0) merge_left(b_end - 1, buf ^ 1);
   }
   if constexpr (HAS_BIAS) {
-    if (p.dbias == nullptr) return;
-    if (active && q0w + t < p.S) {
-      float* drow = p.dbias + (((int64_t)chunk * p.heads + h) * p.S + q0w + t) * p.Spad + g * 4;
+    const auto* pe = kernarg_fresh<AttnBwdArgs>();
+    float* const dbias = pe->dbias;
+    if (dbias == nullptr) return;
+    const int S_ = pe->S, Spad_ = pe->Spad, heads_ = pe->heads;
+    const int nqh_ = *reinterpret_cast<const int __attribute__((address_space(4)))*>(reinterpret_cast<const char __attribute__((address_space(4)))*>(pe) +
+                                                                                    sizeof(AttnBwdArgs) + sizeof(int));
+    const int chunk_ = blockIdx.x / (nqh_ * heads_);
+    if (active && lane_fresh(q0w + t) < S_) {
+      float* drow = dbias + (((int64_t)chunk_ * heads_ + h) * S_ + q0w + t) * Spad_ + g * 4;
 #pragma unroll
       for (int kt = 0; kt < NT; ++kt) {
         f32x4 cur[4];
 #pragma unroll
         for (int kb = 0; kb < 4; ++kb)
-          if ((kt < NT - 1 || kb < LASTB) && kt * BKV + kb * 16 < p.Spad) cur[kb] = *reinterpret_cast<const f32x4*>(drow + kt * BKV + kb * 16);
+          if ((kt < NT - 1 || kb < LASTB) && kt * BKV + kb * 16 < Spad_) cur[kb] = *reinterpret_cast<const f32x4*>(drow + kt * BKV + kb * 16);
 #pragma unroll
         for (int kb = 0; kb < 4; ++kb)
-          if ((kt < NT - 1 || kb < LASTB) && kt * BKV + kb * 16 < p.Spad)
+          if ((kt < NT - 1 || kb < LASTB) && kt * BKV + kb * 16 < Spad_)
             *reinterpret_cast<f32x4*>(drow + kt * BKV + kb * 16) = cur[kb] + acc[kt][kb];
       }
     }
-    if (has_left && t == 0) {
-      float* drow = p.dbias + (((int64_t)chunk * p.heads + h) * p.S + p.S - 1) * p.Spad + g * 4;
+    if (has_left && (lane_fresh(lane) & 15) == 0) {
+      float* drow = dbias + (((int64_t)chunk_ * heads_ + h) * S_ + S_ - 1) * Spad_ + g * 4;
 #pragma unroll
       for (int pc = 0; pc < 2; ++pc) {
         if (pc == 1 && wid != 0) break;
@@ -1955,7 +2036,7 @@
 #pragma unroll
         for (int j = 0; j < 2; ++j) {
           const int key0 = (2 * kp + j) * 16;
-          if (key0 < p.Spad) {
+          if (key0 < Spad_) {
             float* d = drow + key0;
             *reinterpret_cast<f32x4*>(d) = *reinterpret_cast<const f32x4*>(d) + accl[pc][j];
           }
@@ -2005,7 +2086,6 @@
   const int BUFB = 2 * QBY + 6144;
   float* scratch = reinterpret_cast<float*>(smem + 2 * BUFB);
   const int kbase = wid * 32;
-  const bool wave_active = kbase < min(p.S, 256);
   const float c1 = p.scale * LOG2E;
 
   bf16x8 sel_lo, sel_hi;
@@ -2026,9 +2106,9 @@
   const int NG = 2 * ngrp + (LONE ? 6 : 4);
   const int r_in = lane >> 3, slot = lane & 7;
   const int npiece = (NG - wid + PERS_NW - 1) / PERS_NW;
-  auto piece = [&](int it, int buf, int j) {
-    const int b = it / p.heads, h = it - b * p.heads;
-    const int grp = wid + j * PERS_NW;
+  auto piece = [&](int b, int h, int buf, int j) {
+    const auto* pa = kernarg_fresh<AttnBwdArgs>();
+    const int grp = wave_fresh(wid) + j * PERS_NW;
     int rl = r_in;
     asm volatile("" : "+v"(rl));
     const char* sbase;
@@ -2040,17 +2120,17 @@
       const int r = gi * 8 + rl;
       const int qr = min(r, p.S - 1);
       const int ldx = isd ? (int)p.ldo : (int)p.ld;
-      voff = (unsigned)((qr * ldx + ((slot ^ (r & 7)) << 3)) * 2);
-      sbase = isd ? (const char*)(p.dout + (int64_t)b * p.S * p.ldo + h * HD) : (const char*)(p.q + (int64_t)b * p.S * p.ld + h * HD);
+      voff = __umul24((unsigned)qr, (unsigned)ldx * 2u) + (unsigned)((slot ^ (r & 7)) << 4);
+      sbase = isd ? (const char*)(pa->dout + (int64_t)b * p.S * p.ldo + h * HD) : (const char*)(pa->q + (int64_t)b * p.S * p.ld + h * HD);
       dst_off = (isd ? QBY : 0) + gi * 1024;
     } else {
       const int e = grp - 2 * ngrp;
       if (e < 4) {
         voff = (unsigned)min((e & 1) * 1024 + (rl * 8 + slot) * 16, p.Spad * 4 - 16);
-        sbase = (const char*)((e < 2 ? p.lse : p.delta) + ((int64_t)b * p.heads + h) * p.Spad);
+        sbase = (const char*)((e < 2 ? pa->lse : pa->delta) + ((int64_t)b * p.heads + h) * p.Spad);
       } else {
         voff = (unsigned)(((p.S - 1) * (int)p.ld + slot * 8) * 2);
-        sbase = (const char*)((e == 4 ? p.k : p.v) + (int64_t)b * p.S * p.ld + h * HD);
+        sbase = (const char*)((e == 4 ? pa->k : pa->v) + (int64_t)b * p.S * p.ld + h * HD);
       }
       dst_off = 2 * QBY + e * 1024;
     }
@@ -2062,10 +2142,10 @@
   const unsigned vo_k[2] = {(unsigned)((key_kb[0] * (int)p.ld + g * 8) * 2), (unsigned)((key_kb[1] * (int)p.ld + g * 8) * 2)};
   bf16x8 kf[2][2], vf[2][2], kn[LONE ? 1 : 2][2], vn[LONE ? 1 : 2][2];
   unsigned kdn[2] = {0u, 0u}, kdl = 0u;
-  auto kv_loads = [&](int it, bf16x8 (&kd)[2][2], bf16x8 (&vd)[2][2]) {
-    const int b = it / p.heads, h = it - b * p.heads;
-    const bf16_t* sk = p.k + (int64_t)b * p.S * p.ld + h * HD;
-    const bf16_t* sv = p.v + (int64_t)b * p.S * p.ld + h * HD;
+  auto kv_loads = [&](int b, int h, bf16x8 (&kd)[2][2], bf16x8 (&vd)[2][2]) {
+    const auto* pa = kernarg_fresh<AttnBwdArgs>();
+    const bf16_t* sk = pa->k + (int64_t)b * p.S * p.ld + h * HD;
+    const bf16_t* sv = pa->v + (int64_t)b * p.S * p.ld + h * HD;
 #pragma unroll
     for (int kb = 0; kb < 2; ++kb) {
       gload16_s<0>(kd[kb][0], sk, vo_k[kb]);
@@ -2074,7 +2154,7 @@
       gload16_s<64>(vd[kb][1], sv, vo_k[kb]);
     }
     if constexpr (HAS_PAD) {
-      const uint8_t* pr = p.key_pad + (int64_t)b * p.Spad;
+      const uint8_t* pr = pa->key_pad + (int64_t)b * p.Spad;
       gload1_s<0>(kdn[0], pr, (unsigned)key_kb[0]);
       gload1_s<0>(kdn[1], pr, (unsigned)key_kb[1]);
       if constexpr (LONE) gload1_s<0>(kdl, pr, (unsigned)(p.S - 1));
@@ -2084,21 +2164,18 @@
   const unsigned vo_b[2] = {(unsigned)((key_kb[0] * p.Spad + g * 8) * 2), (unsigned)((key_kb[1] * p.Spad + g * 8) * 2)};
   const unsigned vo_bl = (unsigned)(((p.S - 1) * p.Spad + g * 8) * 2);
   bf16x8 bn[2][2], bfl[2];
-  auto bias_loads = [&](int it, auto qt_c, auto m_c) {
+  auto biasT_of = [&](const bf16_t* biasT, int h) { return biasT + (int64_t)h * p.S * p.Spad; };
+  auto bias_loads = [&](const bf16_t* sb, auto qt_c, auto m_c) {
     constexpr int QT = decltype(qt_c)::value, M = decltype(m_c)::value;
     if constexpr (HAS_BIAS) {
-      const int h = it % p.heads;
-      const bf16_t* sb = p.biasT + (int64_t)h * p.S * p.Spad;
       gload16_s<(QT * 64 + M * 32) * 2>(bn[M][0], sb, vo_b[0]);
       gload16_s<(QT * 64 + M * 32) * 2>(bn[M][1], sb, vo_b[1]);
     }
   };
   constexpr int NBH = HAS_BIAS ? 2 : 0;
-  auto lone_bias_loads = [&](int it) {
+  auto lone_bias_loads = [&](const bf16_t* sb) {
     if constexpr (HAS_BIAS && LONE) {
-      const int h = it % p.heads;
-      const bf16_t* sb = p.biasT + (int64_t)h * p.S * p.Spad;
-      gload16_s<0>(bfl[0], sb + wid * 32, vo_bl);
+      gload16_s<0>(bfl[0], sb + wave_fresh(wid) * 32, vo_bl);
       gload16_s<512>(bfl[1], sb, vo_bl);
     }
   };
@@ -2109,12 +2186,13 @@
   const int step = gridDim.x;
   using I0 = std::integral_constant<int, 0>;
   using I1 = std::integral_constant<int, 1>;
+  int b = item / p.heads, h = item - b * p.heads;
   if (item < nitems) {
-    for (int j = 0; j < npiece; ++j) piece(item, 0, j);
-    if constexpr (LONE) kv_loads(item, kf, vf);
-    else kv_loads(item, kn, vn);
-    bias_loads(item, I0{}, I0{});
-    bias_loads(item, I0{}, I1{});
+    for (int j = 0; j < npiece; ++j) piece(b, h, 0, j);
+    if constexpr (LONE) kv_loads(b, h, kf, vf);
+    else kv_loads(b, h, kn, vn);
+    bias_loads(biasT_of(p.biasT, h), I0{}, I0{});
+    bias_loads(biasT_of(p.biasT, h), I0{}, I1{});
   }
 #define DKDV_WAIT_LOADS(NST)                                                                                                                  \
   do {                                                                                                                                     \
@@ -2128,21 +2206,20 @@
                    "+v"(kdl) : "n"(NST) : "memory");                                                                                      \
   } while (0)
   DKDV_WAIT_LOADS(0);
-  int buf = 0, prev_item = -1;
-  auto merge_lone = [&](int it, int sb) {
+  int buf = 0, trip = 0, pb = 0, ph = 0;
+  auto merge_lone = [&](int b, int h, int sb) {
     const float* sc = scratch + sb * (PERS_NW * PERS_SCRL);
     float dv = 0.f, dk = 0.f;
 #pragma unroll
     for (int w = 0; w < PERS_NW; ++w) { dv += sc[w * PERS_SCRL + lane]; dk += sc[w * PERS_SCRL + 64 + lane]; }
     const bool dead = sc[128] != 0.f;
-    const int b = it / p.heads, h = it - b * p.heads;
-    const int64_t row = ((int64_t)b * p.S + p.S - 1) * p.ldg + h * HD + lane;
-    p.dv[row] = dead ? (bf16_t)0.f : (bf16_t)dv;
-    p.dk[row] = dead ? (bf16_t)0.f : (bf16_t)(dk * p.scale);
-  };
-
-  for (; item < nitems; item += step, buf ^= 1) {
-    const int b = item / p.heads, h = item - b * p.heads;
+    const auto* pa = kernarg_fresh<AttnBwdArgs>();
+    const int64_t row = ((int64_t)b * p.S + p.S - 1) * pa->ldg + h * HD + lane;
+    pa->dv[row] = dead ? (bf16_t)0.f : (bf16_t)dv;
+    pa->dk[row] = dead ? (bf16_t)0.f : (bf16_t)(dk * pa->scale);
+  };
+
+  for (; item < nitems; item += step, buf ^= 1, ++trip) {
     asm volatile("s_waitcnt lgkmcnt(0)" ::: "memory");
     __builtin_amdgcn_s_barrier();
     asm volatile("" ::: "memory");
@@ -2155,8 +2232,11 @@
     const bool kdead[2] = {HAS_PAD && kdn[0] != 0u, HAS_PAD && kdn[1] != 0u};
     const bool ldead = HAS_PAD && LONE && kdl != 0u;
     const int nxt = item + step < nitems ? item + step : item;
-    if (LONE && prev_item >= 0 && wid == ((prev_item / step) & (PERS_NW - 1))) merge_lone(prev_item, buf ^ 1);
-    prev_item = item;
+    if (LONE && trip > 0 && wid == ((trip - 1) & (PERS_NW - 1))) merge_lone(pb, ph, buf ^ 1);
+    const int bn_ = nxt / p.heads, hn_ = nxt - bn_ * p.heads;
+    const bool wave_active = wave_fresh(kbase < min(p.S, 256)) != 0;
+    const bf16_t* const sb_it = HAS_BIAS ? biasT_of(kernarg_fresh<AttnBwdArgs>()->biasT, h) : nullptr;
+    const bf16_t* const sb_nxt = HAS_BIAS ? biasT_of(kernarg_fresh<AttnBwdArgs>()->biasT, hn_) : nullptr;
     const char* ldsQ = smem + buf * BUFB;
     const char* ldsO = ldsQ + QBY;
     const float* ldsL = reinterpret_cast<const float*>(ldsQ + 2 * QBY);
@@ -2168,15 +2248,16 @@
 #pragma unroll
       for (int db = 0; db < 4; ++db) { dvT[kb][db] = (f32x4){0.f, 0.f, 0.f, 0.f}; dkT[kb][db] = (f32x4){0.f, 0.f, 0.f, 0.f}; }
 
-    auto half = [&](const int q0h, auto nkb_c, const bf16x8 (&kx)[2][2], const bf16x8 (&vx)[2][2], const bf16x8 (&bx)[2],
+    auto half = [&](const int q0h, auto nkb_c, auto inside_c, const bf16x8 (&kx)[2][2], const bf16x8 (&vx)[2][2], const bf16x8 (&bx)[2],
                     f32x4 (&dvx)[2][4], f32x4 (&dkx)[2][4]) {
       constexpr int NKB = decltype(nkb_c)::value;
+      constexpr bool INSIDE = decltype(inside_c)::value;
       f32x4 s[2][NKB], dp[2][NKB];
 #pragma unroll
       for (int j = 0; j < 2; ++j)
 #pragma unroll
         for (int kb = 0; kb < NKB; ++kb) { s[j][kb] = (f32x4){0.f, 0.f, 0.f, 0.f}; dp[j][kb] = (f32x4){0.f, 0.f, 0.f, 0.f}; }
-      const bool second = q0h + 16 < p.S;
+      const bool second = INSIDE || wave_fresh(q0h + 16 < p.S) != 0;
 #pragma unroll
       for (int j = 0; j < 2; ++j) {
         if (j == 1 && !second) continue;
@@ -2219,9 +2300,10 @@
         const int qrow = q0h + j * 16 + g * 4;
         const f32x4 l4 = *reinterpret_cast<const f32x4*>(ldsL + qrow);
         const f32x4 d4 = *reinterpret_cast<const f32x4*>(ldsD + qrow);
+        const int limq = INSIDE ? 4 : lane_fresh(p.S - qrow);
 #pragma unroll
         for (int r = 0; r < 4; ++r) {
-          const bool live = qrow + r < p.S;
+          const bool live = INSIDE || r < limq;
           l2[j][r] = live ? l4[r] * LOG2E : INFINITY;
           dl[j][r] = live ? d4[r] : 0.f;
         }
@@ -2277,27 +2359,28 @@
       using QN = std::integral_constant<int, LAST ? 0 : QT + 1>;
       if constexpr (!LAST) {
 #pragma unroll
-        for (int jj = 0; jj < BPPT; ++jj) piece(nxt, buf ^ 1, min(QT * BPPT + jj, npiece - 1));
+        for (int jj = 0; jj < BPPT; ++jj) piece(bn_, hn_, buf ^ 1, min(QT * BPPT + jj, npiece - 1));
       }
       __builtin_amdgcn_sched_barrier(0);
-      if (wave_active) half(QT * 64, std::integral_constant<int, 2>{}, kf, vf, bn[0], dvT, dkT);
+      if (wave_active) half(QT * 64, std::integral_constant<int, 2>{}, std::integral_constant<bool, !LAST>{}, kf, vf, bn[0], dvT, dkT);
       __builtin_amdgcn_sched_barrier(0);
-      if constexpr (!LAST) bias_loads(item, QN{}, I0{});
+      if constexpr (!LAST) bias_loads(sb_it, QN{}, I0{});
       if constexpr (HAS_BIAS && QT > 0) {
         if constexpr (!LAST) asm volatile("s_waitcnt vmcnt(%2)" : "+v"(bn[1][0]), "+v"(bn[1][1]) : "n"(BPPT + NBH));
         else asm volatile("s_waitcnt vmcnt(0)" : "+v"(bn[1][0]), "+v"(bn[1][1]));
       }
       __builtin_amdgcn_sched_barrier(0);
-      if (wave_active && QT * 64 + 32 < p.S) half(QT * 64 + 32, std::integral_constant<int, 2>{}, kf, vf, bn[1], dvT, dkT);
+      if (wave_active && (!LAST || wave_fresh(QT * 64 + 32 < p.S) != 0))
+        half(QT * 64 + 32, std::integral_constant<int, 2>{}, std::integral_constant<bool, !LAST>{}, kf, vf, bn[1], dvT, dkT);
       __builtin_amdgcn_sched_barrier(0);
       if constexpr (!LAST) {
-        bias_loads(item, QN{}, I1{});
+        bias_loads(sb_it, QN{}, I1{});
         if constexpr (HAS_BIAS) asm volatile("s_waitcnt vmcnt(%2)" : "+v"(bn[0][0]), "+v"(bn[0][1]) : "n"(NBH));
       } else {
-        lone_bias_loads(item);
-        bias_loads(nxt, I0{}, I0{});
-        bias_loads(nxt, I0{}, I1{});
-        if constexpr (!LONE) kv_loads(nxt, kn, vn);
+        lone_bias_loads(sb_it);
+        bias_loads(sb_nxt, I0{}, I0{});
+        bias_loads(sb_nxt, I0{}, I1{});
+        if constexpr (!LONE) kv_loads(bn_, hn_, kn, vn);
       }
     };
     tile(std::integral_constant<int, 0>{});
@@ -2307,7 +2390,7 @@
     if constexpr (NT == 5) tile(std::integral_constant<int, 4>{});
 
     if constexpr (LONE) {
-      kv_loads(nxt, kf, vf);
+      kv_loads(bn_, hn_, kf, vf);
       if constexpr (NLB > 0) asm volatile("s_waitcnt vmcnt(%2)" : "+v"(bfl[0]), "+v"(bfl[1]) : "n"(NKV + 2 * NBH));
       const char* ldsLK = ldsQ + 2 * QBY + 4096;
       bf16x8 kl[2][2], vl[2][2];
@@ -2322,32 +2405,35 @@
 #pragma unroll
       for (int db = 0; db < 4; ++db) { dvl[0][db] = (f32x4){0.f, 0.f, 0.f, 0.f}; dkl[0][db] = (f32x4){0.f, 0.f, 0.f, 0.f}; }
       const bf16x8 bl0[2] = {bfl[0], bfl[0]}, bl1[2] = {bfl[1], bfl[1]};
-      half(wid * 32, std::integral_constant<int, 1>{}, kl, vl, bl0, dvl, dkl);
-      if (wid == 0) half(256, std::integral_constant<int, 1>{}, kl, vl, bl1, dvl, dkl);
+      half(wid * 32, std::integral_constant<int, 1>{}, std::true_type{}, kl, vl, bl0, dvl, dkl);
+      if (wid == 0) half(256, std::integral_constant<int, 1>{}, std::false_type{}, kl, vl, bl1, dvl, dkl);
       float* sc = scratch + (buf * PERS_NW + wid) * PERS_SCRL;
-      if (t == 0) {
+      if ((lane_fresh(lane) & 15) == 0) {
 #pragma unroll
         for (int db = 0; db < 4; ++db) {
           *reinterpret_cast<f32x4*>(sc + db * 16 + g * 4) = dvl[0][db];
           *reinterpret_cast<f32x4*>(sc + 64 + db * 16 + g * 4) = dkl[0][db];
         }
       }
-      if (wid == 0 && lane == 0) sc[128] = ldead ? 1.f : 0.f;
+      if (wid == 0 && lane_fresh(lane) == 0) sc[128] = ldead ? 1.f : 0.f;
     }
 
     {
-      const int nrec = ((min(p.S, 256) - 1) * (int)p.ldg + HD) * 2;
-      const u32x4 rk = attn_raw_rsrc(p.dk + (int64_t)b * p.S * p.ldg + h * HD, nrec);
-      const u32x4 rv = attn_raw_rsrc(p.dv + (int64_t)b * p.S * p.ldg + h * HD, nrec);
+      const auto* pa = kernarg_fresh<AttnBwdArgs>();
+      const int ldg = (int)pa->ldg;
+      const float scale = pa->scale;
+      const int nrec = ((min(p.S, 256) - 1) * ldg + HD) * 2;
+      const u32x4 rk = attn_raw_rsrc(pa->dk + (int64_t)b * p.S * ldg + h * HD, nrec);
+      const u32x4 rv = attn_raw_rsrc(pa->dv + (int64_t)b * p.S * ldg + h * HD, nrec);
 #pragma unroll
       for (int kb = 0; kb < 2; ++kb) {
-        const unsigned voff = (unsigned)(((kbase + kb * 16 + t) * (int)p.ldg + g * 4) * 2);
+        const unsigned voff = (unsigned)(((lane_fresh(kbase + kb * 16 + t)) * ldg + g * 4) * 2);
 #pragma unroll
         for (int db = 0; db < 4; ++db) {
           bf16x4 a, c;
 #pragma unroll
           for (int r = 0; r < 4; ++r) {
-            a[r] = kdead[kb] ? (bf16_t)0.f : (bf16_t)(dkT[kb][db][r] * p.scale);
+            a[r] = kdead[kb] ? (bf16_t)0.f : (bf16_t)(dkT[kb][db][r] * scale);
             c[r] = kdead[kb] ? (bf16_t)0.f : (bf16_t)dvT[kb][db][r];
           }
           bstore8(a, rk, voff + db * 32);
@@ -2356,10 +2442,12 @@
       }
       DKDV_WAIT_LOADS(16);
     }
-  }
-  if (LONE && prev_item >= 0) {
+    pb = b, ph = h;
+    b = bn_, h = hn_;
+  }
+  if (LONE && wave_fresh(trip) > 0) {
     __syncthreads();
-    if (wid == 0) merge_lone(prev_item, buf ^ 1);
+    if (wid == 0) merge_lone(pb, ph, buf ^ 1);
   }
 }
 
```
